# debbiemarkslab/EVcouplings

Hardware: AMD Instinct MI355X
Metric: plmc L-BFGS iterations/sec (PLM fit, synthetic MSA) (higher is better)
Workload: dtype f32 (forward: f16 hi/lo split couplings on the 2:4 sparse MFMA, f32 accumulation -- in the last iterations of a fit 39-bit fixed-point couplings as five int8 digit planes, exact; backward: 24-bit fixed-point residuals as three int8 digit planes on the int8 MFMA (32-bit / four there), exact int32 acc; 1 GPU; headline: synthetic MSA L=300 q=21 N=50000, theta=0.8, lambda_h=0.01, lambda_J=59.8; parallelism=single GPU

## Files before the change

### evcouplings_amd/_lib.py

```python
import ctypes as C
import os

_HERE = os.path.dirname(os.path.abspath(__file__))
LIB_PATH = os.environ.get("PLM_HIP_LIB") or os.path.join(_HERE, "libplm_hip.so")

PLM_OK = 0
STATUS_CONVERGED, STATUS_MAXITER, STATUS_LINESEARCH, STATUS_INTERRUPTED = 0, 1, 2, 3
ABI_VERSION = 2
K_EXPAND, K_FORWARD, K_BACKWARD, K_ASSEMBLE, K_TOTAL, K_REWEIGHT, K_FIELDS, K_FORWARD_ACCURATE, K_LBFGS_VECTOR, K_COUNT = 0, 1, 2, 3, 4, 5, 6, 7, 8, 9
S_COUNT = 7

ITER_CB = C.CFUNCTYPE(C.c_int, C.c_int32, C.c_double, C.c_double, C.c_double, C.c_double,
                      C.c_double, C.c_double, C.c_void_p)
EXCHANGE_CB = C.CFUNCTYPE(C.c_int, C.c_void_p, C.c_size_t, C.c_int32, C.c_int32, C.c_void_p)
COLLECTIVE_CB = C.CFUNCTYPE(C.c_int, C.c_int32, C.c_void_p, C.c_void_p, C.POINTER(C.c_int64),
                            C.POINTER(C.c_int64), C.c_int32, C.c_int32, C.c_void_p)
COLL_ALLTOALL, COLL_ALLREDUCE_F64, COLL_ALLREDUCE_F32, COLL_BROADCAST = 1, 2, 3, 4


class PlmProblem(C.Structure):
    _fields_ = [
        ("n_seqs", C.c_int32), ("n_sites", C.c_int32), ("n_states", C.c_int32),
        ("msa", C.c_void_p),
        ("theta_id", C.c_double), ("scale", C.c_double),
# ... 181 lines not shown
    ("plm_version", C.c_int, []),
    ("plm_device_count", C.c_int, []),
    ("plm_strerror", C.c_char_p, [C.c_int]),
    ("plm_last_error", C.c_char_p, []),
    ("plm_fit", C.c_int, [C.POINTER(PlmProblem), C.POINTER(PlmResult), C.c_int, _P, ITER_CB, _P,
                          EXCHANGE_CB, _P]),
    ("plm_fit_sharded", C.c_int, [C.POINTER(PlmProblem), C.POINTER(PlmResult), C.c_int, _P, ITER_CB, _P,
                                  COLLECTIVE_CB, _P]),
    ("plm_fit_sharded_rccl", C.c_int, [C.POINTER(PlmProblem), C.POINTER(PlmResult), C.c_int, _P, ITER_CB, _P, _P]),
    ("plm_rccl_unique_id", C.c_int, [_P]),
    ("plm_rccl_runtime_version", C.c_int, []),
    ("plm_rccl_selftest", C.c_int, [C.c_int, _P]),
    ("plm_ctx_attach_rccl", C.c_int, [_P, _P]),
    ("plm_reweight", C.c_int, [_P, C.c_int32, C.c_int32, C.c_double, _P]),
    ("plm_reweight_ex", C.c_int, [_P, C.c_int32, C.c_int32, C.c_double, C.c_int32, _P]),
    ("plm_marginals", C.c_int, [_P, _P, C.c_int32, C.c_int32, C.c_int32, _P, _P]),
    ("plm_eval", C.c_int, [_P, _P, C.c_int32, C.c_int32, C.c_int32, C.c_double, C.c_double, _P,
                           C.POINTER(C.c_double), C.POINTER(C.c_double), _P]),
    ("plm_scores", C.c_int, [_P, C.c_int32, C.c_int32, _P, _P]),
    ("plm_scores_ex", C.c_int, [_P, C.c_int32, C.c_int32, C.c_int32, _P, _P]),
    ("plm_hamiltonians", C.c_int, [_P, C.c_int32, C.c_int32, C.c_int32, _P, C.c_int, _P, _P]),
    ("plm_potentials", C.c_int, [_P, C.c_int32, C.c_int32, C.c_int32, _P, C.c_int, _P, _P]),
    ("plm_model_pair_scores", C.c_int, [_P, _P, _P, C.c_int32, C.c_int32, C.c_int, _P, _P, _P]),
    ("plm_model_pair_scores_ex", C.c_int, [_P, _P, _P, C.c_int32, C.c_int32, C.c_int32, C.c_int, _P, _P, _P]),
    ("plm_double_mutants", C.c_int, [_P, _P, _P, C.c_int32, C.c_int32, C.c_int, _P, _P]),
    ("plm_independent_fields", C.c_int, [_P, C.c_int32, C.c_int32, C.c_double, C.c_double, C.c_int, _P, _P, _P]),
    ("plm_sample", C.c_int, [C.c_int32, C.c_int32, _P, C.POINTER(PlmSampleOpts), C.c_int, _P, _P, _P]),
    ("plm_sample_plan", C.c_int, [C.c_int32, C.c_int32, C.c_int32, C.c_int32, C.POINTER(PlmSamplePlanInfo)]),
    ("plm_bm_fit", C.c_int, [C.c_int32, C.c_int32, _P, _P, _P, C.POINTER(PlmBmOpts), C.c_int, _P, BM_EPOCH_CB, _P,
                             C.POINTER(PlmBmResult)]),
    ("plm_ais", C.c_int, [C.c_int32, C.c_int32, _P, C.POINTER(PlmAisOpts), C.c_int, _P, AIS_CB, _P,
                          C.POINTER(PlmAisResult)]),
    ("plm_pt", C.c_int, [C.c_int32, C.c_int32, _P, C.POINTER(PlmPtOpts), C.c_int, _P, PT_CB, _P,
                         C.POINTER(PlmPtResult)]),
    ("plm_anneal", C.c_int, [C.c_int32, C.c_int32, _P, C.POINTER(PlmAnnealOpts), C.c_int, _P, ANNEAL_CB, _P,
                             C.POINTER(PlmAnnealResult)]),
    ("plm_meanfield", C.c_int, [_P, C.c_int32, C.c_int32, C.c_int32, C.c_double, C.c_double, C.c_int, _P,
                                C.POINTER(PlmMfResult)]),
    ("plm_direct_information", C.c_int, [_P, _P, C.c_int32, C.c_int32, C.c_int, _P, _P]),
    ("plm_alignment_stats", C.c_int, [_P, C.c_int32, C.c_int32, C.c_int32, _P, _P, _P, _P, C.c_int, _P]),
    ("plm_cross_identities", C.c_int, [_P, C.c_int32, _P, C.c_int32, C.c_int32, C.POINTER(PlmIdentOpts), _P, _P, _P, _P,
                                       C.c_int, _P]),
    ("plm_redundancy_filter", C.c_int, [_P, C.c_int32, C.c_int32, C.POINTER(PlmIdentOpts), _P, _P, C.c_int, _P]),
    ("plm_triplet_stats", C.c_int, [_P, _P, C.c_int32, C.c_int32, C.c_int32, _P, C.c_int32, C.POINTER(PlmTripletOpts), _P,
                                    _P, _P, C.POINTER(C.c_uint64), C.c_int, _P]),
    ("plm_triplet_scan", C.c_int, [_P, _P, C.c_int32, C.c_int32, C.c_int32, _P, C.c_int32, C.POINTER(PlmTripletOpts), _P,
                                   _P, _P, C.POINTER(C.c_uint64), C.c_int, _P]),
    ("plm_residue_distances", C.c_int, [_P, C.c_int32, _P, C.c_int32, _P, C.c_int32, _P, C.c_int32, _P, C.c_int, _P]),
    ("plm_distance_maps_aggregate", C.c_int, [_P, C.c_int32, _P, _P, C.c_int32, _P, _P, C.c_int32, C.c_int32, _P,
                                              C.c_int32, _P, _P, C.c_int, _P]),
    ("plm_fasta_split", C.c_int, [_P, C.c_int64, C.POINTER(C.c_int64), C.POINTER(C.c_int64), _P, _P, _P, _P]),
    ("plm_encode_columns", C.c_int, [_P, C.c_int64, C.c_int64, _P, C.c_int64, _P, _P, _P]),
    ("plm_write_raw_ec_file", C.c_int, [C.c_char_p, C.c_int32, _P, C.c_char_p, _P]),
    ("plm_ctx_create", C.c_int, [C.POINTER(PlmProblem), C.c_int, _P, C.POINTER(_P)]),
    ("plm_ctx_destroy", None, [_P]),
    ("plm_ctx_set_exchange", C.c_int, [_P, EXCHANGE_CB, _P]),
    ("plm_ctx_set_collective", C.c_int, [_P, COLLECTIVE_CB, _P]),
    ("plm_ctx_set_options", C.c_int, [_P, C.c_int32, C.c_double, C.c_int32]),
    ("plm_ctx_native_size", C.c_int64, [_P]),
    ("plm_ctx_reweight", C.c_int, [_P]),
    ("plm_ctx_set_weights", C.c_int, [_P, _P]),
    ("plm_ctx_get_weights", C.c_int, [_P, _P, _P, C.POINTER(C.c_float)]),
    ("plm_ctx_marginals", C.c_int, [_P, _P, _P]),
    ("plm_ctx_set_x", C.c_int, [_P, _P]),
    ("plm_ctx_get_x", C.c_int, [_P, _P]),
    ("plm_ctx_get_g", C.c_int, [_P, _P]),
    ("plm_ctx_eval", C.c_int, [_P, C.POINTER(C.c_double), C.POINTER(C.c_double)]),
    ("plm_ctx_optimize", C.c_int, [_P, ITER_CB, _P, C.POINTER(PlmResult)]),
    ("plm_ctx_scores", C.c_int, [_P, _P, _P]),
    ("plm_ctx_time_kernels", C.c_int, [_P, C.c_int32, _P]),
    ("plm_ctx_time_field_positions", C.c_int, [_P, C.c_int32, _P]),
    ("plm_ctx_solver_stats", C.c_int, [_P, _P]),
    ("plm_ctx_field_position", C.c_int, [_P, C.c_int32, C.c_int32, C.c_int32, C.c_int32, C.POINTER(PlmFieldBuffers)]),
    ("plm_ctx_field_solve", C.c_int, [_P, C.c_double, C.c_int32, C.c_int32, C.c_int32, C.POINTER(PlmFieldSolve), _P,
                                      C.c_int64]),
    ("plm_lbfgs_gram", C.c_int, [C.c_int64, C.c_int64, C.c_int32, C.c_int32, C.c_int32, _P, _P, _P, _P, _P, _P, _P, _P,
                                 C.c_int, _P, _P, _P, _P]),
    ("plm_lbfgs_direction", C.c_int, [C.c_int64, C.c_int32, C.c_int32, C.c_int32, _P, _P, _P, _P, _P, C.c_double, _P, _P,
                                      C.c_float, C.c_int, _P, _P]),
    ("plm_lbfgs_multidot", C.c_int, [C.c_int64, C.c_int32, _P, C.c_int32, _P, C.c_int32, _P, _P, C.c_uint32, C.c_uint64,
                                     C.c_int, _P]),
    ("plm_lbfgs_dots", C.c_int, [C.c_int64, C.c_int32, _P, C.c_int32, _P, _P, C.c_int64, C.c_int, _P]),
    ("plm_lbfgs_lincomb", C.c_int, [C.c_int64, C.c_float, _P, C.c_float, _P, C.c_int, _P]),
    ("plm_ctx_precond_diagonal", C.c_int, [_P, _P]),
    ("plm_rccl_probe", C.c_int, [_P, C.c_int32, C.c_int32, C.c_int, _P]),
    ("plm_rccl_probe_local", C.c_int, [C.c_int32, C.c_int, _P]),
    ("plm_lbfgs_coefficients", None, [C.c_int, C.c_int, C.c_int, _P, _P, _P, _P, C.c_double, _P, _P,
                                      C.POINTER(C.c_double), C.POINTER(C.c_double)]),
    ("plm_linesearch_run", C.c_int, [PHI_CB, _P, C.c_double, C.c_double, C.c_double, C.POINTER(C.c_int32),
                                     C.POINTER(C.c_int32), C.POINTER(C.c_double), _P]),
    ("plm_lbfgs_admit", C.c_int, [C.c_int32, C.POINTER(C.c_int32), C.POINTER(C.c_int32), C.POINTER(C.c_int32), _P, _P, _P,
                                  _P, C.POINTER(C.c_double), C.POINTER(C.c_double), _P, C.c_int32, C.c_int32, C.c_int32,
                                  C.c_int32, C.POINTER(C.c_int32), C.POINTER(C.c_int32)]),
    ("plm_mutant_effects", C.c_int, [_P, C.c_int32, C.c_int32, _P, C.c_int64, _P, C.c_int64, _P, _P, C.c_int, _P, _P, _P,
                                     _P]),
    ("plm_mutant_scan", C.c_int, [_P, C.c_int32, C.c_int32, _P, C.POINTER(PlmScanOpts), C.c_int, _P,
                                  C.POINTER(PlmScanResult)]),
]

_lib = None


class PlmError(RuntimeError):

    def __init__(self, code, message):
        super().__init__("libplm_hip error %d: %s" % (code, message))
        self.code = code


def load():
    global _lib
    if _lib is not None:
        return _lib
    if not os.path.exists(LIB_PATH):
        raise ImportError(
            "%s is missing: build it with `python -c 'import __graft_entry__ as g; g.build()'` "
            "(there is no CPU fallback for the PLM solver)" % LIB_PATH)
    lib = C.CDLL(LIB_PATH)
    for name, res, args in SYMBOLS:
        if os.environ.get("PLM_HIP_LIB") and not hasattr(lib, name):
            continue
        fn = getattr(lib, name)
        fn.restype = res
        fn.argtypes = args
    if lib.plm_version() != ABI_VERSION:
        raise ImportError("libplm_hip ABI version %d, expected %d" % (lib.plm_version(), ABI_VERSION))
    _lib = lib
    return lib


def check(rc):
    if rc != PLM_OK:
        lib = load()
        msg = lib.plm_last_error() or lib.plm_strerror(rc) or b""
        raise PlmError(rc, msg.decode("utf-8", "replace"))
```

### evcouplings_amd/csrc/plm_host.cpp

```cpp
#include "../../include/plm_hip.h"
#include "plm_internal.h"
#include "plm_host_util.h"
#include "plm_lbfgs.h"

#include <algorithm>
#include <chrono>
#include <cmath>
#include <cstdarg>
#include <cstdio>
#include <cstdlib>
#include <cstring>
#include <string>
#include <vector>

namespace {

thread_local std::string g_err;

int fail(int code, const char *fmt, ...) {
    char buf[512];
    va_list ap;
    va_start(ap, fmt);
    vsnprintf(buf, sizeof buf, fmt, ap);
    va_end(ap);
    g_err = buf;
    return code;
}

}
int plm_fail(int code, const char *fmt, ...) {
    char buf[512];
    va_list ap;
    va_start(ap, fmt);
    vsnprintf(buf, sizeof buf, fmt, ap);
    va_end(ap);
    return fail(code, "%s", buf);
}
namespace {

double now_s() {
    return std::chrono::duration<double>(std::chrono::steady_clock::now().time_since_epoch()).count();
}

int check_device(int device) {
    int n = 0;
    if (hipGetDeviceCount(&n) != hipSuccess || n <= 0)
        return fail(PLM_EDEVICE, "no HIP device visible (libplm_hip has no CPU path)");
    if (device < 0 || device >= n) return fail(PLM_EINVAL, "device %d out of range (%d visible)", device, n);
    hipDeviceProp_t prop;
    PLM_HIP(hipGetDeviceProperties(&prop, device));
    if (strncmp(prop.gcnArchName, "gfx950", 6) != 0)
        return fail(PLM_EDEVICE, "device %d is %s; this library is built for gfx950 only", device, prop.gcnArchName);
    PLM_HIP(hipSetDevice(device));
    return PLM_OK;
}

}
int plm_check_device(int device) { return check_device(device); }
namespace {

int cluster_threshold(double theta_id, int L, int conv) {
    if (conv & PLM_CONV_THRESHOLD_F32) {
        const float t = (float)(1.0 - theta_id);
        const float need = (1.0f - t) * (float)L;
        return (int)std::ceil(need);
    }
    return (int)std::ceil(theta_id * (double)L - 1e-9);
}

}
PlmOptions plm_options_from_env() {
    PlmOptions o;
    if (const char *e = getenv("PLM_BWD_PLANES")) o.bwd_planes = atoi(e) == 4 ? 4 : 3;
    if (const char *e = getenv("PLM_KSPLIT")) o.ksplit = std::max(1, atoi(e));
    if (const char *e = getenv("PLM_JEXP_BIAS")) o.jexp_bias = atoi(e);
    if (const char *e = getenv("PLM_BWD_KERNEL")) o.bwd_kernel = atoi(e) ? 1 : 0;
    if (const char *e = getenv("PLM_FWD_KERNEL")) o.fwd_kernel = atoi(e) ? 1 : 0;
    if (const char *e = getenv("PLM_FWD_ACCURATE")) o.fwd_mode = atoi(e) ? 1 : 0;
    if (const char *e = getenv("PLM_VP_FLOOR")) o.vp_floor = atof(e);
    if (const char *e = getenv("PLM_VP_REL")) o.vp_rel = atof(e);
    if (const char *e = getenv("PLM_VP_HESS_POS")) o.vp_hess_pos = atoi(e);
    if (const char *e = getenv("PLM_ACC_FACTOR")) o.acc_factor = atof(e);
    o.debug = getenv("PLM_DEBUG") != nullptr;
    o.debug_vp = getenv("PLM_DEBUG_VP") != nullptr;
    return o;
}
namespace {

int pick_ksplit(const PlmDims &d, const PlmOptions &opt, int nplanes, int *out) {
    const int ks_min = std::max(1, (d.nst128 + 1022) / 1023);
    const int ks_max = std::max(ks_min, std::max(1, std::min(16, d.nst128 / 8)));
    if ((int64_t)((d.nst128 + ks_min - 1) / ks_min) * PLM_BWD_KSTEP * 128 * 128 >= ((int64_t)1 << 31))
        return fail(PLM_EUNSUPPORTED, "%d sequences: no admissible K split of the backward GEMM", d.N);
    const double beta = (2.0 * nplanes * (double)d.nmf * d.nnfl * 1024.0 / 12e12) / ((double)d.nst128 * 1.3e-6);
    int best = ks_min;
    double best_cost = 1e300;
    for (int ks = ks_min; ks <= ks_max; ks++) {
        const int groups_per_xcd = (d.ncol_tiles * nplanes * ks + 7) / 8;
        const double cost = (double)((groups_per_xcd * d.nrow_tiles + 31) / 32) / ks + beta * ks;
        if (cost < best_cost * 0.98) { best_cost = cost; best = ks; }
    }
    if (opt.ksplit) best = std::max(ks_min, std::min(ks_max, opt.ksplit));
    *out = best;
    return PLM_OK;
}

int make_dims(const plm_problem_t &p, const PlmOptions &opt, PlmDims *out) {
    PlmDims d;
    memset(&d, 0, sizeof d);
    if (p.n_seqs <= 0 || p.n_sites <= 1) return fail(PLM_EINVAL, "need n_seqs > 0 and n_sites > 1");
    if (!plm_q_supported(p.n_states))
        return fail(PLM_EUNSUPPORTED, "alphabet size %d outside 2..32", p.n_states);
    const int nshards = p.n_shards > 0 ? p.n_shards : 1;
    if (p.shard < 0 || p.shard >= nshards) return fail(PLM_EINVAL, "shard %d outside 0..%d", p.shard, nshards - 1);
    d.N = p.n_seqs;
    d.L = p.n_sites;
    d.Qc = p.n_states;
    d.Q = plm_q_template(p.n_states);
    d.Np = (d.N + PLM_SEQ_TILE - 1) / PLM_SEQ_TILE * PLM_SEQ_TILE;
    d.nb16 = (d.L + 15) / 16;
    d.Lp16 = d.nb16 * 16;
    d.nu = (d.L + 31) / 32;
    d.Lp32 = d.nu * 32;
    d.nksteps = d.nu * PLM_FWD_TILES(d.Q);
    d.nssteps = d.Np / 32;
    d.nst128 = d.Np / PLM_BWD_KSTEP;
    d.nplanes = (p.epsilon > 0 && p.epsilon < 1e-4) ? 4 : 3;
    if (opt.bwd_planes) d.nplanes = opt.bwd_planes;
    d.jexp_bias = opt.jexp_bias;
    const float qmax = d.nplanes == 4 ? PLM_R_QMAX4 : PLM_R_QMAX3;
    d.rscale = qmax;
    d.gscale = 1.0f / (qmax * (float)PLM_BWD_ONEHOT_VALUE);
    d.nstiles = d.Np / PLM_SEQ_TILE;
    plm_pick_tile(d.Q, &d.FM, &d.FN);
    d.nmf = d.nb16 * d.Q + d.FM;
    d.nshards = nshards;
    d.shard = p.shard;
    d.blk_per_shard = (d.nb16 + nshards - 1) / nshards;
    d.shard_base = d.nb16 / nshards;
    d.shard_rem = d.nb16 % nshards;
    d.b16_lo = plm_shard_lo(d, d.shard);
    d.b16_hi = d.b16_lo + plm_shard_cnt(d, d.shard);
    d.nnfl = d.blk_per_shard * d.Q;
    d.nrow_tiles = (d.nmf + 4 * d.FM - 1) / (4 * d.FM);
    d.ncol_tiles = (d.nnfl + 2 * d.FN - 1) / (2 * d.FN);
    d.fwd_w = (d.Q == 21 && opt.fwd_kernel != 0) ? 1 : 0;
    d.bwd_w = (d.Q == 21 && opt.bwd_kernel != 0) ? 1 : 0;
    if (d.bwd_w) d.ncol_tiles = (d.nnfl + PLM_BWDW_COLS - 1) / PLM_BWDW_COLS;
    PLM_TRY(pick_ksplit(d, opt, d.nplanes, &d.ksplit));
    d.nbp = (int64_t)d.nb16 * (d.nb16 + 1) / 2;
    d.nh_pad = ((int64_t)d.L * d.Q + 255) / 256 * 256;
    d.n_native = d.nh_pad + d.nbp * d.Q * d.Q * 256;
    d.n_canon = (int64_t)d.L * d.Qc + (int64_t)d.L * (d.L - 1) / 2 * d.Qc * d.Qc;
    d.gap_mode = (p.flags & PLM_FLAG_IGNORE_GAPS) ? 1 : 0;
    d.conv = p.flags & PLM_CONV_MASK;
    d.theta = p.theta_id;
    d.sharded = ((p.flags & PLM_FLAG_SHARDED_STATE) && nshards > 1) ? 1 : 0;
    d.own_lo = d.sharded ? d.b16_lo : 0;
    d.own_hi = d.sharded ? d.b16_hi : d.nb16;
    d.nblk_own = d.own_hi - d.own_lo;
    d.h_site0 = d.own_lo * 16;
    d.bp_base = 0;
    for (int p = 0; p < PLM_MAX_SHARDS; p++) d.own_base[p] = d.oth_base[p] = -1;
    d.nx_halo = d.ng_halo = 0;
    if (d.sharded) {
        if (nshards > PLM_MAX_SHARDS) return fail(PLM_EUNSUPPORTED, "sharded-state mode takes at most %d shards", PLM_MAX_SHARDS);
        d.ntri = d.nblk_own * (d.nblk_own + 1) / 2;
        for (int p = 0; p < nshards; p++) {
            if (p == d.shard) continue;
            const int64_t mine = plm_half_blocks(d, p), theirs = (int64_t)d.nblk_own * plm_shard_cnt(d, p) - mine;
            d.own_base[p] = (int)d.ng_halo;
            d.ng_halo += mine;
            d.oth_base[p] = (int)d.nx_halo;
            d.nx_halo += theirs;
        }
        d.np_own = d.ntri + d.ng_halo;
    } else {
        d.np_own = d.nbp;
        d.ntri = (int)d.nbp;
    }
    {
        const int site_end = std::min(d.L, d.own_hi * 16);
        const int64_t nhl = (int64_t)std::max(0, site_end - d.h_site0) * d.Q;
        d.nh_pad_l = d.sharded ? std::max<int64_t>(256, (nhl + 255) / 256 * 256) : d.nh_pad;
    }
    d.n_local = d.nh_pad_l + d.np_own * d.Q * d.Q * 256;
    if (d.gap_mode && d.Qc < 3) return fail(PLM_EINVAL, "ignore_gaps needs at least 2 non-gap states");
    *out = d;
    return PLM_OK;
}

}

struct plm_ctx {
    plm_problem_t prob;
    PlmOptions opt;
    PlmDims d;
    int device = 0;
    hipStream_t st = nullptr;
    plm_exchange_cb exchange = nullptr;
    void *exchange_user = nullptr;
    int8_t *msa_rm = nullptr, *msa_cm = nullptr;
    float *w = nullptr;
    int32_t *counts = nullptr;
    void *Bt = nullptr, *Rt = nullptr;
    int32_t *G = nullptr;
    float *gather = nullptr;
    plm_collective_cb collective = nullptr;
    void *collective_user = nullptr;
    PlmRccl *rccl = nullptr;
    float *xhalo = nullptr, *ghalo = nullptr, *xsend = nullptr, *gsend = nullptr;
    std::vector<int64_t> x_send, x_recv, g_send, g_recv;
    double *fx_part = nullptr, *reg_part = nullptr, *dot_scratch = nullptr, *scal = nullptr;
    uint32_t *maxbits = nullptr;
    int32_t *jexp = nullptr;
    float *x = nullptr, *g = nullptr, *xp = nullptr, *gp = nullptr, *dir = nullptr, *hist = nullptr;
    float *xa = nullptr, *ga = nullptr;
    float *canon = nullptr;
    float *pair_n2 = nullptr;
    float *dinv = nullptr;
    float *hj = nullptr, *hpart = nullptr;
    double *gpart = nullptr, *dpart = nullptr;
    double *hg2 = nullptr, *hinv = nullptr, *h64 = nullptr;
    double *hcnt = nullptr;
    bool hcnt_valid = false;
    int *vp_flag = nullptr;
    int vp_hess_age = -1;
    int vp_c_prev = 3;
    int vp_pos = 0;
    unsigned vp_hess_mask = 0;
    int vp_extra = 0;
    double vp_last_gh2 = 0;
    double vp_floor2 = 0;
    hipEvent_t vp_ev[2] = {nullptr, nullptr};
    hipEvent_t gemm_ev[3] = {nullptr, nullptr, nullptr};
    bool vp_ev_pending = false;
    double stat_field_ms = 0, stat_passes = 0, stat_fwd_ms = 0, stat_bwd_ms = 0;
    int stat_gemm_evals = 0;
    int stat_field_evals = 0, stat_chain_short = 0;
    int hist_m = 0;
    double *h_scal = nullptr;
    bool have_weights = false;
    float wmax = 0;
    bool eval_valid = false;
    bool hj_at_x = false;
    double last_fx = 0, last_nll = 0, last_gh2 = 0;
    bool eval_vp = false;
    bool fwd_accurate = false;
    bool eval_accurate = false;
    int planes_base = 3, ksplit_base = 1, ksplit4 = 1;
    double n_eff = 0;
    int n_evals = 0;
    std::vector<float> h_fi;

    int n_fx_part() const { return d.nstiles * (d.b16_hi - d.b16_lo); }
};

namespace {

std::vector<int8_t> padded_rows(const PlmDims &d, const int8_t *seqs) {
    return plm_padded_rows(seqs, d.N, d.L, (size_t)d.Np + 32, (size_t)d.Lp32, (int8_t)PLM_PAD_STATE);
}

void ctx_set_accurate(plm_ctx *c, bool on) {
    c->fwd_accurate = on;
    const int planes = c->opt.bwd_planes ? c->opt.bwd_planes : (on ? 4 : c->planes_base);
    c->d.nplanes = planes;
    c->d.ksplit = planes == 4 ? c->ksplit4 : c->ksplit_base;
    const float qmax = planes == 4 ? PLM_R_QMAX4 : PLM_R_QMAX3, wmax = c->wmax > 0 ? c->wmax : 1.f;
    c->d.rscale = qmax / wmax;
    c->d.gscale = wmax / (qmax * (float)PLM_BWD_ONEHOT_VALUE);
}

int ctx_alloc_lbfgs(plm_ctx *c, int m) {
    if (c->xp && c->hist_m >= m) return PLM_OK;
    const size_t n = (size_t)c->d.n_local;
    if (!c->xp) {
        PLM_TRY(plm_dalloc(&c->xp, n));
        PLM_TRY(plm_dalloc(&c->gp, n));
        PLM_TRY(plm_dalloc(&c->dir, n));
    }
    if (c->hist) (void)hipFree(c->hist);
    c->hist = nullptr;
    PLM_TRY(plm_dalloc(&c->hist, n * 2 * (size_t)m));
    c->hist_m = m;
    return PLM_OK;
}

int ctx_collective(plm_ctx *c, int op, void *send, void *recv, const int64_t *scounts, const int64_t *rcounts) {
    if (c->rccl) {
        if (plm_rccl_collective(c->rccl, op, send, recv, scounts, rcounts, c->st) != 0)
            return fail(PLM_ECALLBACK, "RCCL collective failed (op %d): %s", op, plm_rccl_error());
        return PLM_OK;
    }
    if (!c->collective) return fail(PLM_EINVAL, "sharded-state mode needs a collective callback or an RCCL communicator");
    PLM_HIP(hipStreamSynchronize(c->st));
    if (c->collective(op, send, recv, scounts, rcounts, c->d.nshards, c->d.shard, c->collective_user) != 0)
        return fail(PLM_ECALLBACK, "collective callback failed (op %d)", op);
    return PLM_OK;
}
int ctx_allreduce_scalars(plm_ctx *c, int first, int count) {
    if (!c->d.sharded) return PLM_OK;
    const int64_t bytes = (int64_t)sizeof(double) * count;
    return ctx_collective(c, PLM_COLL_ALLREDUCE_F64, c->scal + first, c->scal + first, &bytes, &bytes);
}

int group_norms(plm_ctx *c) {
    if (!(c->prob.lambda_group > 0)) return PLM_OK;
    if (!c->pair_n2) PLM_TRY(plm_dalloc(&c->pair_n2, (size_t)std::max<int64_t>(1, c->d.np_own) * 256));
    PLM_HIP(plm_launch_pair_norms(c->d, c->x, c->pair_n2, c->st));
    return PLM_OK;
}
int vp_alloc(plm_ctx *c);
int forward_at_x(plm_ctx *c) {
    const PlmDims &d = c->d;
    PLM_TRY(vp_alloc(c));
    PLM_HIP(plm_launch_forward_store(d, c->msa_rm, c->Bt, c->jexp, c->hj, c->fwd_accurate, c->st));
    PLM_HIP(plm_launch_h64_init(d, c->x, c->h64, c->st));
    PLM_HIP(plm_launch_hpass(d, c->hj, c->msa_rm, c->w, c->h64, 1, 0, c->fwd_accurate, c->Rt, c->fx_part, nullptr, nullptr, nullptr, nullptr, PLM_VP_ALWAYS, c->st));
    return PLM_OK;
}

float *x_rectangles(plm_ctx *c) { return c->x + c->d.nh_pad_l + (size_t)c->d.ntri * PLM_BLOCK_FLOATS(c->d); }

int ctx_eval_enqueue_sharded(plm_ctx *c) {
    const PlmDims &d = c->d;
    PLM_TRY(ctx_collective(c, PLM_COLL_ALLTOALL, x_rectangles(c), c->xhalo, c->x_send.data(), c->x_recv.data()));
    PLM_HIP(plm_launch_maxabs2(c->x + d.nh_pad_l, d.n_local - d.nh_pad_l, c->xhalo,
                               d.nx_halo * (int64_t)PLM_BLOCK_FLOATS(d), c->maxbits, c->jexp, d.jexp_bias, c->st));
    PLM_HIP(plm_launch_expand(d, c->x, c->xhalo, c->jexp, c->Bt, c->fwd_accurate ? 1 : 0, c->st));
    PLM_TRY(forward_at_x(c));
    if (d.nblk_own > 0) PLM_HIP(plm_launch_backward(d, c->msa_cm, c->Rt, c->G, nullptr, c->st));
    PLM_HIP(plm_launch_pack_g(d, c->G, c->gsend, c->st));
    PLM_TRY(ctx_collective(c, PLM_COLL_ALLTOALL, c->gsend, c->ghalo, c->g_send.data(), c->g_recv.data()));
    PLM_TRY(group_norms(c));
    PLM_HIP(plm_launch_assemble(d, c->G, d.ksplit, c->ghalo, c->x, c->g, c->prob.lambda_h, c->prob.lambda_j,
                                c->reg_part, 0, 0.f, c->pair_n2, (float)c->prob.lambda_group, c->st));
    PLM_HIP(plm_launch_finish_fx(d, c->fx_part, c->n_fx_part(), nullptr, 0, c->reg_part, plm_reg_parts(d), c->scal,
                                 c->st));
    c->n_evals++;
    return PLM_OK;
}

int ctx_eval_enqueue(plm_ctx *c) {
    const PlmDims &d = c->d;
    if (d.sharded) return ctx_eval_enqueue_sharded(c);
    PLM_HIP(plm_launch_maxabs(d, c->x, c->maxbits, c->jexp, c->st));
    PLM_HIP(plm_launch_expand(d, c->x, nullptr, c->jexp, c->Bt, c->fwd_accurate ? 1 : 0, c->st));
    PLM_TRY(forward_at_x(c));
    PLM_HIP(plm_launch_backward(d, c->msa_cm, c->Rt, c->G, nullptr, c->st));
    const void *Gsrc = c->G;
    int ks_count = d.ksplit, n_shard_nll = 0;
    const double *shard_nll = nullptr;
    if (d.nshards > 1) {
        const size_t slab = plm_slab_bytes(d);
        char *mine = (char *)c->gather + (size_t)d.shard * slab;
        PLM_HIP(plm_launch_slab_reduce(d, c->G, (float *)mine, c->st));
        PLM_HIP(plm_launch_partial_sum(c->fx_part, c->n_fx_part(), (double *)(mine + slab - 256), c->st));
        PLM_HIP(hipStreamSynchronize(c->st));
        if (!c->exchange) return fail(PLM_EINVAL, "n_shards > 1 but no exchange callback set");
        if (c->exchange(c->gather, slab, d.nshards, d.shard, c->exchange_user) != 0)
            return fail(PLM_ECALLBACK, "exchange callback failed");
        Gsrc = c->gather;
        ks_count = 0;
        n_shard_nll = d.nshards;
        shard_nll = (const double *)((char *)c->gather + slab - 256);
    }
    PLM_TRY(group_norms(c));
    PLM_HIP(plm_launch_assemble(d, Gsrc, ks_count, nullptr, c->x, c->g, c->prob.lambda_h, c->prob.lambda_j,
                                c->reg_part, 0, 0.f, c->pair_n2, (float)c->prob.lambda_group, c->st));
    PLM_HIP(plm_launch_finish_fx(d, c->fx_part, c->n_fx_part(), shard_nll, n_shard_nll, c->reg_part,
                                 plm_reg_parts(d), c->scal, c->st));
    c->n_evals++;
    return PLM_OK;
}

bool vp_enabled(const plm_ctx *c) {
    return !(c->prob.flags & PLM_FLAG_JOINT_LBFGS) && (c->d.nshards == 1 || c->d.sharded) && c->prob.lambda_h > 0;
}
int vp_alloc(plm_ctx *c) {
    if (c->hj) return PLM_OK;
    const size_t nsites = (size_t)std::max(std::max(1, (c->d.b16_hi - c->d.b16_lo) * 16),
                                           std::min(c->d.L, c->d.own_hi * 16) - c->d.h_site0);
    PLM_TRY(plm_dalloc((char **)&c->hj, plm_hj_bytes(c->d)));
    PLM_TRY(plm_dalloc((char **)&c->hpart, plm_hpart_bytes(c->d)));
    PLM_TRY(plm_dalloc((char **)&c->gpart, plm_gpart_bytes(c->d)));
    PLM_TRY(plm_dalloc((char **)&c->dpart, plm_gpart_bytes(c->d)));
    PLM_TRY(plm_dalloc(&c->hg2, nsites));
    PLM_TRY(plm_dalloc(&c->hinv, nsites * c->d.Q * c->d.Q));
    PLM_TRY(plm_dalloc(&c->h64, 2 * plm_h64_stride(c->d)));
    PLM_TRY(plm_dalloc(&c->hcnt, plm_h64_stride(c->d)));
    c->hcnt_valid = false;
    PLM_TRY(plm_dalloc((char **)&c->vp_flag, sizeof(PlmVpState)));
    PLM_HIP(hipMemsetAsync(c->vp_flag, 0, sizeof(PlmVpState), c->st));
    for (auto &e : c->vp_ev) PLM_HIP(hipEventCreate(&e));
    for (auto &e : c->gemm_ev) PLM_HIP(hipEventCreate(&e));
    c->vp_hess_age = -1;
    return PLM_OK;
}
int vp_counts(plm_ctx *c) {
    if (!c->hcnt_valid) {
        PLM_HIP(plm_launch_site_counts(c->d, c->msa_cm, c->w, c->hcnt, c->st));
        c->hcnt_valid = true;
    }
    return PLM_OK;
}
int vp_stage1(plm_ctx *c) {
    const PlmDims &d = c->d;
    PLM_TRY(vp_counts(c));
    if (d.sharded) {
        PLM_TRY(ctx_collective(c, PLM_COLL_ALLTOALL, x_rectangles(c), c->xhalo, c->x_send.data(), c->x_recv.data()));
        PLM_HIP(plm_launch_maxabs2(c->x + d.nh_pad_l, d.n_local - d.nh_pad_l, c->xhalo,
                                   d.nx_halo * (int64_t)PLM_BLOCK_FLOATS(d), c->maxbits, c->jexp, d.jexp_bias, c->st));
        PLM_HIP(plm_launch_expand(d, c->x, c->xhalo, c->jexp, c->Bt, c->fwd_accurate ? 1 : 0, c->st));
    } else {
        PLM_HIP(plm_launch_maxabs(d, c->x, c->maxbits, c->jexp, c->st));
        PLM_HIP(plm_launch_expand(d, c->x, nullptr, c->jexp, c->Bt, c->fwd_accurate ? 1 : 0, c->st));
    }
    if (c->gemm_ev[0]) PLM_HIP(hipEventRecord(c->gemm_ev[0], c->st));
    PLM_HIP(plm_launch_forward_store(d, c->msa_rm, c->Bt, c->jexp, c->hj, c->fwd_accurate, c->st));
    PLM_HIP(plm_launch_h64_init(d, c->x, c->h64, c->st));
    return PLM_OK;
}
int vp_counts(plm_ctx *c);
int vp_step_and_residuals(plm_ctx *c, bool refresh) {
    const PlmDims &d = c->d;
    PLM_TRY(vp_counts(c));
    const int full = (refresh || c->vp_hess_age < 0) ? 1 : 0;
    PLM_HIP(plm_launch_hpass(d, c->hj, c->msa_rm, c->w, c->h64, 0, full ? 2 : 1, c->fwd_accurate, nullptr, nullptr, c->hpart,
                             c->gpart, c->dpart, nullptr, PLM_VP_ALWAYS, c->st));
    PLM_HIP(plm_launch_hsolve(d, c->hpart, c->gpart, full, c->x, c->h64, c->prob.lambda_h, 1, c->hinv, c->hg2, c->scal + 5, 0.0,
                              0.0, nullptr, 0, c->hcnt, c->dpart, c->st));
    if (full) c->vp_hess_age = 0;
    PLM_HIP(plm_launch_hpass(d, c->hj, c->msa_rm, c->w, c->h64, 1, 1, c->fwd_accurate, c->Rt, c->fx_part, c->hpart, c->gpart,
                             nullptr, nullptr, PLM_VP_ALWAYS, c->st));
    PLM_HIP(plm_launch_hsolve(d, c->hpart, c->gpart, 0, c->x, c->h64, c->prob.lambda_h, 0, c->hinv, c->hg2, c->scal + 5, 0.0,
                              0.0, nullptr, 0, c->hcnt, c->dpart, c->st));
    return PLM_OK;
}
int vp_chain(plm_ctx *c, int npos, int hess_upto, int expected_last, double tol2) {
    const PlmDims &d = c->d;
    for (int k = 0; k < npos; k++) {
        const int pos = c->vp_pos++;
        const bool hess = pos < hess_upto || pos > expected_last || c->vp_hess_age < 0;
        PLM_HIP(plm_launch_hpass(d, c->hj, c->msa_rm, c->w, c->h64, 0, hess ? 2 : 1, c->fwd_accurate, nullptr, nullptr, c->hpart,
                                 c->gpart, c->dpart, c->vp_flag, PLM_VP_PASS, c->st));
        PLM_HIP(plm_launch_hpass(d, c->hj, c->msa_rm, c->w, c->h64, 1, 1, c->fwd_accurate, c->Rt, c->fx_part, c->hpart, c->gpart,
                                 nullptr, c->vp_flag, PLM_VP_PASS_RT, c->st));
        PLM_HIP(plm_launch_hsolve(d, c->hpart, c->gpart, hess ? 2 : 0, c->x, c->h64, c->prob.lambda_h, 1, c->hinv, c->hg2,
                                  c->scal + 5, tol2, c->vp_floor2, c->vp_flag, 1, c->hcnt, c->dpart, c->st));
        if (hess && pos < 32) c->vp_hess_mask |= 1u << pos;
        if (hess && c->vp_hess_age < 0) c->vp_hess_age = 0;
    }
    return PLM_OK;
}
int vp_stage3(plm_ctx *c, bool conditional, float *gout = nullptr, int mode = 2) {
    const PlmDims &d = c->d;
    if (!gout) gout = c->g;
    if (c->gemm_ev[1]) PLM_HIP(hipEventRecord(c->gemm_ev[1], c->st));
    if (d.nblk_own > 0 || !d.sharded)
        PLM_HIP(plm_launch_backward(d, c->msa_cm, c->Rt, c->G, (conditional && !d.sharded) ? c->vp_flag : nullptr, c->st));
    if (c->gemm_ev[2]) PLM_HIP(hipEventRecord(c->gemm_ev[2], c->st));
    if (d.sharded) {
        PLM_HIP(plm_launch_pack_g(d, c->G, c->gsend, c->st));
        PLM_TRY(ctx_collective(c, PLM_COLL_ALLTOALL, c->gsend, c->ghalo, c->g_send.data(), c->g_recv.data()));
    }
    PLM_TRY(group_norms(c));
    PLM_HIP(plm_launch_assemble(d, c->G, d.ksplit, d.sharded ? c->ghalo : nullptr, c->x, gout, c->prob.lambda_h,
                                c->prob.lambda_j, c->reg_part, mode, 0.f, c->pair_n2, (float)c->prob.lambda_group, c->st));
    if (mode == 2)
        PLM_HIP(plm_launch_finish_fx(d, c->fx_part, c->n_fx_part(), nullptr, 0, c->reg_part, plm_reg_parts(d), c->scal,
                                     c->st));
    return PLM_OK;
}
int ctx_eval_vp_enqueue(plm_ctx *c, double tol2) {
    const PlmDims &d = c->d;
    PLM_TRY(vp_stage1(c));
    if (c->vp_ev_pending) c->vp_ev_pending = false;
    PLM_HIP(hipEventRecord(c->vp_ev[0], c->st));
    const int c_prev = c->vp_c_prev;
    if (c->vp_hess_age >= 0) c->vp_hess_age++;
    const bool stale = c->vp_hess_age < 0 || c->vp_hess_age >= 32;
    PLM_HIP(plm_launch_vp_reset(c->vp_flag, (c_prev == 0 && !stale) ? 1 : 0, c->scal + 5, c->st));
    c->vp_pos = 0;
    c->vp_extra = 0;
    c->vp_hess_mask = 0;
    c->vp_last_gh2 = INFINITY;
    int hess_upto = c_prev >= 2 ? c_prev : (stale ? 1 : 0);
    if (c->opt.vp_hess_pos >= 0) hess_upto = std::min(hess_upto, std::max(c->opt.vp_hess_pos, c->vp_hess_age < 0 ? 1 : 0));
    PLM_TRY(vp_chain(c, std::min(14, c_prev + 3), hess_upto, c_prev, tol2));
    PLM_HIP(plm_launch_fields_to_x(d, c->h64, c->vp_flag, c->x, c->st));
    PLM_HIP(plm_launch_hpass(d, c->hj, c->msa_rm, c->w, c->h64, 1, 0, c->fwd_accurate, c->Rt, c->fx_part, nullptr, nullptr, nullptr,
                             c->vp_flag, PLM_VP_FINAL, c->st));
    PLM_HIP(hipEventRecord(c->vp_ev[1], c->st));
    c->vp_ev_pending = true;
    PLM_TRY(vp_stage3(c, true));
    c->n_evals++;
    return PLM_OK;
}
// ... 73 lines not shown
template <class Fetch>
int ctx_eval_vp_run(plm_ctx *c, double tol2, Fetch &&fetch, double *gh2_out) {
    PLM_TRY(ctx_eval_vp_enqueue(c, tol2));
    for (;;) {
        PLM_TRY(fetch());
        bool again = false;
        PLM_TRY(ctx_eval_vp_finish(c, tol2, &again, gh2_out));
        if (!again) break;
    }
    return PLM_OK;
}

int dots(plm_ctx *c, int npairs, const float *const *a, const float *const *b, int64_t n, int slot) {
    PLM_HIP(plm_launch_dots(npairs, a, b, n, c->dot_scratch, c->scal + slot, c->st));
    return PLM_OK;
}

const char *status_text(int status) {
    switch (status) {
    case PLM_STATUS_CONVERGED: return "converged (|g|/max(1,|x|) below epsilon)";
    case PLM_STATUS_MAXITER: return "maximum number of iterations reached";
    case PLM_STATUS_INTERRUPTED: return "interrupted by the caller";
    default: return "line search could not improve further (treated as converged to precision)";
    }
}

int set_start_point(plm_ctx *c) {
    const PlmDims &d = c->d;
    if (c->h_fi.empty()) return fail(PLM_EINVAL, "start point needs single-site frequencies: run marginals first");
    std::vector<float> h((size_t)d.nh_pad_l, 0.f);
    const int a0 = d.gap_mode;
    for (int i = d.h_site0; i < std::min(d.L, d.own_hi * 16); i++) {
        double mean = 0;
        std::vector<double> v(d.Q);
        for (int a = a0; a < d.Qc; a++) {
            v[a] = std::log((double)c->h_fi[(size_t)i * d.Qc + a] + 1.0 / c->n_eff);
            mean += v[a];
        }
        mean /= (d.Qc - a0);
        for (int a = a0; a < d.Qc; a++) h[(size_t)(i - d.h_site0) * d.Q + a] = (float)(v[a] - mean);
    }
    c->eval_valid = false;
    PLM_HIP(hipMemsetAsync(c->x, 0, sizeof(float) * d.n_local, c->st));
    PLM_HIP(hipMemcpyAsync(c->x, h.data(), sizeof(float) * d.nh_pad_l, hipMemcpyHostToDevice, c->st));
    PLM_HIP(hipStreamSynchronize(c->st));
    return PLM_OK;
}

}

extern "C" {

int plm_version(void) { return PLM_ABI_VERSION; }

int plm_device_count(void) {
    int n = 0;
    if (hipGetDeviceCount(&n) != hipSuccess) return fail(PLM_EDEVICE, "hipGetDeviceCount failed");
    return n;
}

const char *plm_strerror(int code) {
    switch (code) {
    case PLM_OK: return "ok";
    case PLM_EINVAL: return "invalid argument";
    case PLM_ENOMEM: return "out of memory";
    case PLM_EDEVICE: return "HIP device error";
    case PLM_EUNSUPPORTED: return "unsupported alphabet size";
    case PLM_ENUMERIC: return "non-finite value in objective";
    case PLM_ECALLBACK: return "exchange callback failed";
    default: return "unknown error";
    }
}

const char *plm_last_error(void) { return g_err.c_str(); }

void plm_ctx_destroy(plm_ctx_t *c) {
    if (!c) return;
    (void)hipSetDevice(c->device);
    for (auto &e : c->gemm_ev)
        if (e) (void)hipEventDestroy(e);
    for (auto &e : c->vp_ev)
        if (e) (void)hipEventDestroy(e);
    void *bufs[] = {c->msa_rm, c->msa_cm, c->w, c->counts, c->Bt, c->Rt, c->G, c->gather, c->fx_part, c->reg_part,
                    c->dot_scratch, c->scal, c->maxbits, c->jexp, c->x, c->g, c->xp, c->gp, c->dir, c->hist,
                    c->canon, c->xhalo, c->ghalo, c->xsend, c->gsend, c->dinv, c->hj, c->hpart, c->gpart, c->dpart, c->hg2, c->hinv, c->h64, c->hcnt, c->vp_flag,
                    c->xa, c->ga, c->pair_n2};
    for (void *b : bufs)
        if (b) (void)hipFree(b);
    if (c->h_scal) (void)hipHostFree(c->h_scal);
    if (c->rccl) {
        (void)hipStreamSynchronize(c->st);
        plm_rccl_destroy(c->rccl);
    }
    delete c;
}

struct CtxScope {
    plm_ctx_t *c;
    ~CtxScope() { plm_ctx_destroy(c); }
};

int plm_ctx_create(const plm_problem_t *prob, int device, void *stream, plm_ctx_t **out) {
    if (!prob || !out || !prob->msa) return fail(PLM_EINVAL, "NULL problem / msa / out");
    *out = nullptr;
    PLM_TRY(check_device(device));
    const PlmOptions opt = plm_options_from_env();
    PlmDims d;
    PLM_TRY(make_dims(*prob, opt, &d));
    if (!(prob->theta_id >= 0.0 && prob->theta_id <= 1.0)) return fail(PLM_EINVAL, "theta_id must be in [0,1]");
    if (prob->lambda_h < 0 || prob->lambda_j < 0 || prob->lambda_group < 0)
        return fail(PLM_EINVAL, "negative regularisation strength");
    for (size_t k = 0; k < (size_t)d.N * d.L; k++)
        if (prob->msa[k] < 0 || prob->msa[k] >= d.Qc)
            return fail(PLM_EINVAL, "msa[%zu] = %d outside 0..%d", k, (int)prob->msa[k], d.Qc - 1);
    plm_ctx *c = new plm_ctx();
    c->prob = *prob;
    c->prob.msa = nullptr;
    c->opt = opt;
    c->d = d;
    c->planes_base = d.nplanes;
    c->ksplit_base = d.ksplit;
    {
        int ks4 = 1;
        const int rc4 = pick_ksplit(d, opt, 4, &ks4);
        if (rc4 != PLM_OK) { delete c; return rc4; }
        c->ksplit4 = ks4;
    }
    PlmDims dmax = d;
    dmax.nplanes = opt.bwd_planes ? opt.bwd_planes : 4;
    dmax.ksplit = std::max(c->ksplit_base, c->ksplit4);
    c->device = device;
    c->st = (hipStream_t)stream;
    CtxScope scope{c};
    const size_t cm_rows = (size_t)(d.nb16 + 1) * 16, cm_size = cm_rows * d.Np;
    const std::vector<int8_t> rm = padded_rows(d, prob->msa);
    {
        const int m = std::min(20, prob->lbfgs_m > 0 ? prob->lbfgs_m : 6);
        const double need = (double)rm.size() + (double)cm_size + (double)plm_bt_bytes(d) + (double)plm_rt_bytes(dmax) +
                            (double)plm_g_bytes(dmax) + (vp_enabled(c) ? (double)plm_hj_bytes(d) : 0.0) +
                            4.0 * ((double)d.n_local * (2 * m + 5) + (double)d.n_canon + (double)d.L * d.L);
        PLM_TRY(plm_check_free(need, "the problem"));
    }
    PLM_TRY(plm_dalloc(&c->msa_rm, rm.size()));
    PLM_TRY(plm_dalloc(&c->msa_cm, cm_size));
    PLM_TRY(plm_dalloc(&c->w, (size_t)d.Np));
    PLM_TRY(plm_dalloc(&c->counts, (size_t)d.Np));
    PLM_TRY(plm_dalloc((char **)&c->Bt, plm_bt_bytes(d)));
    PLM_TRY(plm_dalloc((char **)&c->Rt, plm_rt_bytes(dmax)));
    PLM_TRY(plm_dalloc((char **)&c->G, plm_g_bytes(dmax)));
    PLM_TRY(plm_dalloc(&c->fx_part, (size_t)c->n_fx_part()));
    PLM_TRY(plm_dalloc(&c->reg_part, (size_t)plm_reg_parts(d)));
    PLM_TRY(plm_dalloc(&c->dot_scratch, (size_t)4 * PLM_MAX_BASIS * PLM_DOT_BLOCKS));
    PLM_TRY(plm_dalloc(&c->scal, (size_t)256));
    PLM_TRY(plm_dalloc(&c->maxbits, (size_t)1));
    PLM_TRY(plm_dalloc(&c->jexp, (size_t)1));
    PLM_TRY(plm_dalloc(&c->x, (size_t)d.n_local));
    PLM_TRY(plm_dalloc(&c->g, (size_t)d.n_local));
    PLM_TRY(plm_dalloc(&c->canon, (size_t)d.n_canon + (size_t)d.L * d.L));
    if (d.nshards > 1 && !d.sharded) PLM_TRY(plm_dalloc((char **)&c->gather, plm_slab_bytes(d) * d.nshards));
    if (d.sharded) {
        const size_t blk = PLM_BLOCK_FLOATS(d);
        PLM_TRY(plm_dalloc(&c->xhalo, (size_t)d.nx_halo * blk));
        PLM_TRY(plm_dalloc(&c->gsend, (size_t)d.nx_halo * blk));
        PLM_TRY(plm_dalloc(&c->ghalo, (size_t)d.ng_halo * blk));
        c->x_send.assign(d.nshards, 0); c->x_recv.assign(d.nshards, 0);
        c->g_send.assign(d.nshards, 0); c->g_recv.assign(d.nshards, 0);
        for (int r = 0; r < d.nshards; r++) {
            if (r == d.shard) continue;
            const int64_t mine = plm_half_blocks(d, r), theirs = (int64_t)d.nblk_own * plm_shard_cnt(d, r) - mine;
            c->x_send[r] = c->g_recv[r] = mine * (int64_t)blk * 4;
            c->x_recv[r] = c->g_send[r] = theirs * (int64_t)blk * 4;
        }
    }
    const hipError_t eh = hipHostMalloc((void **)&c->h_scal, sizeof(double) * 256);
    if (eh != hipSuccess) return fail(PLM_ENOMEM, "hipHostMalloc failed: %s", hipGetErrorString(eh));
    PLM_HIP(hipMemcpyAsync(c->msa_rm, rm.data(), rm.size(), hipMemcpyHostToDevice, c->st));
    PLM_HIP(plm_launch_msa_columns(d, c->msa_rm, c->msa_cm, (int)cm_rows, c->st));
    PLM_HIP(hipMemsetAsync(c->w, 0, sizeof(float) * d.Np, c->st));
    PLM_HIP(hipMemsetAsync(c->Rt, 0, plm_rt_bytes(dmax), c->st));
    PLM_HIP(hipMemsetAsync(c->x, 0, sizeof(float) * d.n_local, c->st));
    PLM_HIP(hipMemsetAsync(c->g, 0, sizeof(float) * d.n_local, c->st));
    PLM_HIP(hipMemsetAsync(c->scal, 0, sizeof(double) * 256, c->st));
    if (c->gather) PLM_HIP(hipMemsetAsync(c->gather, 0, plm_slab_bytes(d) * d.nshards, c->st));
    PLM_HIP(hipStreamSynchronize(c->st));
    scope.c = nullptr;
    *out = c;
    return PLM_OK;
}

int plm_ctx_set_exchange(plm_ctx_t *c, plm_exchange_cb exchange, void *user) {
    if (!c) return fail(PLM_EINVAL, "NULL ctx");
    c->exchange = exchange;
    c->exchange_user = user;
    return PLM_OK;
}

int plm_ctx_set_collective(plm_ctx_t *c, plm_collective_cb collective, void *user) {
    if (!c) return fail(PLM_EINVAL, "NULL ctx");
    c->collective = collective;
    c->collective_user = user;
    return PLM_OK;
}

int plm_ctx_attach_rccl(plm_ctx_t *c, const void *rccl_id) {
    if (!c || !rccl_id) return fail(PLM_EINVAL, "NULL ctx / id");
    if (c->rccl) return fail(PLM_EINVAL, "context already has a communicator");
    PLM_HIP(hipSetDevice(c->device));
    if (plm_rccl_init(rccl_id, c->d.nshards, c->d.shard, &c->rccl) != 0)
        return fail(PLM_ECALLBACK, "RCCL communicator of %d ranks: %s", c->d.nshards, plm_rccl_error());
    return PLM_OK;
}

int plm_rccl_unique_id(void *id_out) {
    if (!id_out) return fail(PLM_EINVAL, "NULL id");
    if (plm_rccl_id(id_out) != 0) return fail(PLM_ECALLBACK, "%s", plm_rccl_error());
    return PLM_OK;
}
int plm_rccl_runtime_version(void) { return plm_rccl_version(); }

int plm_rccl_selftest(int device, void *stream) {
    PLM_TRY(check_device(device));
    hipStream_t st = (hipStream_t)stream;
    unsigned char id[PLM_RCCL_ID_BYTES];
    PLM_TRY(plm_rccl_unique_id(id));
    PlmRccl *r = nullptr;
    if (plm_rccl_init(id, 1, 0, &r) != 0) return fail(PLM_ECALLBACK, "%s", plm_rccl_error());
    const int n = 1000;
    double *buf = nullptr;
    DeviceBuffers mem;
    int rc = mem.alloc(&buf, (size_t)2 * n);
    std::vector<double> h(2 * n, 0.0), back(2 * n, -1.0);
    for (int k = 0; k < n; k++) h[k] = 0.5 * k - 7.0;
    const int64_t bytes = (int64_t)sizeof(double) * n, root = 0;
    auto run = [&](int op, void *s, void *d) {
        if (rc == PLM_OK && plm_rccl_collective(r, op, s, d, &bytes, op == PLM_COLL_BROADCAST ? &root : &bytes, st) != 0)
            rc = fail(PLM_ECALLBACK, "op %d: %s", op, plm_rccl_error());
    };
    if (rc == PLM_OK && hipMemcpyAsync(buf, h.data(), sizeof(double) * 2 * n, hipMemcpyHostToDevice, st) != hipSuccess)
// ... 245 lines not shown
int plm_ctx_get_g(plm_ctx_t *c, float *g_canonical_host) { return get_vec(c, c ? c->g : nullptr, g_canonical_host); }

int plm_ctx_eval(plm_ctx_t *c, double *fx_out, double *nll_out) {
    if (!c) return fail(PLM_EINVAL, "NULL ctx");
    if (!c->have_weights) return fail(PLM_EINVAL, "weights not set");
    PLM_HIP(hipSetDevice(c->device));
    ctx_set_accurate(c, c->opt.fwd_mode != 0);
    PLM_TRY(ctx_eval_enqueue(c));
    if (c->d.sharded) PLM_TRY(ctx_allreduce_scalars(c, 0, 2));
    c->eval_valid = false;
    if (fx_out || nll_out) {
        PLM_TRY(fetch_scalars(c, 0, 2));
        if (fx_out) *fx_out = c->h_scal[0];
        if (nll_out) *nll_out = c->h_scal[1];
        c->eval_valid = true;
        c->eval_vp = false;
        c->eval_accurate = c->fwd_accurate;
        c->last_fx = c->h_scal[0];
        c->last_nll = c->h_scal[1];
    }
    return PLM_OK;
}

static int ctx_build_dinv(plm_ctx_t *c) {
    const PlmDims &d = c->d;
    if (!c->dinv) PLM_TRY(plm_dalloc(&c->dinv, (size_t)d.n_local));
    const size_t lq = (size_t)d.L * d.Q;
    std::vector<float> fv(2 * lq, 0.f);
    const int a0 = d.gap_mode;
    for (int i = 0; i < d.L; i++) {
        double tot = 0;
        for (int a = a0; a < d.Qc; a++) tot += (double)c->h_fi[i * d.Qc + a] + 1.0 / c->n_eff;
        for (int a = a0; a < d.Qc; a++) {
            const double pa = ((double)c->h_fi[i * d.Qc + a] + 1.0 / c->n_eff) / tot;
            fv[i * d.Q + a] = c->h_fi[i * d.Qc + a];
            fv[lq + i * d.Q + a] = (float)(pa * (1.0 - pa));
        }
    }
    PLM_HIP(hipMemcpyAsync(c->canon, fv.data(), sizeof(float) * fv.size(), hipMemcpyHostToDevice, c->st));
    PLM_HIP(plm_launch_precond(d, c->canon, (float)c->n_eff, (float)c->prob.lambda_h, (float)c->prob.lambda_j,
                               c->dinv, c->st));
    PLM_HIP(hipStreamSynchronize(c->st));
    return PLM_OK;
}
static void lbfgs_gram_basis(const float *S, const float *Y, const float *g, int64_t n, int nst, PlmVecList *B,
                             unsigned long long *wb_out, unsigned *wq_out) {
    B->n = 0;
    for (int i = 0; i < nst; i++) B->v[B->n++] = S + (size_t)i * n;
    unsigned long long wb = 0;
    for (int i = 0; i < nst; i++) { wb |= 1ull << B->n; B->v[B->n++] = Y + (size_t)i * n; }
    wb |= 1ull << B->n;
    B->v[B->n++] = g;
    B->v[B->n++] = g;
    *wb_out = wb;
    *wq_out = 6u;
}
static int lbfgs_direction_basis(const float *S, const float *Y, const float *g, int64_t n, int m, int stored, int end,
                                 const double *cs, const double *cy, double cg, PlmVecList *B, PlmCoefList *C) {
    B->n = 0;
    for (int i = 0; i < stored; i++) { const int j = lbfgs_live_slot(m, end, i); B->v[B->n] = S + (size_t)j * n; C->c[B->n++] = (float)cs[j]; }
    const int first_weighted = B->n;
    for (int i = 0; i < stored; i++) { const int j = lbfgs_live_slot(m, end, i); B->v[B->n] = Y + (size_t)j * n; C->c[B->n++] = (float)cy[j]; }
    B->v[B->n] = g;
    C->c[B->n++] = (float)cg;
    return first_weighted;
}

int plm_ctx_optimize(plm_ctx_t *c, plm_iter_cb cb, void *user, plm_result_t *res) {
    if (!c) return fail(PLM_EINVAL, "NULL ctx");
    if (!c->have_weights) return fail(PLM_EINVAL, "weights not set");
    PLM_HIP(hipSetDevice(c->device));
    const double eps = c->prob.epsilon > 0 ? c->prob.epsilon : 1e-3;
    const double t0 = now_s();
    const PlmDims &d = c->d;
    const int64_t n = d.n_local;
    const int m = std::min(20, c->prob.lbfgs_m > 0 ? c->prob.lbfgs_m : 6);
    const int max_iter = c->prob.max_iter;
    PLM_TRY(ctx_alloc_lbfgs(c, m));
    float *S = c->hist, *Y = c->hist + (size_t)m * n;
    const bool precond = (c->prob.flags & PLM_FLAG_PRECOND) && !c->h_fi.empty();
    if (precond) PLM_TRY(ctx_build_dinv(c));
    const float *dinv = precond ? c->dinv : nullptr;
    LbfgsHistory hist(m);
    double xx = 0, hh = 0;
    c->n_evals = 0;
    enum { SL_FX = 0, SL_NLL = 1, SL_DG = 2, SL_XX = 3, SL_HH = 4, SL_GH2 = 5, SL_MD = 8 };

    auto norm_dots = [&]() -> int {
        const float *a[1] = {c->x};
        PLM_TRY(dots(c, 1, a, a, n, SL_XX));
        PLM_TRY(dots(c, 1, a, a, d.nh_pad_l, SL_HH));
        return PLM_OK;
    };
    auto direction = [&](double *dginit, const float *xacc, float stp0, float *trial) -> int {
        double cg;
        hist.coefficients(&cg, dginit);
        PlmVecList B;
        PlmCoefList C;
        const int first_weighted =
            lbfgs_direction_basis(S, Y, c->g, n, m, hist.stored, hist.end, hist.cs.data(), hist.cy.data(), cg, &B, &C);
        if (trial) PLM_HIP(plm_launch_multiaxpy_trial(c->dir, B, C, n, dinv, first_weighted, xacc, stp0, trial, c->st));
        else PLM_HIP(plm_launch_multiaxpy(c->dir, B, C, n, dinv, first_weighted, c->st));
        return PLM_OK;
    };

    const bool vp = vp_enabled(c);
    if (vp) PLM_TRY(vp_alloc(c));
    c->stat_field_ms = c->stat_passes = c->stat_fwd_ms = c->stat_bwd_ms = 0;
    c->stat_field_evals = c->stat_chain_short = c->stat_gemm_evals = 0;
    double gh2 = 0;
    const double vp_rel = c->opt.vp_rel;
    c->vp_floor2 = ctx_vp_floor2(c);
    auto vp_tol2 = [&](double xnorm2) {
        const double t = std::max(0.1 * eps * std::max(1.0, std::sqrt(xnorm2)), vp_rel * std::sqrt(hist.gg));
        return t * t;
    };
    const double fwd_noise = 3e-11 * (double)d.N * (double)d.L;
    const double acc_thr = std::max(3.0 * eps, c->opt.acc_factor * fwd_noise);
    auto want_accurate = [&](double cond) {
        return c->opt.fwd_mode == 1 || (c->opt.fwd_mode != 0 && fwd_noise > 0.05 * eps && cond < acc_thr);
    };
    const bool resume = c->eval_valid && c->eval_vp == vp;
    ctx_set_accurate(c, c->opt.fwd_mode == 1 || (c->opt.fwd_mode != 0 && resume && c->eval_accurate));
    auto start_eval = [&](bool have) -> int {
        const double tol2 = vp_tol2((double)d.L);
        auto fetch = [&]() -> int {
            PlmVecList Qg, Bg;
            Qg.n = 1; Qg.v[0] = c->g;
            Bg.n = 2; Bg.v[0] = c->g; Bg.v[1] = c->g;
            PLM_HIP(plm_launch_multidot(Qg, Bg, n, c->dot_scratch, c->scal + SL_MD, dinv, 1u, 1ull, c->st));
            PLM_TRY(norm_dots());
            PLM_TRY(ctx_allreduce_scalars(c, have ? SL_DG : 0, (have ? 8 - SL_DG : 8) + 2));
            PLM_TRY(fetch_scalars(c, 0, 10));
            return PLM_OK;
        };
        if (vp && !have) {
            PLM_TRY(ctx_eval_vp_run(c, tol2, fetch, &gh2));
        } else {
            if (!have) PLM_TRY(ctx_eval_enqueue(c));
            PLM_TRY(fetch());
        }
        hist.gDg = c->h_scal[SL_MD];
        hist.gg = c->h_scal[SL_MD + 1];
        xx = c->h_scal[SL_XX];
        hh = c->h_scal[SL_HH];
        return PLM_OK;
    };
    PLM_TRY(start_eval(resume));
    if (resume) gh2 = c->last_gh2;
    double fx = resume ? c->last_fx : c->h_scal[SL_FX], nll = resume ? c->last_nll : c->h_scal[SL_NLL];
    c->eval_valid = false;
    if (!std::isfinite(fx)) return fail(PLM_ENUMERIC, "objective is not finite at the start point");
    if (!c->fwd_accurate && want_accurate(std::sqrt(hist.gg + gh2) / std::max(1.0, std::sqrt(xx)))) {
        ctx_set_accurate(c, true);
        PLM_TRY(start_eval(false));
        fx = c->h_scal[SL_FX];
        nll = c->h_scal[SL_NLL];
    }
    auto shipped_cond = [&](double *out) -> int {
        PLM_HIP(plm_launch_h64_init(d, c->x, c->h64, c->st));
        PLM_HIP(plm_launch_hpass(d, c->hj, c->msa_rm, c->w, c->h64, 1, 0, c->fwd_accurate, c->Rt, c->fx_part, nullptr, nullptr,
                                 nullptr, nullptr, PLM_VP_ALWAYS, c->st));
        PLM_TRY(vp_stage3(c, false, c->dir, 0));
        const float *a[1] = {c->dir};
        PLM_TRY(dots(c, 1, a, a, n, SL_DG));
        PLM_TRY(ctx_allreduce_scalars(c, SL_DG, 1));
        PLM_TRY(fetch_scalars(c, SL_DG, 1));
        *out = std::sqrt(c->h_scal[SL_DG]) / std::max(1.0, std::sqrt(xx));
        return PLM_OK;
    };
    double eps_eff = eps;
    double rounding_note = 0;
    int n_cert = 0;
    int k = 0, status = PLM_STATUS_CONVERGED, ls_reason = 0, restarts = 0;
    double last_cond = std::sqrt(hist.gg + gh2) / std::max(1.0, std::sqrt(xx));
    if (last_cond <= eps && vp && (!resume || c->hj_at_x)) {
        double cj = 0;
        PLM_TRY(shipped_cond(&cj));
        const double r2 = std::max(0.0, cj * cj - last_cond * last_cond);
        if (cj > eps && r2 >= 0.75 * eps * eps) rounding_note = std::sqrt(r2);
        else if (cj > eps) { eps_eff = std::sqrt(eps * eps - r2); last_cond = cj; }
    }
    if (last_cond > eps) {
        auto first_step = [&]() { return precond ? std::min(1.0, 1.0 / std::sqrt(hist.gDg)) : 1.0 / std::sqrt(hist.gg); };
        double step = first_step();
        for (k = 1;; k++) {
            double dginit;
            const float stp0 = (float)std::max(MtSearch::stpmin, std::min(MtSearch::stpmax, step));
            PLM_TRY(direction(&dginit, c->x, stp0, c->xp));
            if (!(dginit < 0)) { status = PLM_STATUS_LINESEARCH; ls_reason = 10; k--; break; }
            std::swap(c->x, c->xp);
            std::swap(c->g, c->gp);
            const double finit = fx, nllinit = nll;
            float *s_new = S + (size_t)hist.end * n, *y_new = Y + (size_t)hist.end * n;
            const int nst = hist.nst();
            PlmVecList B;
            unsigned long long wb;
            unsigned wq;
            lbfgs_gram_basis(S, Y, c->g, n, nst, &B, &wb, &wq);
            double gh2_trial = 0;
            auto evaluate_trial = [&]() -> int {
                const double tol2 = vp_tol2(xx);
                if (!vp) PLM_TRY(ctx_eval_enqueue(c));
                else PLM_TRY(ctx_eval_vp_enqueue(c, tol2));
              for (;;) {
                PLM_HIP(plm_launch_sy_multidot(s_new, y_new, c->x, hist.anchored ? c->xa : c->xp, c->g, hist.anchored ? c->ga : c->gp,
                                               c->dir, B, n, d.nh_pad_l, c->dot_scratch, c->scal + SL_MD, c->scal + SL_DG, dinv,
                                               wq, wb, c->st));
                PLM_TRY(ctx_allreduce_scalars(c, SL_FX, SL_MD + 3 * B.n + 1 - SL_FX));
                PLM_TRY(fetch_scalars(c, SL_FX, SL_MD + 3 * B.n + 1 - SL_FX));
                bool again = false;
                if (vp) PLM_TRY(ctx_eval_vp_finish(c, tol2, &again, &gh2_trial));
                if (!again) break;
              }
                return PLM_OK;
            };
            MtSearch ls;
            ls.start(finit, dginit, step);
            int lsrc;
            do {
                const double stp = ls.next();
                if (!(ls.count == 0 && (float)stp == stp0))
                    PLM_HIP(plm_launch_lincomb(c->x, 1.f, c->xp, (float)stp, c->dir, n, c->st));
                PLM_TRY(evaluate_trial());
                double dg = c->h_scal[SL_DG];
                fx = c->h_scal[SL_FX];
                nll = c->h_scal[SL_NLL];
                lsrc = ls.feed(fx, dg);
            } while (lsrc == 0);
            if (lsrc < 0 && c->opt.debug) ls.dump_failure(k, lsrc);
            if (lsrc < 0) {
                std::swap(c->x, c->xp);
                std::swap(c->g, c->gp);
                fx = finit;
                nll = nllinit;
                k--;
                if (hist.stored > 0 && restarts < 2) {
                    restarts++;
                    hist.reset();
                    step = first_step();
                    continue;
                }
                status = PLM_STATUS_LINESEARCH;
                ls_reason = -lsrc;
                break;
            }
            restarts = 0;
            if (c->opt.debug)
                fprintf(stderr, "[plm] it %d: %d trial(s), step %.4e (first %.4e), f - f0 = %.6e, dg0 = %.4e, dg = %.4e%s\n", k, ls.count, ls.stp,
                        ls.trace[0][0], fx - finit, dginit, c->h_scal[SL_DG], c->fwd_accurate ? " [accurate]" : "");
            step = ls.stp;
            const double *md = c->h_scal + SL_MD;
            const int nbv = B.n;
            bool straddle = false;
            if (!c->fwd_accurate &&
                want_accurate(std::sqrt(md[2 * nbv + 2 * nst + 1] + gh2_trial) / std::max(1.0, std::sqrt(c->h_scal[SL_XX])))) {
                ctx_set_accurate(c, true);
                straddle = true;
                PLM_TRY(evaluate_trial());
                fx = c->h_scal[SL_FX];
                nll = c->h_scal[SL_NLL];
                if (!std::isfinite(fx)) return fail(PLM_ENUMERIC, "objective is not finite after the switch of the forward GEMM");
            }
            hist.absorb(md, nbv, nst);
            xx = c->h_scal[SL_XX];
            hh = c->h_scal[SL_HH];
            gh2 = gh2_trial;
            const double xnorm = std::sqrt(xx), gnorm = std::sqrt(hist.gg + gh2);
            last_cond = gnorm / std::max(1.0, xnorm);
            if (cb && cb(k, now_s() - t0, last_cond, fx, nll, std::sqrt(hh), std::sqrt(std::max(0.0, xx - hh)), user) != 0) {
                status = PLM_STATUS_INTERRUPTED;
                break;
            }
            if (last_cond <= eps_eff) {
                if (!vp) { status = PLM_STATUS_CONVERGED; break; }
                double cj = 0;
                PLM_TRY(shipped_cond(&cj));
                if (!(cj > eps)) { last_cond = cj; status = PLM_STATUS_CONVERGED; break; }
                const double r2 = std::max(0.0, cj * cj - last_cond * last_cond);
                if (r2 >= 0.75 * eps * eps || ++n_cert > 8) {
                    status = PLM_STATUS_CONVERGED;
                    rounding_note = std::sqrt(r2);
                    break;
                }
                eps_eff = std::min(0.9 * eps_eff, std::sqrt(eps * eps - r2));
            }
            if (max_iter > 0 && k >= max_iter) { status = PLM_STATUS_MAXITER; break; }
            if (hist.admit(md, nbv, nst, vp, straddle, c->opt.debug).copy_anchor) {
                if (!c->xa) {
                    PLM_TRY(plm_dalloc(&c->xa, (size_t)n));
                    PLM_TRY(plm_dalloc(&c->ga, (size_t)n));
                }
                PLM_HIP(hipMemcpyAsync(c->xa, c->xp, sizeof(float) * n, hipMemcpyDeviceToDevice, c->st));
                PLM_HIP(hipMemcpyAsync(c->ga, c->gp, sizeof(float) * n, hipMemcpyDeviceToDevice, c->st));
            }
            step = 1.0;
        }
    }
    PLM_HIP(hipStreamSynchronize(c->st));
    c->eval_valid = true;
    c->hj_at_x = vp && status != PLM_STATUS_LINESEARCH;
    c->eval_vp = vp;
    c->eval_accurate = c->fwd_accurate;
    c->last_fx = fx;
    c->last_nll = nll;
    c->last_gh2 = gh2;
// ... 201 lines not shown
        PLM_HIP(hipMemset(*p, 0xFF, sizeof(T) * n_elems));
        return PLM_OK;
    }
    int nan_scratch() {
        if (!scratch) PLM_TRY(mem.alloc(&scratch, n_scratch));
        PLM_HIP(hipMemset(scratch, 0xFF, sizeof(double) * n_scratch));
        return PLM_OK;
    }
    template <typename T> int download(T *host, const T *p, size_t n_elems) {
        PLM_HIP(hipMemcpy(host, p, sizeof(T) * n_elems, hipMemcpyDeviceToHost));
        return PLM_OK;
    }
};
int lbfgs_probe_length(int64_t n) {
    if (n <= 0 || (n & 3)) return fail(PLM_EINVAL, "the vector length must be a positive multiple of 4, not %lld", (long long)n);
    return PLM_OK;
}
}
}

int plm_lbfgs_gram(int64_t n, int64_t nh, int32_t m, int32_t end, int32_t nst, const float *S, const float *Y,
                   const float *x, const float *xp, const float *g, const float *gp, const float *dir, const float *dinv,
                   int device, float *s_new, float *y_new, double *md, double *ex) {
    if (!S || !Y || !x || !xp || !g || !gp || !dir || !s_new || !y_new || !md || !ex) return fail(PLM_EINVAL, "NULL argument");
    PLM_TRY(lbfgs_probe_length(n));
    if (nh < 0 || (nh & 3) || nh > n) return fail(PLM_EINVAL, "nh must be a multiple of 4 in 0..n, not %lld", (long long)nh);
    if (m < 1 || nst < 1 || nst > m) return fail(PLM_EINVAL, "need 1 <= nst <= m (m = %d, nst = %d)", (int)m, (int)nst);
    if (2 * nst + 2 > PLM_MAX_BASIS) return fail(PLM_EINVAL, "%d basis vectors, at most %d", 2 * (int)nst + 2, PLM_MAX_BASIS);
    if (end < 0 || end >= m) return fail(PLM_EINVAL, "ring slot %d outside 0..%d", (int)end, (int)m - 1);
    if (end >= nst) return fail(PLM_EINVAL, "the new pair's slot %d is not among the %d slots of the basis", (int)end, (int)nst);
    PLM_TRY(check_device(device));
    LbfgsProbe P;
    float *dS, *dY, *dx, *dxp, *dg, *dgp, *ddir, *ddinv = nullptr;
    double *dmd, *dex;
    const size_t nn = (size_t)n;
    PLM_TRY(P.upload(&dS, S, (size_t)nst * nn));
    PLM_TRY(P.upload(&dY, Y, (size_t)nst * nn));
    PLM_TRY(P.upload(&dx, x, nn));
    PLM_TRY(P.upload(&dxp, xp, nn));
    PLM_TRY(P.upload(&dg, g, nn));
    PLM_TRY(P.upload(&dgp, gp, nn));
    PLM_TRY(P.upload(&ddir, dir, nn));
    if (dinv) PLM_TRY(P.upload(&ddinv, dinv, nn));
    PlmVecList B;
    unsigned long long wb;
    unsigned wq;
    lbfgs_gram_basis(dS, dY, dg, n, nst, &B, &wb, &wq);
    PLM_TRY(P.nan_out(&dmd, (size_t)3 * B.n + 1));
    PLM_TRY(P.nan_out(&dex, 3));
    PLM_TRY(P.nan_scratch());
    float *ds_new = dS + (size_t)end * nn, *dy_new = dY + (size_t)end * nn;
    PLM_HIP(plm_launch_sy_multidot(ds_new, dy_new, dx, dxp, dg, dgp, ddir, B, n, nh, P.scratch, dmd, dex, ddinv, wq, wb, nullptr));
    PLM_HIP(hipDeviceSynchronize());
    PLM_TRY(P.download(s_new, ds_new, nn));
    PLM_TRY(P.download(y_new, dy_new, nn));
    PLM_TRY(P.download(md, dmd, (size_t)3 * B.n + 1));
    PLM_TRY(P.download(ex, dex, 3));
    return PLM_OK;
}

int plm_lbfgs_direction(int64_t n, int32_t m, int32_t stored, int32_t end, const float *S, const float *Y, const float *g,
                        const double *cs, const double *cy, double cg, const float *dinv, const float *xacc, float stp0,
                        int device, float *dir, float *trial) {
    if (!S || !Y || !g || !cs || !cy || !dir) return fail(PLM_EINVAL, "NULL argument");
    if (trial && !xacc) return fail(PLM_EINVAL, "a trial point needs xacc");
    PLM_TRY(lbfgs_probe_length(n));
    if (m < 1 || stored < 0 || stored > m) return fail(PLM_EINVAL, "need 0 <= stored <= m (m = %d, stored = %d)", (int)m, (int)stored);
    if (2 * stored + 1 > PLM_MAX_BASIS) return fail(PLM_EINVAL, "%d basis vectors, at most %d", 2 * (int)stored + 1, PLM_MAX_BASIS);
    if (end < 0 || end >= m) return fail(PLM_EINVAL, "ring slot %d outside 0..%d", (int)end, (int)m - 1);
    PLM_TRY(check_device(device));
    LbfgsProbe P;
    float *dS, *dY, *dg, *ddinv = nullptr, *dxacc = nullptr, *ddir, *dtrial = nullptr;
    const size_t nn = (size_t)n;
    PLM_TRY(P.upload(&dS, S, (size_t)m * nn));
    PLM_TRY(P.upload(&dY, Y, (size_t)m * nn));
    PLM_TRY(P.upload(&dg, g, nn));
    if (dinv) PLM_TRY(P.upload(&ddinv, dinv, nn));
    if (trial) PLM_TRY(P.upload(&dxacc, xacc, nn));
    PLM_TRY(P.nan_out(&ddir, nn));
    if (trial) PLM_TRY(P.nan_out(&dtrial, nn));
    PlmVecList B;
    PlmCoefList C;
    const int first_weighted = lbfgs_direction_basis(dS, dY, dg, n, m, stored, end, cs, cy, cg, &B, &C);
    if (trial) PLM_HIP(plm_launch_multiaxpy_trial(ddir, B, C, n, ddinv, first_weighted, dxacc, stp0, dtrial, nullptr));
    else PLM_HIP(plm_launch_multiaxpy(ddir, B, C, n, ddinv, first_weighted, nullptr));
    PLM_HIP(hipDeviceSynchronize());
    PLM_TRY(P.download(dir, ddir, nn));
    if (trial) PLM_TRY(P.download(trial, dtrial, nn));
    return PLM_OK;
}

int plm_lbfgs_multidot(int64_t n, int32_t nv, const float *V, int32_t nq, const int32_t *q_index, int32_t nb,
                       const int32_t *b_index, const float *dinv, uint32_t wq, uint64_t wb, int device, double *out) {
    if (!V || !q_index || !b_index || !out) return fail(PLM_EINVAL, "NULL argument");
    PLM_TRY(lbfgs_probe_length(n));
    if (nv < 1) return fail(PLM_EINVAL, "no vectors");
    if (nq < 1 || nq > 4) return fail(PLM_EINVAL, "%d queries, need 1..4", (int)nq);
    if (nb < 1 || nb > PLM_MAX_BASIS) return fail(PLM_EINVAL, "%d basis vectors, need 1..%d", (int)nb, PLM_MAX_BASIS);
    for (int k = 0; k < nq; k++)
        if (q_index[k] < 0 || q_index[k] >= nv) return fail(PLM_EINVAL, "query %d names vector %d of %d", k, (int)q_index[k], (int)nv);
    for (int k = 0; k < nb; k++)
        if (b_index[k] < 0 || b_index[k] >= nv) return fail(PLM_EINVAL, "basis entry %d names vector %d of %d", k, (int)b_index[k], (int)nv);
    PLM_TRY(check_device(device));
    LbfgsProbe P;
    float *dV, *ddinv = nullptr;
    double *dout;
    const size_t nn = (size_t)n;
    PLM_TRY(P.upload(&dV, V, (size_t)nv * nn));
    if (dinv) PLM_TRY(P.upload(&ddinv, dinv, nn));
    PLM_TRY(P.nan_out(&dout, (size_t)nq * nb));
    PLM_TRY(P.nan_scratch());
    PlmVecList Qv, B;
    Qv.n = nq;
    for (int k = 0; k < nq; k++) Qv.v[k] = dV + (size_t)q_index[k] * nn;
    B.n = nb;
    for (int k = 0; k < nb; k++) B.v[k] = dV + (size_t)b_index[k] * nn;
    PLM_HIP(plm_launch_multidot(Qv, B, n, P.scratch, dout, ddinv, wq, wb, nullptr));
    PLM_HIP(hipDeviceSynchronize());
    PLM_TRY(P.download(out, dout, (size_t)nq * nb));
    return PLM_OK;
}

int plm_lbfgs_dots(int64_t stride, int32_t nv, const float *V, int32_t npairs, const int32_t *a_index,
                   const int32_t *b_index, int64_t n, int device, double *out) {
    if (!V || !a_index || !b_index || !out) return fail(PLM_EINVAL, "NULL argument");
    PLM_TRY(lbfgs_probe_length(stride));
    if (n < 0 || (n & 3) || n > stride) return fail(PLM_EINVAL, "n must be a multiple of 4 in 0..stride, not %lld", (long long)n);
    if (nv < 1) return fail(PLM_EINVAL, "no vectors");
    if (npairs < 1 || npairs > 4) return fail(PLM_EINVAL, "%d pairs, need 1..4", (int)npairs);
    for (int k = 0; k < npairs; k++)
        if (a_index[k] < 0 || a_index[k] >= nv || b_index[k] < 0 || b_index[k] >= nv)
            return fail(PLM_EINVAL, "pair %d names vectors %d, %d of %d", k, (int)a_index[k], (int)b_index[k], (int)nv);
    PLM_TRY(check_device(device));
    LbfgsProbe P;
    float *dV;
    double *dout;
    const size_t ns = (size_t)stride;
    PLM_TRY(P.upload(&dV, V, (size_t)nv * ns));
    PLM_TRY(P.nan_out(&dout, (size_t)npairs));
    PLM_TRY(P.nan_scratch());
    const float *a[4], *b[4];
    for (int k = 0; k < npairs; k++) { a[k] = dV + (size_t)a_index[k] * ns; b[k] = dV + (size_t)b_index[k] * ns; }
    PLM_HIP(plm_launch_dots(npairs, a, b, n, P.scratch, dout, nullptr));
    PLM_HIP(hipDeviceSynchronize());
    PLM_TRY(P.download(out, dout, (size_t)npairs));
    return PLM_OK;
}

int plm_lbfgs_lincomb(int64_t n, float ca, const float *a, float cb, const float *b, int device, float *out) {
    if (!a || !out) return fail(PLM_EINVAL, "NULL argument");
    PLM_TRY(lbfgs_probe_length(n));
    PLM_TRY(check_device(device));
    LbfgsProbe P;
    float *da, *db = nullptr, *dout;
    PLM_TRY(P.upload(&da, a, (size_t)n));
    if (b) PLM_TRY(P.upload(&db, b, (size_t)n));
    PLM_TRY(P.nan_out(&dout, (size_t)n));
    PLM_HIP(plm_launch_lincomb(dout, ca, da, cb, db, n, nullptr));
    PLM_HIP(hipDeviceSynchronize());
    PLM_TRY(P.download(out, dout, (size_t)n));
    return PLM_OK;
}

int plm_ctx_precond_diagonal(plm_ctx_t *c, float *canonical_out) {
    if (!c || !canonical_out) return fail(PLM_EINVAL, "NULL argument");
    if (c->d.nshards != 1 || c->d.sharded) return fail(PLM_EINVAL, "the H0 diagonal is returned for single-shard contexts only");
    if (c->h_fi.empty()) return fail(PLM_EINVAL, "the H0 diagonal needs single-site frequencies: run marginals first");
    PLM_HIP(hipSetDevice(c->device));
    PLM_TRY(ctx_build_dinv(c));
    return get_vec(c, c->dinv, canonical_out);
}

int plm_ctx_time_kernels(plm_ctx_t *c, int32_t reps, float *out_ms) {
    if (!c || !out_ms || reps <= 0) return fail(PLM_EINVAL, "bad argument");
    if (!c->have_weights) return fail(PLM_EINVAL, "weights not set");
    if (c->d.nshards > 1 && !c->d.sharded) return fail(PLM_EUNSUPPORTED, "kernel timing runs on 1-shard or sharded-state contexts");
    PLM_HIP(hipSetDevice(c->device));
    c->eval_valid = false;
    ctx_set_accurate(c, false);
    const PlmDims &d = c->d;
    struct Events {
        hipEvent_t e[6] = {nullptr, nullptr, nullptr, nullptr, nullptr, nullptr};
        ~Events() { for (auto &x : e) if (x) (void)hipEventDestroy(x); }
    } evs;
    hipEvent_t (&ev)[6] = evs.e;
    for (auto &e : ev) PLM_HIP(hipEventCreate(&e));
    double acc[PLM_K_COUNT] = {0};
    const bool vp = vp_enabled(c);
    if (vp) PLM_TRY(vp_alloc(c));
    for (int r = 0; r < reps; r++) {
        float ms;
        PLM_HIP(hipEventRecord(ev[0], c->st));
        if (d.sharded) {
            PLM_HIP(plm_launch_maxabs2(c->x + d.nh_pad_l, d.n_local - d.nh_pad_l, c->xhalo,
                                       d.nx_halo * (int64_t)PLM_BLOCK_FLOATS(d), c->maxbits, c->jexp, d.jexp_bias, c->st));
            PLM_HIP(plm_launch_expand(d, c->x, c->xhalo, c->jexp, c->Bt, c->fwd_accurate ? 1 : 0, c->st));
        } else {
            PLM_HIP(plm_launch_maxabs(d, c->x, c->maxbits, c->jexp, c->st));
            PLM_HIP(plm_launch_expand(d, c->x, nullptr, c->jexp, c->Bt, c->fwd_accurate ? 1 : 0, c->st));
        }
        PLM_HIP(hipEventRecord(ev[1], c->st));
        if (vp) {
            PLM_HIP(plm_launch_forward_store(d, c->msa_rm, c->Bt, c->jexp, c->hj, 0, c->st));
            PLM_HIP(hipEventRecord(ev[2], c->st));
            PLM_TRY(vp_step_and_residuals(c, r == 0));
            PLM_HIP(hipEventRecord(ev[5], c->st));
        } else {
            PLM_TRY(forward_at_x(c));
            PLM_HIP(hipEventRecord(ev[2], c->st));
            PLM_HIP(hipEventRecord(ev[5], c->st));
        }
        if (d.nblk_own > 0 || !d.sharded) PLM_HIP(plm_launch_backward(d, c->msa_cm, c->Rt, c->G, nullptr, c->st));
        PLM_HIP(hipEventRecord(ev[3], c->st));
        if (d.sharded) PLM_HIP(plm_launch_pack_g(d, c->G, c->gsend, c->st));
        PLM_HIP(plm_launch_assemble(d, c->G, d.ksplit, d.sharded ? c->ghalo : nullptr, c->x, c->g, c->prob.lambda_h, c->prob.lambda_j,
                                    c->reg_part, vp ? 2 : 0, 0.f, nullptr, 0.f, c->st));
        PLM_HIP(plm_launch_finish_fx(d, c->fx_part, c->n_fx_part(), nullptr, 0, c->reg_part, plm_reg_parts(d),
                                     c->scal, c->st));
        PLM_HIP(hipEventRecord(ev[4], c->st));
        PLM_HIP(hipEventSynchronize(ev[4]));
        PLM_HIP(hipEventElapsedTime(&ms, ev[0], ev[1])); acc[PLM_K_EXPAND] += ms;
        PLM_HIP(hipEventElapsedTime(&ms, ev[1], ev[2])); acc[PLM_K_FORWARD] += ms;
        PLM_HIP(hipEventElapsedTime(&ms, ev[2], ev[5])); acc[PLM_K_FIELDS] += ms;
        PLM_HIP(hipEventElapsedTime(&ms, ev[5], ev[3])); acc[PLM_K_BACKWARD] += ms;
        PLM_HIP(hipEventElapsedTime(&ms, ev[3], ev[4])); acc[PLM_K_ASSEMBLE] += ms;
        PLM_HIP(hipEventElapsedTime(&ms, ev[0], ev[4])); acc[PLM_K_TOTAL] += ms;
    }
    {
        const int m = 6;
        PLM_TRY(ctx_alloc_lbfgs(c, m));
        const int64_t n = d.n_local;
        float *S = c->hist, *Y = c->hist + (size_t)m * n;
        PlmVecList Qv, B;
        PlmCoefList C;
        Qv.n = 3; Qv.v[0] = S; Qv.v[1] = Y; Qv.v[2] = c->g;
        B.n = 0;
        for (int i = 0; i < m; i++) B.v[B.n++] = S + (size_t)i * n;
        for (int i = 0; i < m; i++) B.v[B.n++] = Y + (size_t)i * n;
        B.v[B.n++] = c->g;
        B.v[B.n++] = c->g;
        for (int i = 0; i < B.n; i++) C.c[i] = 0.f;
        PLM_HIP(hipMemsetAsync(c->hist, 0, sizeof(float) * 2 * (size_t)m * n, c->st));
        PLM_HIP(hipMemsetAsync(c->dir, 0, sizeof(float) * n, c->st));
        PLM_HIP(hipMemcpyAsync(c->xp, c->x, sizeof(float) * n, hipMemcpyDeviceToDevice, c->st));
        PLM_HIP(hipMemcpyAsync(c->gp, c->g, sizeof(float) * n, hipMemcpyDeviceToDevice, c->st));
        PLM_HIP(hipEventRecord(ev[0], c->st));
        for (int r = 0; r < reps; r++) {
            PLM_HIP(plm_launch_sy_multidot(S, Y, c->x, c->xp, c->g, c->gp, c->dir, B, n, d.nh_pad_l, c->dot_scratch, c->scal + 8,
                                           c->scal + 2, nullptr, 6u, 0ull, c->st));
            B.n -= 1;
            PLM_HIP(plm_launch_multiaxpy_trial(c->dir, B, C, n, nullptr, m, c->xp, 0.f, c->x, c->st));
            B.n += 1;
        }
        PLM_HIP(hipEventRecord(ev[1], c->st));
        PLM_HIP(hipEventSynchronize(ev[1]));
        float ms;
        PLM_HIP(hipEventElapsedTime(&ms, ev[0], ev[1]));
        acc[PLM_K_LBFGS_VECTOR] = ms;
        PLM_HIP(hipMemsetAsync(c->hist, 0, sizeof(float) * 2 * (size_t)m * n, c->st));
    }
    if (vp && !d.sharded) {
        float ms;
        PLM_HIP(plm_launch_expand(d, c->x, nullptr, c->jexp, c->Bt, 1, c->st));
        PLM_HIP(hipEventRecord(ev[0], c->st));
        for (int r = 0; r < reps; r++) PLM_HIP(plm_launch_forward_store(d, c->msa_rm, c->Bt, c->jexp, c->hj, 1, c->st));
        PLM_HIP(hipEventRecord(ev[1], c->st));
        PLM_HIP(hipEventSynchronize(ev[1]));
        PLM_HIP(hipEventElapsedTime(&ms, ev[0], ev[1]));
        acc[PLM_K_FORWARD_ACCURATE] = ms;
    }
    {
        const int thresh = cluster_threshold(c->prob.theta_id, d.L, d.conv);
        PLM_HIP(hipEventRecord(ev[0], c->st));
        PLM_HIP(plm_launch_reweight(d, c->msa_rm, std::max(1, thresh), c->counts, c->st));
        PLM_HIP(hipEventRecord(ev[1], c->st));
        PLM_HIP(hipEventSynchronize(ev[1]));
        float ms;
        PLM_HIP(hipEventElapsedTime(&ms, ev[0], ev[1]));
        acc[PLM_K_REWEIGHT] = ms * reps;
    }
    for (int k = 0; k < PLM_K_COUNT; k++) out_ms[k] = (float)(acc[k] / reps);
    return PLM_OK;
}

int plm_ctx_solver_stats(plm_ctx_t *c, double *out) {
    if (!c || !out) return fail(PLM_EINVAL, "NULL argument");
    out[PLM_S_EVALS] = c->stat_field_evals;
    out[PLM_S_FIELD_MS] = c->stat_field_ms;
    out[PLM_S_PASSES] = c->stat_passes;
    out[PLM_S_CHAIN_SHORT] = c->stat_chain_short;
    out[PLM_S_GEMM_EVALS] = c->stat_gemm_evals;
    out[PLM_S_FWD_MS] = c->stat_fwd_ms;
    out[PLM_S_BWD_MS] = c->stat_bwd_ms;
    return PLM_OK;
}

static plm_problem_t basic_problem(const int8_t *msa, int n, int l, int q) {
    plm_problem_t p;
    memset(&p, 0, sizeof p);
    p.n_seqs = n; p.n_sites = l; p.n_states = q; p.msa = msa;
    p.theta_id = 0.8; p.scale = 1.0; p.n_shards = 1;
    return p;
}

int plm_reweight(const int8_t *msa, int32_t n_seqs, int32_t n_sites, double theta_id, int32_t *counts_out) {
    return plm_reweight_ex(msa, n_seqs, n_sites, theta_id, 0, counts_out);
}

int plm_reweight_ex(const int8_t *msa, int32_t n_seqs, int32_t n_sites, double theta_id, int32_t flags,
                    int32_t *counts_out) {
    if (!msa || !counts_out) return fail(PLM_EINVAL, "NULL argument");
    for (size_t k = 0; k < (size_t)n_seqs * n_sites; k++)
        if (msa[k] < 0 || msa[k] > 126) return fail(PLM_EINVAL, "msa[%zu] outside 0..126", k);
    plm_problem_t p = basic_problem(msa, n_seqs, n_sites, 21);
    p.theta_id = theta_id;
    p.flags = flags & (PLM_FLAG_IGNORE_GAPS | PLM_CONV_MASK);
    PLM_TRY(check_device(0));
    PlmDims d;
    PLM_TRY(make_dims(p, plm_options_from_env(), &d));
    const std::vector<int8_t> rm = padded_rows(d, msa);
    int8_t *dev = nullptr;
    int32_t *cnt = nullptr;
    DeviceBuffers mem;
    PLM_TRY(mem.alloc(&dev, rm.size()));
    PLM_TRY(mem.alloc(&cnt, (size_t)d.Np));
    const int thresh = cluster_threshold(theta_id, d.L, d.conv);
    PLM_HIP(hipMemcpy(dev, rm.data(), rm.size(), hipMemcpyHostToDevice));
    if (thresh > 0) {
        PLM_HIP(plm_launch_reweight(d, dev, thresh, cnt, nullptr));
        PLM_HIP(hipMemcpy(counts_out, cnt, sizeof(int32_t) * d.N, hipMemcpyDeviceToHost));
    } else {
        std::fill(counts_out, counts_out + d.N, d.N);
    }
    return PLM_OK;
// ... 300 lines not shown
```

### evcouplings_amd/csrc/plm_internal.h

```cpp
#pragma once
#include <stdint.h>
#include <stddef.h>
#include <hip/hip_runtime.h>

#define PLM_MAX_SHARDS 16
#define PLM_PAD_STATE 127
#define PLM_SEQ_TILE 256
#define PLM_R_EXP 14
#define PLM_BWD_MAXPLANES 4
#define PLM_R_QMAX3 8355000.0f
#define PLM_R_QMAX4 2138000000.0f
#define PLM_BWD_KSTEP 128
#define PLM_BWDW_COLS 9
#define PLM_BWD_ONEHOT_VALUE (-128)

#define PLM_FWD_NG(Q) (((Q) + 2) / 4)
#define PLM_FWD_SPU(Q) (4 * PLM_FWD_NG(Q))
#define PLM_FWD_TILES(Q) (5 * PLM_FWD_NG(Q))

struct PlmDims {
    int N, L, Q;
    int Qc;
    int Np;
    int nb16;
    int Lp16;
    int nu;
    int Lp32;
    int nksteps;
    int nssteps;
    int nst128;
    int nplanes;
    float rscale;
    float gscale;
    int nstiles;
    int FM, FN;
    int nmf;
    int nshards, shard;
    int blk_per_shard;
    int shard_base, shard_rem;
    int b16_lo, b16_hi;
    int nnfl;
    int ksplit;
    int nrow_tiles, ncol_tiles;
    int fwd_w;
    int bwd_w;
    int64_t nbp;
    int64_t nh_pad;
    int64_t n_native;
    int64_t n_canon;
    int gap_mode;
    int jexp_bias;
    int conv;
    double theta;
    int sharded;
    int own_lo, own_hi;
    int nblk_own;
    int h_site0;
    int64_t bp_base;
    int64_t np_own;
    int64_t nh_pad_l;
    int64_t n_local;
    int64_t nx_halo;
    int64_t ng_halo;
    int ntri;
    int own_base[PLM_MAX_SHARDS], oth_base[PLM_MAX_SHARDS];
};

struct PlmOptions {
    int bwd_planes = 0;
    int ksplit = 0;
    int fwd_kernel = -1;
    int bwd_kernel = -1;
    int jexp_bias = 0;
    int fwd_mode = -1;
    double acc_factor = 8.0;
    double vp_rel = 1e-4;
    int vp_hess_pos = -1;
    double vp_floor = 2e-7;
    bool debug = false;
    bool debug_vp = false;
};
PlmOptions plm_options_from_env();

static inline __host__ __device__ int plm_shard_lo(const PlmDims &d, int r) {
    const int small = d.nshards - d.shard_rem;
    return r * d.shard_base + (r > small ? r - small : 0);
}
static inline __host__ __device__ int plm_shard_cnt(const PlmDims &d, int r) {
    return d.shard_base + (r >= d.nshards - d.shard_rem ? 1 : 0);
}
static inline __host__ __device__ int plm_shard_of(const PlmDims &d, int b) {
    const int small = d.nshards - d.shard_rem, nsmall = small * d.shard_base;
    if (b < nsmall) return d.shard_base > 0 ? b / d.shard_base : 0;
    return small + (b - nsmall) / (d.shard_base + 1);
}
static inline __host__ __device__ int64_t plm_bp_index(int I, int J, int nb16) {
    return (int64_t)I * nb16 - (int64_t)I * (I - 1) / 2 + (J - I);
}
static inline __host__ __device__ int plm_pair_owner(const PlmDims &d, int I, int sI, int sJ) {
    return ((I - plm_shard_lo(d, sI)) & 1) ? sJ : sI;
}
static inline __host__ __device__ int64_t plm_half_blocks(const PlmDims &d, int p) {
    return d.shard < p ? (int64_t)((d.nblk_own + 1) / 2) * plm_shard_cnt(d, p) : (int64_t)(plm_shard_cnt(d, p) / 2) * d.nblk_own;
}
static inline __host__ __device__ int64_t plm_pair_local(const PlmDims &d, int I, int J, int *halo) {
    if (halo) *halo = -1;
    if (!d.sharded) return plm_bp_index(I, J, d.nb16);
    const int sI = plm_shard_of(d, I), sJ = plm_shard_of(d, J);
    if (sI == d.shard && sJ == d.shard) {
        const int r = I - d.own_lo;
        return (int64_t)r * d.nblk_own - (int64_t)r * (r - 1) / 2 + (J - I);
    }
    if (sI != d.shard && sJ != d.shard) return -1;
    const int p = sI == d.shard ? sJ : sI;
    const int idx = ((I - plm_shard_lo(d, sI)) >> 1) * plm_shard_cnt(d, sJ) + (J - plm_shard_lo(d, sJ));
    if (plm_pair_owner(d, I, sI, sJ) == d.shard) return (int64_t)d.ntri + d.own_base[p] + idx;
    if (halo) *halo = d.oth_base[p] + idx;
    return -1;
}
static inline __host__ __device__ void plm_half_pair(const PlmDims &d, int p, bool mine, int64_t k, int *I, int *J) {
    const int np = plm_shard_cnt(d, p);
    if (d.shard < p) {
        *I = d.own_lo + 2 * (int)(k / np) + (mine ? 0 : 1);
        *J = plm_shard_lo(d, p) + (int)(k % np);
    } else {
        *I = plm_shard_lo(d, p) + 2 * (int)(k / d.nblk_own) + (mine ? 1 : 0);
        *J = d.own_lo + (int)(k % d.nblk_own);
    }
}
static inline __host__ __device__ void plm_pair_of_local(const PlmDims &d, int64_t k, int *I, int *J) {
    if (k < d.ntri) {
        int r = 0;
        while (k >= d.nblk_own - r) { k -= d.nblk_own - r; r++; }
        *I = d.own_lo + r;
        *J = d.own_lo + r + (int)k;
        return;
    }
    k -= d.ntri;
    for (int p = 0; p < d.nshards; p++) {
        if (p == d.shard) continue;
        const int64_t n = plm_half_blocks(d, p);
        if (k < n) {
            plm_half_pair(d, p, true, k, I, J);
            return;
        }
        k -= n;
    }
    *I = *J = 0;
}
static inline __host__ __device__ int64_t plm_pair_index(int i, int j, int L) {
    return (int64_t)i * (2 * L - i - 1) / 2 + (j - i - 1);
}

hipError_t plm_launch_reweight(const PlmDims &d, const int8_t *msa_rm, int thresh, int32_t *counts,
                               hipStream_t st);
hipError_t plm_launch_onehot_rt(const PlmDims &d, const int8_t *msa_rm, const float *w, void *Rt,
                                hipStream_t st);
hipError_t plm_launch_maxabs(const PlmDims &d, const float *x, uint32_t *maxbits, int32_t *jexp,
                             hipStream_t st);
hipError_t plm_launch_expand(const PlmDims &d, const float *x, const float *xhalo, const int32_t *jexp,
                             void *Bt, int exact, hipStream_t st);
hipError_t plm_launch_forward_energy(const PlmDims &d, const int8_t *msa_rm, const void *Bt, const float *x,
                                     const int32_t *jexp, int potentials, int accurate, float *out, hipStream_t st);
hipError_t plm_launch_energy_sum(const PlmDims &d, const float *part, double *out, hipStream_t st);
hipError_t plm_launch_forward_store(const PlmDims &d, const int8_t *msa_rm, const void *Bt, const int32_t *jexp,
                                    float *hj, int exact, hipStream_t st);
int plm_fwd_groups(int q, int exact);
hipError_t plm_launch_hpass(const PlmDims &d, const float *hj, const int8_t *msa_rm, const float *w,
                            const double *h64, int write_rt, int stats, int exact, void *Rt, double *fx_part, float *hpart,
                            double *gpart, double *dpart, const int *state, int cond, hipStream_t st);
#define PLM_VP_HIST 24
#define PLM_VP_MAXBLK 256
struct PlmVpState {
    int done;
    int want_rt;
    int final_skip;
    int passes;
    int cur;
    int pad_;
    double g2_prev;
    double g2_prev2;
    double hist[PLM_VP_HIST];
    int hist_loud[PLM_VP_HIST];
    unsigned char quiet[PLM_VP_MAXBLK];
};
#define PLM_VP_ALWAYS 0
#define PLM_VP_PASS 1
#define PLM_VP_PASS_RT 2
#define PLM_VP_FINAL 3
hipError_t plm_launch_vp_reset(int *state, int want_rt, double *zero3, hipStream_t st);
struct PlmRccl;
int plm_rccl_id(void *id128);
int plm_rccl_version();
int plm_rccl_init(const void *id128, int nranks, int rank, PlmRccl **out);
void plm_rccl_destroy(PlmRccl *p);
int plm_rccl_collective(PlmRccl *p, int op, void *send, void *recv, const int64_t *scounts, const int64_t *rcounts,
                        hipStream_t st);
const char *plm_rccl_error();
hipError_t plm_launch_h64_init(const PlmDims &d, const float *x, double *h64, hipStream_t st);
hipError_t plm_launch_hsolve(const PlmDims &d, const float *hpart, const double *gpart, int full, float *x, double *h64,
                             double lambda_h, int update, double *hinv, double *g2_site, double *g2_out, double tol2,
                             double floor2, int *state, int chain, const double *cnt, const double *dpart, hipStream_t st);
hipError_t plm_launch_site_counts(const PlmDims &d, const int8_t *msa_cm, const float *w, double *cnt, hipStream_t st);
size_t plm_h64_stride(const PlmDims &d);
hipError_t plm_launch_fields_to_x(const PlmDims &d, const double *h64, const int *state, float *x, hipStream_t st);
size_t plm_hj_bytes(const PlmDims &d);
size_t plm_hpart_bytes(const PlmDims &d);
size_t plm_gpart_bytes(const PlmDims &d);
hipError_t plm_launch_backward(const PlmDims &d, const int8_t *msa_cm, const void *Rt, int32_t *G, const int *run,
                               hipStream_t st);
hipError_t plm_launch_slab_reduce(const PlmDims &d, const int32_t *G, float *slab, hipStream_t st);
hipError_t plm_launch_assemble(const PlmDims &d, const void *G, int ks_count, const float *ghalo,
                               const float *x, float *g, float lambda_h, float lambda_j, double *reg_part,
                               int mode, float inv_neff, const float *pair_n2, float lambda_g, hipStream_t st);
hipError_t plm_launch_pair_norms(const PlmDims &d, const float *x, float *n2, hipStream_t st);
#define PLM_BLOCK_FLOATS(d) ((size_t)(d).Q * (d).Q * 256)
hipError_t plm_launch_pack_g(const PlmDims &d, const int32_t *G, float *sendbuf, hipStream_t st);
hipError_t plm_launch_maxabs2(const float *a, int64_t na, const float *b, int64_t nb, uint32_t *maxbits,
                              int32_t *jexp, int jexp_bias, hipStream_t st);
hipError_t plm_launch_finish_fx(const PlmDims &d, const double *fx_part, int n_fx_part,
                                const double *shard_nll, int n_shard_nll, const double *reg_part,
                                int n_reg_part, double *out2 , hipStream_t st);
hipError_t plm_launch_partial_sum(const double *part, int n, double *out, hipStream_t st);
#define PLM_DOT_BLOCKS 1024
hipError_t plm_launch_dots(int npairs, const float *const *a, const float *const *b, int64_t n,
                           double *scratch, double *out, hipStream_t st);
hipError_t plm_launch_lincomb(float *out, float ca, const float *a, float cb, const float *b,
                              int64_t n, hipStream_t st);
hipError_t plm_launch_canon_to_native(const PlmDims &d, const float *xc, float *xn, hipStream_t st);
hipError_t plm_launch_native_to_canon(const PlmDims &d, const float *xn, float *xc, hipStream_t st);
hipError_t plm_launch_fn(const PlmDims &d, const float *jij_canon, float *fn, int a_lo, int g_lo, hipStream_t st);
hipError_t plm_launch_msa_columns(const PlmDims &d, const int8_t *msa_rm, int8_t *msa_cm, int cm_rows, hipStream_t st);
hipError_t plm_launch_compact_gap_blocks(const PlmDims &d, const float *blocks, float *out, hipStream_t st);
hipError_t plm_launch_gap_normalise_pairs(const PlmDims &d, float *fij_canon, double fixed_total, hipStream_t st);
hipError_t plm_launch_align_stats(const int8_t *msa, int n, int L, int gap_state, const int8_t *query, int32_t *seq_gaps,
                                  int32_t *col_gaps, int32_t *ident, hipStream_t st);
size_t plm_bt_bytes(const PlmDims &d);
size_t plm_rt_bytes(const PlmDims &d);
size_t plm_g_bytes(const PlmDims &d);
size_t plm_slab_bytes(const PlmDims &d);
int plm_reg_parts(const PlmDims &d);
bool plm_q_supported(int q);
int plm_q_template(int q);
void plm_pick_tile(int q, int *fm, int *fn);

#define PLM_MAX_BASIS 42
struct PlmVecList {
    const float *v[PLM_MAX_BASIS];
    int n;
};
hipError_t plm_launch_multidot(const PlmVecList &queries, const PlmVecList &basis, int64_t n, double *scratch,
                               double *out, const float *dinv, unsigned wq, unsigned long long wb, hipStream_t st);
struct PlmCoefList {
    float c[PLM_MAX_BASIS];
};
hipError_t plm_launch_multiaxpy(float *out, const PlmVecList &basis, const PlmCoefList &coef, int64_t n,
                                const float *dinv, int first_weighted, hipStream_t st);
hipError_t plm_launch_precond(const PlmDims &d, const float *fv, float neff, float lambda_h, float lambda_j, float *dinv,
                              hipStream_t st);
hipError_t plm_launch_sy_multidot(float *s_new, float *y_new, const float *x, const float *xp, const float *g, const float *gp,
                                  const float *dir, const PlmVecList &basis, int64_t n, int64_t nh, double *scratch,
                                  double *out_md, double *out_ex, const float *dinv, unsigned wq, unsigned long long wb,
                                  hipStream_t st);
hipError_t plm_launch_multiaxpy_trial(float *out, const PlmVecList &basis, const PlmCoefList &coef, int64_t n,
                                      const float *dinv, int first_weighted, const float *xacc, float stp, float *trial,
                                      hipStream_t st);
```

### evcouplings_amd/csrc/plm_kernels.hip

```cpp
#include "../../include/plm_hip.h"
#include "plm_internal.h"
#include <math.h>
#include <stdlib.h>
#include <string.h>
#include <mutex>
#include <utility>

typedef _Float16 half8 __attribute__((ext_vector_type(8)));
typedef _Float16 half4 __attribute__((ext_vector_type(4)));
typedef _Float16 half16 __attribute__((ext_vector_type(16)));
typedef float f32x4 __attribute__((ext_vector_type(4)));
typedef int i32x4 __attribute__((ext_vector_type(4)));
typedef unsigned int u32;

#ifndef PLM_DMA_STAGGER_FWD
#define PLM_DMA_STAGGER_FWD 4
#endif
#ifndef PLM_DMA_STAGGER_BWD
#define PLM_DMA_STAGGER_BWD 0
#endif
typedef unsigned long long u64;
#ifndef PLM_ASYNC_A
#define PLM_ASYNC_A 1
#endif
// ... 352 lines not shown
    return hipGetLastError();
}

__global__ __launch_bounds__(256) void k_msa_columns(PlmDims d, const int8_t *__restrict__ rm, int8_t *__restrict__ cm,
                                                    int cm_rows) {
    __shared__ int8_t tile[64][65];
    const int s0 = blockIdx.x * 64, i0 = blockIdx.y * 64;
    const int tx = threadIdx.x & 63, ty = threadIdx.x >> 6;
    const int ones_row = d.nb16 * 16;
#pragma unroll
    for (int k = 0; k < 16; k++) {
        const int s = s0 + ty * 16 + k, i = i0 + tx;
        int8_t v = (int8_t)PLM_PAD_STATE;
        if (s < d.Np && i < d.Lp32) v = rm[(size_t)s * d.Lp32 + i];
        if (i == ones_row) v = s < d.N ? (int8_t)0 : (int8_t)PLM_PAD_STATE;
        tile[ty * 16 + k][tx] = v;
    }
    __syncthreads();
#pragma unroll
    for (int k = 0; k < 16; k++) {
        const int i = i0 + ty * 16 + k, s = s0 + tx;
        if (i < cm_rows && s < d.Np) cm[(size_t)i * d.Np + s] = tile[tx][ty * 16 + k];
    }
}
hipError_t plm_launch_msa_columns(const PlmDims &d, const int8_t *msa_rm, int8_t *msa_cm, int cm_rows, hipStream_t st) {
    hipLaunchKernelGGL(k_msa_columns, dim3((d.Np + 63) / 64, (cm_rows + 63) / 64), dim3(256), 0, st, d, msa_rm, msa_cm, cm_rows);
    return hipGetLastError();
}

__global__ __launch_bounds__(256) void k_onehot_rt(PlmDims d, const int8_t *__restrict__ msa_rm,
                                                  const float *__restrict__ w, char *__restrict__ Rt) {
    const int s64 = blockIdx.x, b16l = blockIdx.y, b16 = d.b16_lo + b16l;
    for (int idx = threadIdx.x; idx < d.Q * 64; idx += 256) {
        const int a = idx >> 6, lane = idx & 63, kg = lane >> 4, ii = lane & 15;
        const int i = b16 * 16 + ii;
        u32 pw[PLM_BWD_MAXPLANES][4];
        const bool four = d.nplanes == 4;
#pragma unroll
        for (int q4 = 0; q4 < 4; q4++) {
            u32 x[4];
#pragma unroll
            for (int e = 0; e < 4; e++) {
                const int s = s64 * 64 + kg * 16 + q4 * 4 + e;
                float v = 0.f;
                if (i < d.L && b16 < d.nb16 && msa_rm[(size_t)s * d.Lp32 + i] == a) v = w[s] * d.rscale;
                x[e] = digits_of(v, four);
            }
            u32 pl[PLM_BWD_MAXPLANES];
            planes_of4(x[0], x[1], x[2], x[3], pl);
#pragma unroll
            for (int p = 0; p < PLM_BWD_MAXPLANES; p++) pw[p][q4] = pl[p];
        }
#pragma unroll
        for (int p = 0; p < PLM_BWD_MAXPLANES; p++)
            if (p < d.nplanes)
                *(uint4 *)(Rt + rt_slot(d, p, s64, b16l * d.Q + a, lane)) = make_uint4(pw[p][0], pw[p][1], pw[p][2], pw[p][3]);
    }
}
hipError_t plm_launch_onehot_rt(const PlmDims &d, const int8_t *msa_rm, const float *w, void *Rt,
                                hipStream_t st) {
    if (d.b16_hi <= d.b16_lo) return hipSuccess;
    hipLaunchKernelGGL(k_onehot_rt, dim3(2 * d.nst128, d.b16_hi - d.b16_lo), dim3(256), 0, st, d, msa_rm, w, (char *)Rt);
    return hipGetLastError();
}

__global__ __launch_bounds__(256) void k_maxabs(const float *__restrict__ x, int64_t n, u32 *maxbits) {
    u32 m = 0;
    const uint4 *x4 = (const uint4 *)x;
    for (int64_t i = (int64_t)blockIdx.x * 256 + threadIdx.x; i < n / 4; i += (int64_t)gridDim.x * 256) {
        const uint4 v = x4[i];
        m = max(max(m, v.x & 0x7fffffffu), max(max(v.y & 0x7fffffffu, v.z & 0x7fffffffu), v.w & 0x7fffffffu));
    }
    for (int64_t i = (n / 4) * 4 + (int64_t)blockIdx.x * 256 + threadIdx.x; i < n; i += (int64_t)gridDim.x * 256)
        m = max(m, __float_as_uint(x[i]) & 0x7fffffffu);
    for (int o = 32; o > 0; o >>= 1) m = max(m, (u32)__shfl_down((int)m, o, 64));
    __shared__ u32 wmax[4];
    if ((threadIdx.x & 63) == 0) wmax[threadIdx.x >> 6] = m;
    __syncthreads();
    if (threadIdx.x == 0) {
        const u32 t = max(max(wmax[0], wmax[1]), max(wmax[2], wmax[3]));
        if (t) atomicMax(maxbits, t);
    }
}
__global__ void k_scale_from_max(const u32 *maxbits, int32_t *jexp, int bias) {
    const float mx = __uint_as_float(*maxbits);
    int e = 0;
    if (mx > 0.f && mx < INFINITY) frexpf(mx, &e);
    int s = PLM_R_EXP - e + bias;
    s = max(-100, min(100, s));
    *jexp = (mx > 0.f) ? s : 0;
}
hipError_t plm_launch_maxabs2(const float *a, int64_t na, const float *b, int64_t nb, u32 *maxbits, int32_t *jexp,
                              int jexp_bias, hipStream_t st) {
    hipError_t e = hipMemsetAsync(maxbits, 0, sizeof(u32), st);
    if (e != hipSuccess) return e;
    if (na > 0) hipLaunchKernelGGL(k_maxabs, dim3((unsigned)std::min<int64_t>(512, (na / 4 + 255) / 256 + 1)), dim3(256), 0, st, a, na, maxbits);
    if (nb > 0) hipLaunchKernelGGL(k_maxabs, dim3((unsigned)std::min<int64_t>(256, (nb / 4 + 255) / 256 + 1)), dim3(256), 0, st, b, nb, maxbits);
    hipLaunchKernelGGL(k_scale_from_max, dim3(1), dim3(1), 0, st, maxbits, jexp, jexp_bias);
    return hipGetLastError();
}
hipError_t plm_launch_maxabs(const PlmDims &d, const float *x, u32 *maxbits, int32_t *jexp, hipStream_t st) {
    hipError_t e = hipMemsetAsync(maxbits, 0, sizeof(u32), st);
    if (e != hipSuccess) return e;
    const int64_t n = d.n_local - d.nh_pad_l;
    hipLaunchKernelGGL(k_maxabs, dim3((unsigned)std::min<int64_t>(512, (n / 4 + 255) / 256 + 1)), dim3(256), 0, st, x + d.nh_pad_l, n, maxbits);
    hipLaunchKernelGGL(k_scale_from_max, dim3(1), dim3(1), 0, st, maxbits, jexp, d.jexp_bias);
    return hipGetLastError();
}

__device__ __forceinline__ float load_coupling(const PlmDims &d, const float *__restrict__ xj,
                                               const float *__restrict__ xhalo, int I, int ii, int a, int J, int jj,
                                               int b) {
    const int QQ = d.Q * d.Q;
    if (I == J) {
        if (ii == jj) return 0.f;
        const float *blk = xj + (size_t)plm_pair_local(d, I, I, nullptr) * QQ * 256;
        return ii < jj ? blk[(a * d.Q + b) * 256 + ii * 16 + jj] : blk[(b * d.Q + a) * 256 + jj * 16 + ii];
    }
    int h;
    const int64_t k = plm_pair_local(d, min(I, J), max(I, J), &h);
    const float *blk = k >= 0 ? xj + (size_t)k * QQ * 256 : xhalo + (size_t)h * QQ * 256;
    return I < J ? blk[(a * d.Q + b) * 256 + ii * 16 + jj] : blk[(b * d.Q + a) * 256 + jj * 16 + ii];
}
__global__ __launch_bounds__(64) void k_fwd_ref(PlmDims d, const float *__restrict__ x, const float *__restrict__ xhalo,
                                               float *__restrict__ cref, double *__restrict__ cref64) {
    const int b16l = blockIdx.x, b16 = d.b16_lo + b16l, r = blockIdx.y, a = blockIdx.z, t = threadIdx.x;
    const int i = b16 * 16 + r;
    const float *__restrict__ xj = x + d.nh_pad_l;
    double s = 0;
    if (!d.gap_mode && i < d.L)
        for (int j = t; j < d.L; j += 64)
            if (j != i) s += (double)load_coupling(d, xj, xhalo, b16, r, a, j >> 4, j & 15, 0);
    for (int o = 32; o > 0; o >>= 1) s += __shfl_down(s, o, 64);
    if (t == 0) {
        cref[((size_t)b16l * 16 + r) * d.Q + a] = (float)s;
        cref64[((size_t)b16l * 16 + r) * d.Q + a] = s;
    }
}
__global__ __launch_bounds__(256) void k_expand(PlmDims d, const float *__restrict__ x,
                                               const float *__restrict__ xhalo,
                                               const int32_t *__restrict__ jexp, _Float16 *__restrict__ Bt) {
    const int NG = PLM_FWD_NG(d.Q), SPU = 4 * NG;
    const int u = blockIdx.x / (2 * NG), ci = blockIdx.x % (2 * NG), b16l = blockIdx.y, b16 = d.b16_lo + b16l;
    const float sc = ldexpf(1.f, *jexp);
    const float *__restrict__ xj = x + d.nh_pad_l;
    _Float16 *tile_hi = Bt + ((size_t)b16l * d.nu * SPU + (size_t)u * SPU + 2 * ci) * (size_t)(2 * d.Q * 512);
    _Float16 *tile_lo = tile_hi + (size_t)(2 * d.Q * 512);
    for (int idx = blockIdx.z * 256 + threadIdx.x; idx < d.Q * 64; idx += gridDim.z * 256) {
        const int a = idx >> 6, lane = idx & 63, gb = lane >> 4, r = lane & 15;
        const int i = b16 * 16 + r;
#pragma unroll
        for (int half = 0; half < 2; half++) {
            half8 hi, lo;
#pragma unroll
            for (int e8 = 0; e8 < 8; e8++) {
                const int ga = 2 * half + (gb >> 1), pp = 2 * (gb & 1) + (e8 >> 2), e = e8 & 3;
                const int gl = 4 * ci + pp, s8 = gl & 7, sg = gl >> 3;
                const int b = 4 * sg + e + 1, j = 32 * u + 8 * ga + s8;
                float v = 0.f;
                if (b < d.Q && i < d.L && j < d.L && i != j) {
                    v = load_coupling(d, xj, xhalo, b16, r, a, j >> 4, j & 15, b);
                    if (!d.gap_mode) v -= load_coupling(d, xj, xhalo, b16, r, a, j >> 4, j & 15, 0);
                    v *= sc;
                }
                const _Float16 h = (_Float16)v;
                hi[e8] = h;
                lo[e8] = (_Float16)(v - (float)h);
            }
            *(half8 *)(tile_hi + (size_t)(half * d.Q + a) * 512 + lane * 8) = hi;
            *(half8 *)(tile_lo + (size_t)(half * d.Q + a) * 512 + lane * 8) = lo;
        }
    }
}

#define PLM_FWDX_PLANES 5
#define PLM_FWDX_SHIFT 23
__global__ __launch_bounds__(256) void k_expand_x(PlmDims d, const float *__restrict__ x,
                                                 const float *__restrict__ xhalo,
                                                 const int32_t *__restrict__ jexp, char *__restrict__ Bt) {
    const int NG = PLM_FWD_NG(d.Q);
    const int u = blockIdx.x / NG, grp = blockIdx.x % NG, b16l = blockIdx.y, b16 = d.b16_lo + b16l;
    const double sc = ldexp(1.0, *jexp + PLM_FWDX_SHIFT);
    const float *__restrict__ xj = x + d.nh_pad_l;
    const size_t tile = (size_t)2 * d.Q * 1024, plane_stride = (size_t)d.nu * NG * tile;
    char *t0 = Bt + (size_t)b16l * PLM_FWDX_PLANES * plane_stride + ((size_t)u * NG + grp) * tile;
    for (int idx = threadIdx.x; idx < 2 * d.Q * 64; idx += 256) {
        const int h16 = idx / (d.Q * 64), rem = idx - h16 * d.Q * 64;
        const int a = rem >> 6, lane = rem & 63, kg = lane >> 4, r = lane & 15;
        const int i = b16 * 16 + r;
        u32 w[PLM_FWDX_PLANES][4];
#pragma unroll
        for (int e = 0; e < 4; e++) {
            u32 dig[4], top = 0;
#pragma unroll
            for (int t = 0; t < 4; t++) {
                const int b = 4 * grp + 1 + e, j = 32 * u + 8 * kg + 4 * h16 + t;
                double v = 0.0;
                if (b < d.Q && i < d.L && j < d.L && i != j) {
                    const float jb = load_coupling(d, xj, xhalo, b16, r, a, j >> 4, j & 15, b);
                    const float j0 = d.gap_mode ? 0.f : load_coupling(d, xj, xhalo, b16, r, a, j >> 4, j & 15, 0);
                    v = ((double)jb - (double)j0) * sc;
                }
                const long long R = llrint(v);
                const u64 dg = ((u64)R + 0x8080808080ull) ^ 0x8080808080ull;
                dig[t] = (u32)dg;
                top |= (u32)((dg >> 32) & 0xffu) << (8 * t);
            }
            u32 pl[PLM_BWD_MAXPLANES];
            planes_of4(dig[0], dig[1], dig[2], dig[3], pl);
#pragma unroll
            for (int p = 0; p < 4; p++) w[p][e] = pl[p];
            w[4][e] = top;
        }
#pragma unroll
        for (int p = 0; p < PLM_FWDX_PLANES; p++)
            *(uint4 *)(t0 + (size_t)p * plane_stride + (size_t)(h16 * d.Q + a) * 1024 + lane * 16) =
                make_uint4(w[p][0], w[p][1], w[p][2], w[p][3]);
    }
}
hipError_t plm_launch_expand(const PlmDims &d, const float *x, const float *xhalo, const int32_t *jexp, void *Bt,
                             int exact, hipStream_t st) {
    if (d.b16_hi <= d.b16_lo) return hipSuccess;
    const int NG = PLM_FWD_NG(d.Q);
    if (exact)
        hipLaunchKernelGGL(k_expand_x, dim3(d.nu * NG, d.b16_hi - d.b16_lo), dim3(256), 0, st, d, x, xhalo, jexp, (char *)Bt);
    else
        hipLaunchKernelGGL(k_expand, dim3(d.nu * 2 * NG, d.b16_hi - d.b16_lo, (d.Q * 64 + 255) / 256), dim3(256), 0, st, d, x, xhalo,
                           jexp, (_Float16 *)Bt);
    hipLaunchKernelGGL(k_fwd_ref, dim3(d.b16_hi - d.b16_lo, 16, d.Q), dim3(64), 0, st, d, x, xhalo,
                       (float *)bt_cref32(d, Bt), (double *)bt_cref64(d, Bt));
    return hipGetLastError();
}

struct FwdArgs {
    const int8_t *msa_rm;
    const char *Bt;
    const float *h;
    const int32_t *jexp;
    float *out;
};
enum { FWD_ENERGY = 1, FWD_POTENTIALS = 2, FWD_STORE = 3 };

template <int QG, int A>
__device__ __forceinline__ void fwd_state(f32x4 (&acc)[2][QG], const half8 &a0, const half8 &a1, int i0, int i1, u32 lb,
                                          half8 (&bh)[3], half8 (&bl)[3], const DmaPlan &dma) {
    constexpr int NP = (2 * QG + 7) / 8;
    if constexpr (A + 2 < QG) {
        bh[(A + 2) % 3] = lds_read_b128<(A + 2) * 1024>(lb);
        bl[(A + 2) % 3] = lds_read_b128<(QG + A + 2) * 1024>(lb);
    }
    constexpr int newer = (A + 2 < QG) ? 4 : (A + 1 < QG) ? 2 : 0;
    lds_wait<newer>(bh[A % 3], bl[A % 3]);
    const half16 bb = __builtin_shufflevector(bh[A % 3], bl[A % 3], 0, 1, 2, 3, 4, 5, 6, 7, 8, 9, 10, 11, 12, 13, 14, 15);
    acc[0][A] = __builtin_amdgcn_smfmac_f32_16x16x64_f16(a0, bb, acc[0][A], i0, 0, 0);
    dma_at<QG, A, NP, PLM_DMA_STAGGER_FWD>(dma);
    acc[1][A] = __builtin_amdgcn_smfmac_f32_16x16x64_f16(a1, bb, acc[1][A], i1, 0, 0);
}
template <int QG, int... A>
__device__ __forceinline__ void fwd_kstep(f32x4 (&acc)[2][QG], const half8 &a0, const half8 &a1, int i0, int i1, u32 lb,
                                          half8 (&bh)[3], half8 (&bl)[3], const DmaPlan &dma,
                                          std::integer_sequence<int, A...>) {
    bh[0] = lds_read_b128<0>(lb);
    bl[0] = lds_read_b128<QG * 1024>(lb);
    if constexpr (QG > 1) {
        bh[1] = lds_read_b128<1024>(lb);
        bl[1] = lds_read_b128<(QG + 1) * 1024>(lb);
    }
    (fwd_state<QG, A>(acc, a0, a1, i0, i1, lb, bh, bl, dma), ...);
}

template <int Q, int MODE, int NSG>
__global__ __launch_bounds__(512) void k_fwd(PlmDims d, FwdArgs A) {
    static_assert(Q % NSG == 0, "state groups must divide the alphabet");
    extern __shared__ __attribute__((aligned(16))) char smem[];
    constexpr int QG = Q / NSG;
    constexpr int TILE_G = 2 * Q * 1024, TILE = 2 * QG * 1024, NP = (2 * QG + 7) / 8;
    const int tid = threadIdx.x, lane = tid & 63, wave = tid >> 6;
    const int wave_s = __builtin_amdgcn_readfirstlane(wave);
    const int nwork = d.nstiles * (d.b16_hi - d.b16_lo) * NSG, per_xcd = (nwork + 7) >> 3;
    const int wk = (int)(blockIdx.x & 7) * per_xcd + (int)(blockIdx.x >> 3);
    if ((int)(blockIdx.x >> 3) >= per_xcd || wk >= nwork) return;
    const int stile = wk % d.nstiles, sg = (wk / d.nstiles) % NSG, b16l = wk / (d.nstiles * NSG);
    const int tile = b16l * d.nstiles + stile;
    const int a_lo = sg * QG;
    const int b16 = d.b16_lo + b16l;
    const int r = lane & 15, g = lane >> 4;
    const int s_wave = stile * PLM_SEQ_TILE + wave * 32;
    constexpr int NG = PLM_FWD_NG(Q), SPU = 4 * NG;
    const int nsteps = d.nu * SPU;
    const char *bt = A.Bt + (size_t)b16l * nsteps * TILE_G + (size_t)a_lo * 1024;
    const u32 arow0 = (u32)(s_wave + r) * (u32)d.Lp32 + 8 * g, arow1 = arow0 + 16 * (u32)d.Lp32;

    f32x4 acc[2][QG];
#pragma unroll
    for (int a = 0; a < QG; a++) {
        acc[0][a] = (f32x4){0.f, 0.f, 0.f, 0.f};
        acc[1][a] = (f32x4){0.f, 0.f, 0.f, 0.f};
    }
#if PLM_PROBE
    unsigned long long pr_wait = 0;
    const unsigned long long pr_t0 = PROBE_NOW();
#endif
    if (nsteps > 0) {
        const DmaPlan first{bt, smem, wave_s, 2 * QG, (u32)lane * 16, false, nullptr, 0, nullptr, QG, (Q - QG) * 1024};
        dma_issue_all<NP>(first);
    }
    u64 na0 = *(const u64 *)(A.msa_rm + arow0), na1 = *(const u64 *)(A.msa_rm + arow1);
    half8 bh[3], bl[3];
// ... 1869 lines not shown
                if (i0 + j * 256 < nfx) s += v[j];
        }
    }
    const double nll = block_reduce_sum(s, red);
    __syncthreads();
    double rsum = 0;
    for (int i0 = threadIdx.x; i0 < nreg; i0 += 8 * 256) {
        double v[8];
#pragma unroll
        for (int j = 0; j < 8; j++) v[j] = reg_part[min(i0 + j * 256, nreg - 1)];
#pragma unroll
        for (int j = 0; j < 8; j++)
            if (i0 + j * 256 < nreg) rsum += v[j];
    }
    const double reg = block_reduce_sum(rsum, red);
    if (threadIdx.x == 0) {
        out2[0] = nll + reg;
        out2[1] = nll;
    }
}
hipError_t plm_launch_partial_sum(const double *part, int n, double *out, hipStream_t st) {
    hipLaunchKernelGGL(k_sum_partials, dim3(1), dim3(256), 0, st, part, n, out);
    return hipGetLastError();
}
hipError_t plm_launch_finish_fx(const PlmDims &d, const double *fx_part, int n_fx_part, const double *shard_nll,
                                int n_shard_nll, const double *reg_part, int n_reg_part, double *out2,
                                hipStream_t st) {
    hipLaunchKernelGGL(k_finish_fx, dim3(1), dim3(256), 0, st, fx_part, n_fx_part, shard_nll,
                       plm_slab_bytes(d), n_shard_nll, reg_part, n_reg_part, out2);
    return hipGetLastError();
}

struct DotArgs {
    const float *a[4];
    const float *b[4];
};
template <int NP>
__global__ __launch_bounds__(256) void k_dots(DotArgs A, int64_t n4, double *__restrict__ scratch) {
    __shared__ double red[4];
    double s[NP];
#pragma unroll
    for (int p = 0; p < NP; p++) s[p] = 0;
    for (int64_t i = (int64_t)blockIdx.x * 256 + threadIdx.x; i < n4; i += (int64_t)gridDim.x * 256) {
#pragma unroll
        for (int p = 0; p < NP; p++) {
            const float4 u = ((const float4 *)A.a[p])[i], v = ((const float4 *)A.b[p])[i];
            s[p] += (double)u.x * v.x + (double)u.y * v.y + (double)u.z * v.z + (double)u.w * v.w;
        }
    }
#pragma unroll
    for (int p = 0; p < NP; p++) {
        const double t = block_reduce_sum(s[p], red);
        if (threadIdx.x == 0) scratch[(size_t)p * PLM_DOT_BLOCKS + blockIdx.x] = t;
        __syncthreads();
    }
}
__global__ __launch_bounds__(256) void k_dots_final(const double *__restrict__ scratch, double *out) {
    __shared__ double red[4];
    double s = 0;
    for (int i = threadIdx.x; i < PLM_DOT_BLOCKS; i += 256) s += scratch[(size_t)blockIdx.x * PLM_DOT_BLOCKS + i];
    const double t = block_reduce_sum(s, red);
    if (threadIdx.x == 0) out[blockIdx.x] = t;
}
hipError_t plm_launch_dots(int npairs, const float *const *a, const float *const *b, int64_t n, double *scratch,
                           double *out, hipStream_t st) {
    if (npairs < 1 || npairs > 4 || (n & 3)) return hipErrorInvalidValue;
    DotArgs A;
    for (int p = 0; p < 4; p++) {
        A.a[p] = a[p < npairs ? p : 0];
        A.b[p] = b[p < npairs ? p : 0];
    }
    const int64_t n4 = n / 4;
    switch (npairs) {
    case 1: hipLaunchKernelGGL(k_dots<1>, dim3(PLM_DOT_BLOCKS), dim3(256), 0, st, A, n4, scratch); break;
    case 2: hipLaunchKernelGGL(k_dots<2>, dim3(PLM_DOT_BLOCKS), dim3(256), 0, st, A, n4, scratch); break;
    case 3: hipLaunchKernelGGL(k_dots<3>, dim3(PLM_DOT_BLOCKS), dim3(256), 0, st, A, n4, scratch); break;
    default: hipLaunchKernelGGL(k_dots<4>, dim3(PLM_DOT_BLOCKS), dim3(256), 0, st, A, n4, scratch); break;
    }
    hipLaunchKernelGGL(k_dots_final, dim3(npairs), dim3(256), 0, st, scratch, out);
    return hipGetLastError();
}

__global__ __launch_bounds__(256) void k_lincomb(float4 *__restrict__ out, float ca, const float4 *__restrict__ a,
                                                float cb, const float4 *__restrict__ b, int64_t n4) {
    for (int64_t i = (int64_t)blockIdx.x * 256 + threadIdx.x; i < n4; i += (int64_t)gridDim.x * 256) {
        const float4 u = a[i];
        float4 r;
        if (b) {
            const float4 v = b[i];
            r.x = fmaf(cb, v.x, ca * u.x); r.y = fmaf(cb, v.y, ca * u.y);
            r.z = fmaf(cb, v.z, ca * u.z); r.w = fmaf(cb, v.w, ca * u.w);
        } else {
            r.x = ca * u.x; r.y = ca * u.y; r.z = ca * u.z; r.w = ca * u.w;
        }
        out[i] = r;
    }
}
hipError_t plm_launch_lincomb(float *out, float ca, const float *a, float cb, const float *b, int64_t n,
                              hipStream_t st) {
    if (n & 3) return hipErrorInvalidValue;
    hipLaunchKernelGGL(k_lincomb, dim3(2048), dim3(256), 0, st, (float4 *)out, ca, (const float4 *)a, cb,
                       (const float4 *)b, n / 4);
    return hipGetLastError();
}

__global__ __launch_bounds__(256) void k_canon_to_native(PlmDims d, const float *__restrict__ xc,
                                                        float *__restrict__ xn) {
    const int a = blockIdx.y;
    int I, J;
    plm_pair_of_local(d, blockIdx.x, &I, &J);
    const int ii = threadIdx.x >> 4, jj = threadIdx.x & 15;
    const int i = I * 16 + ii, j = J * 16 + jj;
    const bool valid = i < d.L && j < d.L && i < j && a < d.Qc;
    const size_t QQc = (size_t)d.Qc * d.Qc;
    const size_t src = valid ? (size_t)d.L * d.Qc + (size_t)plm_pair_index(i, j, d.L) * QQc + (size_t)a * d.Qc : 0;
    const size_t dst = d.nh_pad_l + ((size_t)blockIdx.x * d.Q + a) * d.Q * 256 + threadIdx.x;
    for (int b = 0; b < d.Q; b++) xn[dst + (size_t)b * 256] = (valid && b < d.Qc) ? xc[src + b] : 0.f;
}
__global__ __launch_bounds__(256) void k_copy_h(PlmDims d, const float *__restrict__ src, float *__restrict__ dst,
                                               int to_native) {
    const int nsites = min(d.L, d.own_hi * 16) - d.h_site0;
    const int64_t n = to_native ? d.nh_pad_l : (int64_t)nsites * d.Qc;
    for (int64_t k = (int64_t)blockIdx.x * 256 + threadIdx.x; k < n; k += (int64_t)gridDim.x * 256) {
        if (to_native) {
            const int64_t il = k / d.Q;
            const int a = (int)(k % d.Q);
            dst[k] = (il < nsites && a < d.Qc) ? src[(size_t)(d.h_site0 + il) * d.Qc + a] : 0.f;
        } else {
            const int64_t il = k / d.Qc;
            const int a = (int)(k % d.Qc);
            dst[(size_t)(d.h_site0 + il) * d.Qc + a] = src[(size_t)il * d.Q + a];
        }
    }
}
__global__ __launch_bounds__(64) void k_native_to_canon(PlmDims d, const float *__restrict__ xn,
                                                       float *__restrict__ xc) {
    const int i = blockIdx.x, j = blockIdx.y;
    if (j <= i) return;
    const int I = i >> 4, J = j >> 4;
    const int64_t k = plm_pair_local(d, I, J, nullptr);
    if (k < 0) return;
    const int QQc = d.Qc * d.Qc;
    const size_t src = d.nh_pad_l + (size_t)k * d.Q * d.Q * 256 + (i & 15) * 16 + (j & 15);
    const size_t dst = (size_t)d.L * d.Qc + (size_t)plm_pair_index(i, j, d.L) * QQc;
    for (int ab = threadIdx.x; ab < QQc; ab += 64)
        xc[dst + ab] = xn[src + (size_t)((ab / d.Qc) * d.Q + ab % d.Qc) * 256];
}
hipError_t plm_launch_canon_to_native(const PlmDims &d, const float *xc, float *xn, hipStream_t st) {
    hipLaunchKernelGGL(k_copy_h, dim3(64), dim3(256), 0, st, d, xc, xn, 1);
    if (d.np_own > 0)
        hipLaunchKernelGGL(k_canon_to_native, dim3((unsigned)d.np_own, d.Q), dim3(256), 0, st, d, xc, xn);
    return hipGetLastError();
}
hipError_t plm_launch_native_to_canon(const PlmDims &d, const float *xn, float *xc, hipStream_t st) {
    hipLaunchKernelGGL(k_copy_h, dim3(64), dim3(256), 0, st, d, xn, xc, 0);
    hipLaunchKernelGGL(k_native_to_canon, dim3(d.L, d.L), dim3(64), 0, st, d, xn, xc);
    return hipGetLastError();
}

__global__ __launch_bounds__(64) void k_fn(int L, int Q, const float *__restrict__ jij, float *__restrict__ fn,
                                          int a_lo, int g_lo) {
    __shared__ float blk[32 * 32];
    __shared__ double rm[32], cm[32];
    __shared__ double red[1];
    const int i = blockIdx.x, j = blockIdx.y;
    if (j <= i) {
        if (threadIdx.x == 0 && j == i) fn[(size_t)i * L + i] = 0.f;
        return;
    }
    const int QQ = Q * Q, Qm = Q - g_lo;
    const float *src = jij + (size_t)plm_pair_index(i, j, L) * QQ;
    for (int k = threadIdx.x; k < QQ; k += 64) blk[k] = src[k];
    __syncthreads();
    if (threadIdx.x < Q) {
        double r = 0, c = 0;
        for (int k = g_lo; k < Q; k++) {
            r += blk[threadIdx.x * Q + k];
            c += blk[k * Q + threadIdx.x];
        }
        rm[threadIdx.x] = r / Qm;
        cm[threadIdx.x] = c / Qm;
    }
    __syncthreads();
    double m = 0;
    for (int k = g_lo; k < Q; k++) m += rm[k];
    m /= Qm;
// ... 158 lines not shown
    if (p >= d.nshards) return;
    int I, J;
    plm_half_pair(d, p, false, k, &I, &J);
    const int lane = threadIdx.x & 63, wave = threadIdx.x >> 6;
    const size_t dst = (((size_t)blockIdx.x * d.Q + a) * d.Q) * 256 + 4 * lane;
    const size_t kstride = (size_t)d.nmf * d.nnfl * 256;
    for (int b = wave; b < d.Q; b += 4) {
        const size_t o = (d.shard < p ? g_frag(d, d.ksplit, 0, I, a, J * d.Q + b) : g_frag(d, d.ksplit, 0, J, b, I * d.Q + a)) + 4 * lane;
        float v[4];
        g_combine4(G, o, d.ksplit, kstride, d.nplanes, v);
        *(float4 *)(out + dst + (size_t)b * 256) = make_float4(v[0], v[1], v[2], v[3]);
    }
}
hipError_t plm_launch_pack_g(const PlmDims &d, const int32_t *G, float *sendbuf, hipStream_t st) {
    if (d.nblk_own <= 0 || d.nx_halo <= 0) return hipSuccess;
    hipLaunchKernelGGL(k_pack_g, dim3((unsigned)d.nx_halo, d.Q), dim3(256), 0, st, d, (const int *)G, sendbuf);
    return hipGetLastError();
}

#ifndef MD_CHUNK
#define MD_CHUNK 14
#endif
template <int NQ>
__global__ __launch_bounds__(256) void k_multidot(PlmVecList Q, PlmVecList B, int64_t n4, double *__restrict__ scratch,
                                                 const float4 *__restrict__ dinv, unsigned wq, unsigned long long wb) {
    __shared__ double red[4];
    const int nb = B.n, k0 = blockIdx.y * MD_CHUNK;
    const float4 *bp[MD_CHUNK];
#pragma unroll
    for (int k = 0; k < MD_CHUNK; k++) bp[k] = (const float4 *)B.v[min(k0 + k, nb - 1)];
    const unsigned wbc = (unsigned)(wb >> k0) & ((1u << MD_CHUNK) - 1u);
    const bool any_w = dinv != nullptr && wq != 0 && wbc != 0;
    double acc[NQ][MD_CHUNK];
#pragma unroll
    for (int q = 0; q < NQ; q++)
#pragma unroll
        for (int k = 0; k < MD_CHUNK; k++) acc[q][k] = 0;
    for (int64_t i = (int64_t)blockIdx.x * 256 + threadIdx.x; i < n4; i += (int64_t)gridDim.x * 256) {
        float4 qv[NQ], qd[NQ];
#pragma unroll
        for (int q = 0; q < NQ; q++) qd[q] = qv[q] = ((const float4 *)Q.v[q])[i];
        if (any_w) {
            const float4 dv = dinv[i];
#pragma unroll
            for (int q = 0; q < NQ; q++)
                if ((wq >> q) & 1u) { qd[q].x *= dv.x; qd[q].y *= dv.y; qd[q].z *= dv.z; qd[q].w *= dv.w; }
        }
#pragma unroll
        for (int k = 0; k < MD_CHUNK; k++) {
            const float4 b = bp[k][i];
            const bool wk = (wbc >> k) & 1u;
#pragma unroll
            for (int q = 0; q < NQ; q++) {
                const float4 a = wk ? qd[q] : qv[q];
                acc[q][k] += (double)a.x * b.x + (double)a.y * b.y + (double)a.z * b.z + (double)a.w * b.w;
            }
        }
    }
#pragma unroll
    for (int q = 0; q < NQ; q++)
#pragma unroll
        for (int k = 0; k < MD_CHUNK; k++) {
            const double t = block_reduce_sum(acc[q][k], red);
            if (threadIdx.x == 0 && k0 + k < nb) scratch[((size_t)q * nb + k0 + k) * PLM_DOT_BLOCKS + blockIdx.x] = t;
            __syncthreads();
        }
}
hipError_t plm_launch_multidot(const PlmVecList &queries, const PlmVecList &basis, int64_t n, double *scratch,
                               double *out, const float *dinv, unsigned wq, unsigned long long wb, hipStream_t st) {
    if (queries.n < 1 || queries.n > 4 || basis.n < 1 || basis.n > PLM_MAX_BASIS || (n & 3)) return hipErrorInvalidValue;
    const int64_t n4 = n / 4;
    const dim3 grid(PLM_DOT_BLOCKS, (basis.n + MD_CHUNK - 1) / MD_CHUNK), block(256);
    const float4 *d4 = (const float4 *)dinv;
    switch (queries.n) {
    case 1: hipLaunchKernelGGL(k_multidot<1>, grid, block, 0, st, queries, basis, n4, scratch, d4, wq, wb); break;
    case 2: hipLaunchKernelGGL(k_multidot<2>, grid, block, 0, st, queries, basis, n4, scratch, d4, wq, wb); break;
    case 3: hipLaunchKernelGGL(k_multidot<3>, grid, block, 0, st, queries, basis, n4, scratch, d4, wq, wb); break;
    default: hipLaunchKernelGGL(k_multidot<4>, grid, block, 0, st, queries, basis, n4, scratch, d4, wq, wb); break;
    }
    hipLaunchKernelGGL(k_dots_final, dim3(queries.n * basis.n), dim3(256), 0, st, scratch, out);
    return hipGetLastError();
}

__global__ __launch_bounds__(256) void k_multiaxpy(float4 *__restrict__ out, PlmVecList B, PlmCoefList C, int64_t n4,
                                                  const float4 *__restrict__ dinv, int kw,
                                                  const float4 *__restrict__ xacc, float stp, float4 *__restrict__ trial) {
    const int nb = B.n;
    for (int64_t i = (int64_t)blockIdx.x * 256 + threadIdx.x; i < n4; i += (int64_t)gridDim.x * 256) {
        float4 r = {0.f, 0.f, 0.f, 0.f}, t = {0.f, 0.f, 0.f, 0.f};
#pragma unroll 4
        for (int k = 0; k < kw; k++) {
            const float4 b = ((const float4 *)B.v[k])[i];
            const float c = C.c[k];
            r.x = fmaf(c, b.x, r.x); r.y = fmaf(c, b.y, r.y); r.z = fmaf(c, b.z, r.z); r.w = fmaf(c, b.w, r.w);
        }
#pragma unroll 4
        for (int k = kw; k < nb; k++) {
            const float4 b = ((const float4 *)B.v[k])[i];
            const float c = C.c[k];
            t.x = fmaf(c, b.x, t.x); t.y = fmaf(c, b.y, t.y); t.z = fmaf(c, b.z, t.z); t.w = fmaf(c, b.w, t.w);
        }
        if (dinv) {
            const float4 dv = dinv[i];
            r.x = fmaf(dv.x, t.x, r.x); r.y = fmaf(dv.y, t.y, r.y); r.z = fmaf(dv.z, t.z, r.z); r.w = fmaf(dv.w, t.w, r.w);
        } else {
            r.x += t.x; r.y += t.y; r.z += t.z; r.w += t.w;
        }
        out[i] = r;
        if (trial) {
            const float4 u = xacc[i];
            trial[i] = make_float4(fmaf(stp, r.x, 1.f * u.x), fmaf(stp, r.y, 1.f * u.y), fmaf(stp, r.z, 1.f * u.z),
                                   fmaf(stp, r.w, 1.f * u.w));
        }
    }
}
hipError_t plm_launch_multiaxpy(float *out, const PlmVecList &basis, const PlmCoefList &coef, int64_t n,
                                const float *dinv, int first_weighted, hipStream_t st) {
    if (basis.n < 1 || basis.n > PLM_MAX_BASIS || (n & 3)) return hipErrorInvalidValue;
    const int kw = dinv ? std::max(0, std::min(basis.n, first_weighted)) : basis.n;
    hipLaunchKernelGGL(k_multiaxpy, dim3(2048), dim3(256), 0, st, (float4 *)out, basis, coef, n / 4,
                       (const float4 *)dinv, kw, (const float4 *)nullptr, 0.f, (float4 *)nullptr);
    return hipGetLastError();
}
hipError_t plm_launch_multiaxpy_trial(float *out, const PlmVecList &basis, const PlmCoefList &coef, int64_t n,
                                      const float *dinv, int first_weighted, const float *xacc, float stp, float *trial,
                                      hipStream_t st) {
    if (basis.n < 1 || basis.n > PLM_MAX_BASIS || (n & 3) || !xacc || !trial) return hipErrorInvalidValue;
    const int kw = dinv ? std::max(0, std::min(basis.n, first_weighted)) : basis.n;
    hipLaunchKernelGGL(k_multiaxpy, dim3(2048), dim3(256), 0, st, (float4 *)out, basis, coef, n / 4,
                       (const float4 *)dinv, kw, (const float4 *)xacc, stp, (float4 *)trial);
    return hipGetLastError();
}

#define SYD_OLD 10
struct PlmSyDot {
    const float4 *x, *xp, *g, *gp, *dir, *dinv;
    float4 *s_new, *y_new;
    const float4 *old[PLM_MAX_BASIS];
    int pos[PLM_MAX_BASIS];
    int n_old, nb, pos_s, pos_y, pos_g0, pos_g1;
    unsigned wq;
    unsigned long long wb;
    int64_t n4, nh4;
};
__device__ __forceinline__ double dot4(const float4 &a, const float4 &b) {
    return (double)a.x * b.x + (double)a.y * b.y + (double)a.z * b.z + (double)a.w * b.w;
}
__global__ __launch_bounds__(256) void k_sy_multidot(PlmSyDot A, double *__restrict__ scratch) {
    __shared__ double red[4];
    const int k0 = blockIdx.y * SYD_OLD;
    const bool first = blockIdx.y == 0;
    const float4 *bp[SYD_OLD];
    unsigned wold = 0;
#pragma unroll
    for (int k = 0; k < SYD_OLD; k++) {
        const int kk = min(k0 + k, max(A.n_old - 1, 0));
        bp[k] = A.n_old > 0 ? A.old[kk] : A.g;
        if (A.n_old > 0 && ((A.wb >> A.pos[kk]) & 1ull)) wold |= 1u << k;
    }
    const int spos[4] = {A.pos_s, A.pos_y, A.pos_g0, A.pos_g1};
    bool wsp[4];
#pragma unroll
    for (int e = 0; e < 4; e++) wsp[e] = spos[e] >= 0 && ((A.wb >> spos[e]) & 1ull);
    const bool any_w = A.dinv != nullptr && A.wq != 0;
    double acc[3][SYD_OLD], sp[3][4], ex[3] = {0, 0, 0}, ssh = 0;
#pragma unroll
    for (int q = 0; q < 3; q++) {
#pragma unroll
        for (int k = 0; k < SYD_OLD; k++) acc[q][k] = 0;
#pragma unroll
        for (int e = 0; e < 4; e++) sp[q][e] = 0;
    }
    for (int64_t i = (int64_t)blockIdx.x * 256 + threadIdx.x; i < A.n4; i += (int64_t)gridDim.x * 256) {
        const float4 xv = A.x[i], xpv = A.xp[i], gv = A.g[i], gpv = A.gp[i];
        float4 qv[3], qd[3];
        qv[0] = make_float4(xv.x - xpv.x, xv.y - xpv.y, xv.z - xpv.z, xv.w - xpv.w);
        qv[1] = make_float4(gv.x - gpv.x, gv.y - gpv.y, gv.z - gpv.z, gv.w - gpv.w);
        qv[2] = gv;
        if (first) {
            A.s_new[i] = qv[0];
            A.y_new[i] = qv[1];
        }
#pragma unroll
        for (int q = 0; q < 3; q++) qd[q] = qv[q];
        if (any_w) {
            const float4 dv = A.dinv[i];
#pragma unroll
            for (int q = 0; q < 3; q++)
                if ((A.wq >> q) & 1u) { qd[q].x *= dv.x; qd[q].y *= dv.y; qd[q].z *= dv.z; qd[q].w *= dv.w; }
        }
        if (A.n_old > 0) {
#pragma unroll
            for (int k = 0; k < SYD_OLD; k++) {
                const float4 b = bp[k][i];
                const bool wk = (wold >> k) & 1u;
#pragma unroll
                for (int q = 0; q < 3; q++) acc[q][k] += dot4(wk ? qd[q] : qv[q], b);
            }
        }
        if (first) {
#pragma unroll
            for (int e = 0; e < 4; e++) {
                const float4 b = e == 0 ? qv[0] : e == 1 ? qv[1] : gv;
#pragma unroll
                for (int q = 0; q < 3; q++) sp[q][e] += dot4(wsp[e] ? qd[q] : qv[q], b);
            }
            ex[0] += dot4(gv, A.dir[i]);
            const double x2 = dot4(xv, xv);
            ex[1] += x2;
            if (i < A.nh4) {
                ex[2] += x2;
                ssh += dot4(qv[0], qv[0]);
            }
        }
    }
#pragma unroll
    for (int q = 0; q < 3; q++)
#pragma unroll
        for (int k = 0; k < SYD_OLD; k++) {
            const double t = block_reduce_sum(acc[q][k], red);
            if (threadIdx.x == 0 && k0 + k < A.n_old)
                scratch[((size_t)q * A.nb + A.pos[k0 + k]) * PLM_DOT_BLOCKS + blockIdx.x] = t;
            __syncthreads();
        }
    if (!first) return;
#pragma unroll
    for (int q = 0; q < 3; q++)
#pragma unroll
        for (int e = 0; e < 4; e++) {
            const double t = block_reduce_sum(sp[q][e], red);
            if (threadIdx.x == 0 && spos[e] >= 0) scratch[((size_t)q * A.nb + spos[e]) * PLM_DOT_BLOCKS + blockIdx.x] = t;
            __syncthreads();
        }
    {
        const double t = block_reduce_sum(ssh, red);
        if (threadIdx.x == 0) scratch[((size_t)3 * A.nb) * PLM_DOT_BLOCKS + blockIdx.x] = t;
        __syncthreads();
    }
#pragma unroll
    for (int e = 0; e < 3; e++) {
        const double t = block_reduce_sum(ex[e], red);
        if (threadIdx.x == 0) scratch[((size_t)3 * A.nb + 1 + e) * PLM_DOT_BLOCKS + blockIdx.x] = t;
        __syncthreads();
    }
}
__global__ __launch_bounds__(256) void k_dots_final2(const double *__restrict__ scratch, double *out_a, int na, double *out_b) {
    __shared__ double red[4];
    double s = 0;
    for (int i = threadIdx.x; i < PLM_DOT_BLOCKS; i += 256) s += scratch[(size_t)blockIdx.x * PLM_DOT_BLOCKS + i];
    const double t = block_reduce_sum(s, red);
    if (threadIdx.x == 0) {
        if ((int)blockIdx.x < na) out_a[blockIdx.x] = t;
        else out_b[blockIdx.x - na] = t;
    }
}
hipError_t plm_launch_sy_multidot(float *s_new, float *y_new, const float *x, const float *xp, const float *g, const float *gp,
                                  const float *dir, const PlmVecList &basis, int64_t n, int64_t nh, double *scratch,
                                  double *out_md, double *out_ex, const float *dinv, unsigned wq, unsigned long long wb,
                                  hipStream_t st) {
    if (basis.n < 1 || basis.n > PLM_MAX_BASIS || (n & 3) || (nh & 3) || nh > n) return hipErrorInvalidValue;
    PlmSyDot A;
    memset(&A, 0, sizeof A);
    A.x = (const float4 *)x; A.xp = (const float4 *)xp; A.g = (const float4 *)g; A.gp = (const float4 *)gp;
    A.dir = (const float4 *)dir; A.dinv = (const float4 *)dinv;
    A.s_new = (float4 *)s_new; A.y_new = (float4 *)y_new;
    A.nb = basis.n; A.wq = wq; A.wb = wb; A.n4 = n / 4; A.nh4 = nh / 4;
    A.pos_s = A.pos_y = A.pos_g0 = A.pos_g1 = -1;
    for (int k = 0; k < basis.n; k++) {
        const float *v = basis.v[k];
        if (v == s_new && A.pos_s < 0) A.pos_s = k;
        else if (v == y_new && A.pos_y < 0) A.pos_y = k;
        else if (v == g && A.pos_g0 < 0) A.pos_g0 = k;
        else if (v == g && A.pos_g1 < 0) A.pos_g1 = k;
        else { A.old[A.n_old] = (const float4 *)v; A.pos[A.n_old++] = k; }
    }
    const dim3 grid(PLM_DOT_BLOCKS, std::max(1, (A.n_old + SYD_OLD - 1) / SYD_OLD)), block(256);
    hipLaunchKernelGGL(k_sy_multidot, grid, block, 0, st, A, scratch);
    hipLaunchKernelGGL(k_dots_final2, dim3(3 * basis.n + 4), dim3(256), 0, st, scratch, out_md, 3 * basis.n + 1, out_ex);
    return hipGetLastError();
}
```

### evcouplings_amd/plm.py

```python
import ctypes as C

import numpy as np

from evcouplings_amd import _lib
from evcouplings_amd._lib import PlmProblem, PlmResult, check


def _ptr(a):
    return None if a is None else a.ctypes.data_as(C.c_void_p)


def _msa(msa):
    msa = np.ascontiguousarray(msa, dtype=np.int8)
    if msa.ndim != 2:
        raise ValueError("msa must be a 2-D (N, L) int8 matrix")
    return msa


def n_params(L, q):
    return L * q + L * (L - 1) // 2 * q * q


def default_lambda_j(L, q, base=0.01):
    return base * (q - 1) * (L - 1)
# ... 712 lines not shown

def top_combinations(target, q, hi, jij, sites, letters=None, top=100, device=0, max_keep=None, chunk=1 << 24):
    top = int(top)
    if top < 1:
        raise ValueError("top must be >= 1")
    kw = dict(letters=letters, device=device)
    ext = mutant_scan(target, q, hi, jij, sites, **kw)
    total = ext["n_combinations"]
    top = min(top, total)
    max_keep = max(4 * top, 1 << 20) if max_keep is None else max(int(max_keep), top)

    def best(idx, en):
        order = np.lexsort((idx, -en[:, 0]))[:top]
        return idx[order], en[order]

    def compact(thr, expect, first=0, count=None):
        res = mutant_scan(target, q, hi, jij, sites, first=first, count=count, threshold=thr, capacity=max(expect, 1), **kw)
        if res["kept_index"] is None:
            res = mutant_scan(target, q, hi, jij, sites, first=first, count=count, threshold=thr, capacity=res["n_kept"], **kw)
        return res["kept_index"], res["kept_energies"]

    lo, hi_ = ext["dh_min"], ext["dh_max"]
    thr, n_kept = -np.inf, total
    while n_kept > max_keep:
        edges = np.linspace(lo, hi_, _lib.SCAN_MAX_EDGES)
        edges[0], edges[-1] = lo, hi_
        edges = np.maximum.accumulate(np.clip(edges, lo, hi_))
        counts = mutant_scan(target, q, hi, jij, sites, edges=edges, **kw)["histogram"].astype(np.int64)
        tail = counts[::-1].cumsum()[::-1]
        b = int(np.nonzero(tail >= top)[0].max())
        if b == 0:
            break
        thr, n_kept = float(edges[b - 1]), int(tail[b])
        if n_kept <= max_keep:
            break
        if b == edges.size:
            break
        upper = float(edges[b])
        if not np.nextafter(thr, np.inf) < upper or (thr == lo and upper == hi_):
            break
        lo, hi_ = thr, upper
    if n_kept <= max_keep:
        return best(*compact(thr, n_kept))
    idx, en = np.zeros(0, np.int64), np.zeros((0, 3))
    for first in range(0, total, int(chunk)):
        count = min(int(chunk), total - first)
        ci, ce = compact(thr, min(count, max_keep), first, count)
        idx, en = best(np.concatenate([idx, ci]), np.concatenate([en, ce]))
    return idx, en


def _f32(a):
    return None if a is None else np.ascontiguousarray(a, dtype=np.float32)


def _i32(a):
    return np.ascontiguousarray(a, dtype=np.int32)


def _nan(shape, dtype):
    return np.full(shape, np.nan, dtype)


def lbfgs_gram(S, Y, x, xp, g, gp, direction, end, nst, nh, dinv=None, device=0):
    S, Y, x, xp, g, gp, direction, dinv = (_f32(a) for a in (S, Y, x, xp, g, gp, direction, dinv))
    m, n = S.shape
    s_new, y_new = _nan(n, np.float32), _nan(n, np.float32)
    md, ex = _nan(3 * (2 * nst + 2) + 1, np.float64), _nan(3, np.float64)
    check(_lib.load().plm_lbfgs_gram(n, int(nh), m, int(end), int(nst), _ptr(S), _ptr(Y), _ptr(x), _ptr(xp), _ptr(g),
                                     _ptr(gp), _ptr(direction), _ptr(dinv), device, _ptr(s_new), _ptr(y_new), _ptr(md),
                                     _ptr(ex)))
    return s_new, y_new, md, ex


def lbfgs_direction(S, Y, g, cs, cy, cg, stored, end, dinv=None, xacc=None, stp0=0.0, device=0):
    S, Y, g, dinv, xacc = (_f32(a) for a in (S, Y, g, dinv, xacc))
    cs, cy = _f64(cs), _f64(cy)
    m, n = S.shape
    out = _nan(n, np.float32)
    trial = None if xacc is None else _nan(n, np.float32)
    check(_lib.load().plm_lbfgs_direction(n, m, int(stored), int(end), _ptr(S), _ptr(Y), _ptr(g), _ptr(cs), _ptr(cy),
                                          float(cg), _ptr(dinv), _ptr(xacc), float(stp0), device, _ptr(out), _ptr(trial)))
    return out if xacc is None else (out, trial)


def lbfgs_multidot(V, q_index, b_index, dinv=None, wq=0, wb=0, device=0):
    V, dinv, q_index, b_index = _f32(V), _f32(dinv), _i32(q_index), _i32(b_index)
    nv, n = V.shape
    out = _nan((q_index.size, b_index.size), np.float64)
    check(_lib.load().plm_lbfgs_multidot(n, nv, _ptr(V), q_index.size, _ptr(q_index), b_index.size, _ptr(b_index),
                                         _ptr(dinv), int(wq), int(wb), device, _ptr(out)))
    return out


def lbfgs_dots(V, a_index, b_index, n=None, device=0):
    V, a_index, b_index = _f32(V), _i32(a_index), _i32(b_index)
    nv, stride = V.shape
    out = _nan(a_index.size, np.float64)
    check(_lib.load().plm_lbfgs_dots(stride, nv, _ptr(V), a_index.size, _ptr(a_index), _ptr(b_index),
                                     stride if n is None else int(n), device, _ptr(out)))
    return out


def lbfgs_lincomb(ca, a, cb=0.0, b=None, device=0):
    a, b = _f32(a), _f32(b)
    out = _nan(a.size, np.float32)
    check(_lib.load().plm_lbfgs_lincomb(a.size, float(ca), _ptr(a), float(cb), _ptr(b), device, _ptr(out)))
    return out


def linesearch_run(phi, finit, dginit, step0):
    def cfunc(stp, dphi, user):
        f, dphi[0] = phi(stp)
        return f
    code, count, stp = C.c_int32(0), C.c_int32(0), C.c_double(0)
    trace = _nan((_lib.LS_MAX_TRIALS, 3), np.float64)
    check(_lib.load().plm_linesearch_run(_lib.PHI_CB(cfunc), None, float(finit), float(dginit), float(step0),
                                         C.byref(code), C.byref(count), C.byref(stp), _ptr(trace)))
    return code.value, count.value, stp.value, trace[:count.value]


ADMIT_STORED, ADMIT_STRADDLE, ADMIT_SKIPPED, ADMIT_RESTARTED = 0, 1, 2, 3


def lbfgs_admit(state, md, vp=False, straddle=False):
    m = int(state["m"])
    SY, YDY, Sg, YDg = (_f64(state[k]).copy() for k in ("SY", "YDY", "Sg", "YDg"))
    md = _f64(md)
    stored, end, anchored = (C.c_int32(int(state[k])) for k in ("stored", "end", "anchored"))
    gDg, gg = C.c_double(state["gDg"]), C.c_double(state["gg"])
    outcome, copy_anchor = C.c_int32(-1), C.c_int32(-1)
    nst = min(m, stored.value + 1)
    if SY.shape != (m, m) or YDY.shape != (m, m) or Sg.shape != (m,) or YDg.shape != (m,) or md.size != 3 * (2 * nst + 2) + 1:
        raise ValueError("history arrays or md of the wrong shape")
    check(_lib.load().plm_lbfgs_admit(m, C.byref(stored), C.byref(end), C.byref(anchored), _ptr(SY), _ptr(YDY), _ptr(Sg),
                                      _ptr(YDg), C.byref(gDg), C.byref(gg), _ptr(md), 2 * nst + 2, nst, int(bool(vp)),
                                      int(bool(straddle)), C.byref(outcome), C.byref(copy_anchor)))
    new = dict(m=m, stored=stored.value, end=end.value, anchored=bool(anchored.value), SY=SY, YDY=YDY, Sg=Sg, YDg=YDg,
               gDg=gDg.value, gg=gg.value)
    return new, outcome.value, bool(copy_anchor.value)


FLAG_IGNORE_GAPS = 2
FLAG_SHARDED_STATE = 4
FLAG_PRECOND = 8
FLAG_JOINT_LBFGS = 16
FLAG_COMPACT_GAPS = 1024


class _IterationCallback:

    def __init__(self, callback=None):
        self.table, self.callback, self.pending = [], callback, None
        self.cfunc = _lib.ITER_CB(self._call)

    def _call(self, it, secs, cond, fx, nll, nh, ne, user):
        try:
            self.table.append((it, secs, cond, fx, nll, nh, ne))
            if self.callback is not None:
                self.callback(it, secs, cond, fx, nll, nh, ne)
            return 0
        except BaseException as exc:
            self.pending = exc
            return 1

    def reraise(self):
# ... 307 lines not shown
```

### include/plm_hip.h

```cpp
#ifndef PLM_HIP_H
#define PLM_HIP_H

#include <stddef.h>
#include <stdint.h>

#ifdef __cplusplus
extern "C" {
#endif
#pragma GCC visibility push(default)

#define PLM_ABI_VERSION 2

#define PLM_OK 0
#define PLM_EINVAL (-1)
#define PLM_ENOMEM (-2)
#define PLM_EDEVICE (-3)
#define PLM_EUNSUPPORTED (-4)
#define PLM_ENUMERIC (-5)
#define PLM_ECALLBACK (-6)

#define PLM_STATUS_CONVERGED 0
#define PLM_STATUS_MAXITER 1
#define PLM_STATUS_LINESEARCH 2
#define PLM_STATUS_INTERRUPTED 3
// ... 299 lines not shown
int plm_fasta_split(const char *buf, int64_t n, int64_t *n_records, int64_t *seq_bytes, int64_t *hdr_off,
                    int32_t *hdr_len, int64_t *seq_len, char *seq_out);
int plm_encode_columns(const uint8_t *mat, int64_t n_rows, int64_t width, const int64_t *cols, int64_t n_cols,
                       const int8_t *lut256, int8_t *out, uint8_t *valid);
int plm_write_raw_ec_file(const char *path, int32_t n_sites, const int32_t *index_list, const char *target_seq,
                          const double *cn);

int plm_ctx_create(const plm_problem_t *problem, int device, void *stream, plm_ctx_t **out);
void plm_ctx_destroy(plm_ctx_t *ctx);
int plm_ctx_set_exchange(plm_ctx_t *ctx, plm_exchange_cb exchange, void *user);
int plm_ctx_set_collective(plm_ctx_t *ctx, plm_collective_cb collective, void *user);
int plm_ctx_attach_rccl(plm_ctx_t *ctx, const void *rccl_id);
int plm_ctx_set_options(plm_ctx_t *ctx, int32_t max_iter, double epsilon, int32_t lbfgs_m);
int64_t plm_ctx_native_size(const plm_ctx_t *ctx);
int plm_ctx_reweight(plm_ctx_t *ctx);
int plm_ctx_set_weights(plm_ctx_t *ctx, const float *weights_host);
int plm_ctx_get_weights(plm_ctx_t *ctx, float *weights_host, int32_t *counts_host, float *n_eff);
int plm_ctx_marginals(plm_ctx_t *ctx, float *fi_host, float *fij_host);
int plm_ctx_set_x(plm_ctx_t *ctx, const float *x_canonical_host);
int plm_ctx_get_x(plm_ctx_t *ctx, float *x_canonical_host);
int plm_ctx_get_g(plm_ctx_t *ctx, float *g_canonical_host);
int plm_ctx_eval(plm_ctx_t *ctx, double *fx_out, double *nll_out);
int plm_ctx_optimize(plm_ctx_t *ctx, plm_iter_cb cb, void *user, plm_result_t *result);
int plm_ctx_scores(plm_ctx_t *ctx, float *fn_host, float *cn_host);
#define PLM_K_EXPAND 0
#define PLM_K_FORWARD 1
#define PLM_K_BACKWARD 2
#define PLM_K_ASSEMBLE 3
#define PLM_K_TOTAL 4
#define PLM_K_REWEIGHT 5
#define PLM_K_FIELDS 6
#define PLM_K_FORWARD_ACCURATE 7
#define PLM_K_LBFGS_VECTOR 8
#define PLM_K_COUNT 9
int plm_ctx_time_kernels(plm_ctx_t *ctx, int32_t reps, float *out_ms );
int plm_ctx_time_field_positions(plm_ctx_t *ctx, int32_t reps, float *out_ms );
#define PLM_S_EVALS 0
#define PLM_S_FIELD_MS 1
#define PLM_S_PASSES 2
#define PLM_S_CHAIN_SHORT 3
#define PLM_S_GEMM_EVALS 4
#define PLM_S_FWD_MS 5
#define PLM_S_BWD_MS 6
#define PLM_S_COUNT 7
int plm_ctx_solver_stats(plm_ctx_t *ctx, double *out );

#define PLM_FIELD_ROLE_STATS 0
#define PLM_FIELD_ROLE_HESSIAN 1
#define PLM_FIELD_ROLE_RESIDUAL 2
typedef struct {
    double *gpart, *dpart;
    float *hpart;
    double *hcnt, *hinv, *g2_site, *g2_sum, *h64, *nll_part;
    int64_t n_gpart, n_hpart, n_hcnt, n_hinv, n_g2_site, n_h64, n_nll_part;
} plm_field_buffers_t;
int plm_ctx_field_position(plm_ctx_t *ctx, int32_t role, int32_t accurate, int32_t update, int32_t prefill,
                           plm_field_buffers_t *out);
#define PLM_FIELD_HIST 24
#define PLM_FIELD_MAXBLK 256
typedef struct {
    double gh2;
    double fx, nll;
    int32_t passes, done;
    int32_t continuations;
    int32_t final_skip, want_rt, cur, state_passes;
    int32_t c_prev_next;
    double hist[PLM_FIELD_HIST];
    unsigned char quiet[PLM_FIELD_MAXBLK];
} plm_field_solve_t;
int plm_ctx_field_solve(plm_ctx_t *ctx, double tol, int32_t vp_c_prev, int32_t invalidate, int32_t accurate,
                        plm_field_solve_t *result, double *fields, int64_t n_fields);

int plm_lbfgs_gram(int64_t n, int64_t nh, int32_t m, int32_t end, int32_t nst, const float *S, const float *Y,
                   const float *x, const float *xp, const float *g, const float *gp, const float *dir, const float *dinv,
                   int device, float *s_new, float *y_new, double *md, double *ex);
int plm_lbfgs_direction(int64_t n, int32_t m, int32_t stored, int32_t end, const float *S, const float *Y, const float *g,
                        const double *cs, const double *cy, double cg, const float *dinv, const float *xacc, float stp0,
                        int device, float *dir, float *trial);
int plm_lbfgs_multidot(int64_t n, int32_t nv, const float *V, int32_t nq, const int32_t *q_index, int32_t nb,
                       const int32_t *b_index, const float *dinv, uint32_t wq, uint64_t wb, int device, double *out);
int plm_lbfgs_dots(int64_t stride, int32_t nv, const float *V, int32_t npairs, const int32_t *a_index,
                   const int32_t *b_index, int64_t n, int device, double *out);
int plm_lbfgs_lincomb(int64_t n, float ca, const float *a, float cb, const float *b, int device, float *out);
int plm_ctx_precond_diagonal(plm_ctx_t *ctx, float *canonical_out);

void plm_lbfgs_coefficients(int m, int stored, int end, const double *SY, const double *YDY, const double *Sg,
                            const double *YDg, double gDg, double *cs, double *cy, double *cg, double *dg);

#define PLM_LS_MAX_TRIALS 20
typedef double (*plm_phi_cb)(double stp, double *dphi, void *user);
int plm_linesearch_run(plm_phi_cb phi, void *user, double finit, double dginit, double step0, int32_t *code,
                       int32_t *n_trials, double *stp, double *trace);
int plm_lbfgs_admit(int32_t m, int32_t *stored, int32_t *end, int32_t *anchored, double *SY, double *YDY, double *Sg,
                    double *YDg, double *gDg, double *gg, const double *md, int32_t nbv, int32_t nst, int32_t vp,
                    int32_t straddle, int32_t *outcome, int32_t *copy_anchor);

#define PLM_MUT_OK 0
#define PLM_MUT_ETOOMANY 1
#define PLM_MUT_EPOSITION 2
#define PLM_MUT_ESTATE 3
#define PLM_MUT_EREPEAT 4
int plm_mutant_effects(const float *x_canonical, int32_t n_sites, int32_t n_states, const int8_t *target,
                       int64_t n_variants, const int64_t *offsets, int64_t n_entries, const int32_t *positions,
                       const int8_t *states, int device, void *stream, double *out, uint8_t *status,
                       double *tables_out);

#define PLM_SCAN_MAX_SITES 8
#define PLM_SCAN_MAX_EDGES 1024
typedef struct {
    int32_t n_scan_sites;
    int32_t flags;
    const int32_t *sites;
    const int32_t *letter_offsets;
    const int8_t *letters;
    int64_t first, count;
    const double *edges;
    int32_t n_edges;
    int32_t use_threshold;
    double threshold;
    int64_t capacity;
} plm_scan_opts;
typedef struct {
    double *energies;
    uint64_t *histogram;
    int64_t *kept_index;
    double *kept_energies;
    double dh_min, dh_max;
    int64_t n_kept;
    int64_t n_combinations;
} plm_scan_result;
int plm_mutant_scan(const float *x_canonical, int32_t n_sites, int32_t n_states, const int8_t *target,
                    const plm_scan_opts *opts, int device, void *stream, plm_scan_result *result);

#pragma GCC visibility pop
#ifdef __cplusplus
}
#endif
#endif
```

Baseline: 112.9 iterations/s.

## Fuse coupling max-abs scale reduction into trial-point kernels; add transposed expand and templated multidot

The trial-point writers (multiaxpy trial and a new lincomb_scale) now fold a max-abs reduction over the coupling part into their own pass. The last block to finish, found through grouped atomic counters, writes the exponent, so the separate maxabs kernel launch and its full read of x are skipped when x was just produced that way. The change also adds an optional transposed expand kernel behind an environment switch, and templates the S/Y multidot kernel on first/weighted with a software-pipelined load order and launch_bounds(256,2). The risks are atomic contention in the fused reduction, and correctness of the last-block handoff, which relies on relaxed atomics.

After: 112.4 iterations/s. No clear change (-0.4%).

```diff
diff --git a/evcouplings_amd/_lib.py b/evcouplings_amd/_lib.py
--- a/evcouplings_amd/_lib.py
+++ b/evcouplings_amd/_lib.py
@@ -287,6 +287,8 @@
                                      C.c_int, _P]),
     ("plm_lbfgs_dots", C.c_int, [C.c_int64, C.c_int32, _P, C.c_int32, _P, _P, C.c_int64, C.c_int, _P]),
     ("plm_lbfgs_lincomb", C.c_int, [C.c_int64, C.c_float, _P, C.c_float, _P, C.c_int, _P]),
+    ("plm_lbfgs_trial_scale", C.c_int, [C.c_int64, C.c_int64, C.c_int32, C.c_int32, C.c_int32, _P, _P, _P, _P, _P, C.c_double,
+                                        _P, _P, C.c_int32, _P, C.c_int32, C.c_int, _P, _P, _P, C.POINTER(C.c_int32)]),
     ("plm_ctx_precond_diagonal", C.c_int, [_P, _P]),
     ("plm_rccl_probe", C.c_int, [_P, C.c_int32, C.c_int32, C.c_int, _P]),
     ("plm_rccl_probe_local", C.c_int, [C.c_int32, C.c_int, _P]),
diff --git a/evcouplings_amd/csrc/plm_host.cpp b/evcouplings_amd/csrc/plm_host.cpp
--- a/evcouplings_amd/csrc/plm_host.cpp
+++ b/evcouplings_amd/csrc/plm_host.cpp
@@ -76,6 +76,7 @@
     if (const char *e = getenv("PLM_JEXP_BIAS")) o.jexp_bias = atoi(e);
     if (const char *e = getenv("PLM_BWD_KERNEL")) o.bwd_kernel = atoi(e) ? 1 : 0;
     if (const char *e = getenv("PLM_FWD_KERNEL")) o.fwd_kernel = atoi(e) ? 1 : 0;
+    if (const char *e = getenv("PLM_EXPAND_KERNEL")) o.expand_kernel = atoi(e) ? 1 : 0;
     if (const char *e = getenv("PLM_FWD_ACCURATE")) o.fwd_mode = atoi(e) ? 1 : 0;
     if (const char *e = getenv("PLM_VP_FLOOR")) o.vp_floor = atof(e);
     if (const char *e = getenv("PLM_VP_REL")) o.vp_rel = atof(e);
@@ -146,6 +147,7 @@
     d.ncol_tiles = (d.nnfl + 2 * d.FN - 1) / (2 * d.FN);
     d.fwd_w = (d.Q == 21 && opt.fwd_kernel != 0) ? 1 : 0;
     d.bwd_w = (d.Q == 21 && opt.bwd_kernel != 0) ? 1 : 0;
+    d.expand_t = opt.expand_kernel != 0 ? 1 : 0;
     if (d.bwd_w) d.ncol_tiles = (d.nnfl + PLM_BWDW_COLS - 1) / PLM_BWDW_COLS;
     PLM_TRY(pick_ksplit(d, opt, d.nplanes, &d.ksplit));
     d.nbp = (int64_t)d.nb16 * (d.nb16 + 1) / 2;
@@ -214,6 +216,8 @@
     double *fx_part = nullptr, *reg_part = nullptr, *dot_scratch = nullptr, *scal = nullptr;
     uint32_t *maxbits = nullptr;
     int32_t *jexp = nullptr;
+    uint32_t *scale_state = nullptr;
+    const float *jexp_of = nullptr;
     float *x = nullptr, *g = nullptr, *xp = nullptr, *gp = nullptr, *dir = nullptr, *hist = nullptr;
     float *xa = nullptr, *ga = nullptr;
     float *canon = nullptr;
@@ -342,10 +346,22 @@
     return PLM_OK;
 }
 
+int ctx_scale_exponent(plm_ctx *c) {
+    const bool have = c->jexp_of != nullptr && c->jexp_of == c->x;
+    c->jexp_of = nullptr;
+    if (!have) PLM_HIP(plm_launch_maxabs(c->d, c->x, c->maxbits, c->jexp, c->st));
+    return PLM_OK;
+}
+PlmScaleFuse ctx_scale_fuse(plm_ctx *c) {
+    PlmScaleFuse f;
+    if (!c->d.sharded) { f.state = c->scale_state; f.jexp = c->jexp; f.first = c->d.nh_pad_l; f.bias = c->d.jexp_bias; }
+    return f;
+}
+
 int ctx_eval_enqueue(plm_ctx *c) {
     const PlmDims &d = c->d;
     if (d.sharded) return ctx_eval_enqueue_sharded(c);
-    PLM_HIP(plm_launch_maxabs(d, c->x, c->maxbits, c->jexp, c->st));
+    PLM_TRY(ctx_scale_exponent(c));
     PLM_HIP(plm_launch_expand(d, c->x, nullptr, c->jexp, c->Bt, c->fwd_accurate ? 1 : 0, c->st));
     PLM_TRY(forward_at_x(c));
     PLM_HIP(plm_launch_backward(d, c->msa_cm, c->Rt, c->G, nullptr, c->st));
@@ -414,7 +430,7 @@
                                    d.nx_halo * (int64_t)PLM_BLOCK_FLOATS(d), c->maxbits, c->jexp, d.jexp_bias, c->st));
         PLM_HIP(plm_launch_expand(d, c->x, c->xhalo, c->jexp, c->Bt, c->fwd_accurate ? 1 : 0, c->st));
     } else {
-        PLM_HIP(plm_launch_maxabs(d, c->x, c->maxbits, c->jexp, c->st));
+        PLM_TRY(ctx_scale_exponent(c));
         PLM_HIP(plm_launch_expand(d, c->x, nullptr, c->jexp, c->Bt, c->fwd_accurate ? 1 : 0, c->st));
     }
     if (c->gemm_ev[0]) PLM_HIP(hipEventRecord(c->gemm_ev[0], c->st));
@@ -654,7 +670,7 @@
     for (auto &e : c->vp_ev)
         if (e) (void)hipEventDestroy(e);
     void *bufs[] = {c->msa_rm, c->msa_cm, c->w, c->counts, c->Bt, c->Rt, c->G, c->gather, c->fx_part, c->reg_part,
-                    c->dot_scratch, c->scal, c->maxbits, c->jexp, c->x, c->g, c->xp, c->gp, c->dir, c->hist,
+                    c->dot_scratch, c->scal, c->maxbits, c->scale_state, c->jexp, c->x, c->g, c->xp, c->gp, c->dir, c->hist,
                     c->canon, c->xhalo, c->ghalo, c->xsend, c->gsend, c->dinv, c->hj, c->hpart, c->gpart, c->dpart, c->hg2, c->hinv, c->h64, c->hcnt, c->vp_flag,
                     c->xa, c->ga, c->pair_n2};
     for (void *b : bufs)
@@ -726,6 +742,8 @@
     PLM_TRY(plm_dalloc(&c->scal, (size_t)256));
     PLM_TRY(plm_dalloc(&c->maxbits, (size_t)1));
     PLM_TRY(plm_dalloc(&c->jexp, (size_t)1));
+    PLM_TRY(plm_dalloc(&c->scale_state, (size_t)PLM_SCALE_WORDS));
+    PLM_HIP(hipMemset(c->scale_state, 0, sizeof(uint32_t) * PLM_SCALE_WORDS));
     PLM_TRY(plm_dalloc(&c->x, (size_t)d.n_local));
     PLM_TRY(plm_dalloc(&c->g, (size_t)d.n_local));
     PLM_TRY(plm_dalloc(&c->canon, (size_t)d.n_canon + (size_t)d.L * d.L));
@@ -1137,6 +1155,11 @@
     if (precond) PLM_TRY(ctx_build_dinv(c));
     const float *dinv = precond ? c->dinv : nullptr;
     LbfgsHistory hist(m);
+    struct ForgetScale {
+        plm_ctx_t *c;
+        ~ForgetScale() { c->jexp_of = nullptr; }
+    } forget_scale{c};
+    c->jexp_of = nullptr;
     double xx = 0, hh = 0;
     c->n_evals = 0;
     enum { SL_FX = 0, SL_NLL = 1, SL_DG = 2, SL_XX = 3, SL_HH = 4, SL_GH2 = 5, SL_MD = 8 };
@@ -1154,8 +1177,13 @@
         PlmCoefList C;
         const int first_weighted =
             lbfgs_direction_basis(S, Y, c->g, n, m, hist.stored, hist.end, hist.cs.data(), hist.cy.data(), cg, &B, &C);
-        if (trial) PLM_HIP(plm_launch_multiaxpy_trial(c->dir, B, C, n, dinv, first_weighted, xacc, stp0, trial, c->st));
-        else PLM_HIP(plm_launch_multiaxpy(c->dir, B, C, n, dinv, first_weighted, c->st));
+        if (trial) {
+            const PlmScaleFuse fuse = ctx_scale_fuse(c);
+            PLM_HIP(plm_launch_multiaxpy_trial(c->dir, B, C, n, dinv, first_weighted, xacc, stp0, trial, fuse, c->st));
+            c->jexp_of = fuse.state ? trial : nullptr;
+        } else {
+            PLM_HIP(plm_launch_multiaxpy(c->dir, B, C, n, dinv, first_weighted, c->st));
+        }
         return PLM_OK;
     };
 
@@ -1275,8 +1303,11 @@
             int lsrc;
             do {
                 const double stp = ls.next();
-                if (!(ls.count == 0 && (float)stp == stp0))
-                    PLM_HIP(plm_launch_lincomb(c->x, 1.f, c->xp, (float)stp, c->dir, n, c->st));
+                if (!(ls.count == 0 && (float)stp == stp0)) {
+                    const PlmScaleFuse fuse = ctx_scale_fuse(c);
+                    PLM_HIP(plm_launch_lincomb_scale(c->x, 1.f, c->xp, (float)stp, c->dir, n, fuse, c->st));
+                    c->jexp_of = fuse.state ? c->x : nullptr;
+                }
                 PLM_TRY(evaluate_trial());
                 double dg = c->h_scal[SL_DG];
                 fx = c->h_scal[SL_FX];
@@ -1644,11 +1675,66 @@
     PlmVecList B;
     PlmCoefList C;
     const int first_weighted = lbfgs_direction_basis(dS, dY, dg, n, m, stored, end, cs, cy, cg, &B, &C);
-    if (trial) PLM_HIP(plm_launch_multiaxpy_trial(ddir, B, C, n, ddinv, first_weighted, dxacc, stp0, dtrial, nullptr));
+    if (trial) PLM_HIP(plm_launch_multiaxpy_trial(ddir, B, C, n, ddinv, first_weighted, dxacc, stp0, dtrial, PlmScaleFuse(), nullptr));
     else PLM_HIP(plm_launch_multiaxpy(ddir, B, C, n, ddinv, first_weighted, nullptr));
     PLM_HIP(hipDeviceSynchronize());
     PLM_TRY(P.download(dir, ddir, nn));
     if (trial) PLM_TRY(P.download(trial, dtrial, nn));
+    return PLM_OK;
+}
+
+int plm_lbfgs_trial_scale(int64_t n, int64_t nh, int32_t m, int32_t stored, int32_t end, const float *S, const float *Y,
+                          const float *g, const double *cs, const double *cy, double cg, const float *dinv, const float *xacc,
+                          int32_t nsteps, const float *steps, int32_t jexp_bias, int device, float *trials, int32_t *jexp_fused,
+                          int32_t *jexp_pass, int32_t *state_nonzero) {
+    if (!S || !Y || !g || !cs || !cy || !xacc || !steps || !trials || !jexp_fused || !jexp_pass || !state_nonzero)
+        return fail(PLM_EINVAL, "NULL argument");
+    PLM_TRY(lbfgs_probe_length(n));
+    if (nh < 0 || (nh & 3) || nh > n) return fail(PLM_EINVAL, "nh must be a multiple of 4 in 0..n, not %lld", (long long)nh);
+    if (m < 1 || stored < 0 || stored > m) return fail(PLM_EINVAL, "need 0 <= stored <= m (m = %d, stored = %d)", (int)m, (int)stored);
+    if (2 * stored + 1 > PLM_MAX_BASIS) return fail(PLM_EINVAL, "%d basis vectors, at most %d", 2 * (int)stored + 1, PLM_MAX_BASIS);
+    if (end < 0 || end >= m) return fail(PLM_EINVAL, "ring slot %d outside 0..%d", (int)end, (int)m - 1);
+    if (nsteps < 1) return fail(PLM_EINVAL, "no step");
+    PLM_TRY(check_device(device));
+    LbfgsProbe P;
+    float *dS, *dY, *dg, *ddinv = nullptr, *dxacc, *ddir, *dtrial;
+    uint32_t *dstate, *dmaxbits;
+    int32_t *djexp;
+    const size_t nn = (size_t)n;
+    PLM_TRY(P.upload(&dS, S, (size_t)m * nn));
+    PLM_TRY(P.upload(&dY, Y, (size_t)m * nn));
+    PLM_TRY(P.upload(&dg, g, nn));
+    if (dinv) PLM_TRY(P.upload(&ddinv, dinv, nn));
+    PLM_TRY(P.upload(&dxacc, xacc, nn));
+    PLM_TRY(P.nan_out(&ddir, nn));
+    PLM_TRY(P.nan_out(&dtrial, nn));
+    PLM_TRY(P.nan_out(&djexp, (size_t)2));
+    PLM_TRY(P.nan_out(&dmaxbits, (size_t)1));
+    PLM_TRY(P.mem.alloc(&dstate, (size_t)PLM_SCALE_WORDS));
+    PLM_HIP(hipMemset(dstate, 0, sizeof(uint32_t) * PLM_SCALE_WORDS));
+    PlmVecList B;
+    PlmCoefList C;
+    const int first_weighted = lbfgs_direction_basis(dS, dY, dg, n, m, stored, end, cs, cy, cg, &B, &C);
+    PlmScaleFuse fuse;
+    fuse.state = dstate; fuse.jexp = djexp; fuse.first = nh; fuse.bias = jexp_bias;
+    PlmDims d;
+    memset(&d, 0, sizeof d);
+    d.n_local = n; d.nh_pad_l = nh; d.jexp_bias = jexp_bias;
+    for (int k = 0; k < nsteps; k++) {
+        PLM_HIP(hipMemset(djexp, 0xFF, sizeof(int32_t) * 2));
+        if (k == 0) PLM_HIP(plm_launch_multiaxpy_trial(ddir, B, C, n, ddinv, first_weighted, dxacc, steps[0], dtrial, fuse, nullptr));
+        else PLM_HIP(plm_launch_lincomb_scale(dtrial, 1.f, dxacc, steps[k], ddir, n, fuse, nullptr));
+        PLM_HIP(plm_launch_maxabs(d, dtrial, dmaxbits, djexp + 1, nullptr));
+        PLM_HIP(hipDeviceSynchronize());
+        int32_t je[2];
+        PLM_TRY(P.download(je, djexp, (size_t)2));
+        jexp_fused[k] = je[0];
+        jexp_pass[k] = je[1];
+        PLM_TRY(P.download(trials + (size_t)k * nn, dtrial, nn));
+    }
+    std::vector<uint32_t> st((size_t)PLM_SCALE_WORDS);
+    PLM_TRY(P.download(st.data(), dstate, st.size()));
+    *state_nonzero = (int32_t)std::count_if(st.begin(), st.end(), [](uint32_t v) { return v != 0; });
     return PLM_OK;
 }
 
@@ -1811,7 +1897,7 @@
             PLM_HIP(plm_launch_sy_multidot(S, Y, c->x, c->xp, c->g, c->gp, c->dir, B, n, d.nh_pad_l, c->dot_scratch, c->scal + 8,
                                            c->scal + 2, nullptr, 6u, 0ull, c->st));
             B.n -= 1;
-            PLM_HIP(plm_launch_multiaxpy_trial(c->dir, B, C, n, nullptr, m, c->xp, 0.f, c->x, c->st));
+            PLM_HIP(plm_launch_multiaxpy_trial(c->dir, B, C, n, nullptr, m, c->xp, 0.f, c->x, ctx_scale_fuse(c), c->st));
             B.n += 1;
         }
         PLM_HIP(hipEventRecord(ev[1], c->st));
diff --git a/evcouplings_amd/csrc/plm_internal.h b/evcouplings_amd/csrc/plm_internal.h
--- a/evcouplings_amd/csrc/plm_internal.h
+++ b/evcouplings_amd/csrc/plm_internal.h
@@ -44,6 +44,7 @@
     int nrow_tiles, ncol_tiles;
     int fwd_w;
     int bwd_w;
+    int expand_t;
     int64_t nbp;
     int64_t nh_pad;
     int64_t n_native;
@@ -71,6 +72,7 @@
     int ksplit = 0;
     int fwd_kernel = -1;
     int bwd_kernel = -1;
+    int expand_kernel = -1;
     int jexp_bias = 0;
     int fwd_mode = -1;
     double acc_factor = 8.0;
@@ -158,6 +160,15 @@
                                 hipStream_t st);
 hipError_t plm_launch_maxabs(const PlmDims &d, const float *x, uint32_t *maxbits, int32_t *jexp,
                              hipStream_t st);
+#define PLM_SCALE_GROUPS 32
+#define PLM_SCALE_STRIDE 32
+#define PLM_SCALE_WORDS ((2 * PLM_SCALE_GROUPS + 1) * PLM_SCALE_STRIDE)
+struct PlmScaleFuse {
+    uint32_t *state = nullptr;
+    int32_t *jexp = nullptr;
+    int64_t first = 0;
+    int bias = 0;
+};
 hipError_t plm_launch_expand(const PlmDims &d, const float *x, const float *xhalo, const int32_t *jexp,
                              void *Bt, int exact, hipStream_t st);
 hipError_t plm_launch_forward_energy(const PlmDims &d, const int8_t *msa_rm, const void *Bt, const float *x,
@@ -264,4 +275,6 @@
                                   hipStream_t st);
 hipError_t plm_launch_multiaxpy_trial(float *out, const PlmVecList &basis, const PlmCoefList &coef, int64_t n,
                                       const float *dinv, int first_weighted, const float *xacc, float stp, float *trial,
-                                      hipStream_t st);
+                                      const PlmScaleFuse &fuse, hipStream_t st);
+hipError_t plm_launch_lincomb_scale(float *out, float ca, const float *a, float cb, const float *b, int64_t n,
+                                    const PlmScaleFuse &fuse, hipStream_t st);
diff --git a/evcouplings_amd/csrc/plm_kernels.hip b/evcouplings_amd/csrc/plm_kernels.hip
--- a/evcouplings_amd/csrc/plm_kernels.hip
+++ b/evcouplings_amd/csrc/plm_kernels.hip
@@ -458,13 +458,44 @@
         if (t) atomicMax(maxbits, t);
     }
 }
-__global__ void k_scale_from_max(const u32 *maxbits, int32_t *jexp, int bias) {
-    const float mx = __uint_as_float(*maxbits);
+__device__ __forceinline__ int32_t scale_exponent(u32 maxbits, int bias) {
+    const float mx = __uint_as_float(maxbits);
     int e = 0;
     if (mx > 0.f && mx < INFINITY) frexpf(mx, &e);
     int s = PLM_R_EXP - e + bias;
     s = max(-100, min(100, s));
-    *jexp = (mx > 0.f) ? s : 0;
+    return (mx > 0.f) ? s : 0;
+}
+__global__ void k_scale_from_max(const u32 *maxbits, int32_t *jexp, int bias) { *jexp = scale_exponent(*maxbits, bias); }
+
+__device__ __forceinline__ u32 scale_fold(u32 m, const float4 &v) {
+    return max(max(m, __float_as_uint(v.x) & 0x7fffffffu),
+               max(max(__float_as_uint(v.y) & 0x7fffffffu, __float_as_uint(v.z) & 0x7fffffffu), __float_as_uint(v.w) & 0x7fffffffu));
+}
+__device__ __forceinline__ void scale_fuse_finish(const PlmScaleFuse &F, u32 m) {
+    for (int o = 32; o > 0; o >>= 1) m = max(m, (u32)__shfl_down((int)m, o, 64));
+    __shared__ u32 wmax[4];
+    if ((threadIdx.x & 63) == 0) wmax[threadIdx.x >> 6] = m;
+    __syncthreads();
+    if (threadIdx.x != 0) return;
+    const u32 t = max(max(wmax[0], wmax[1]), max(wmax[2], wmax[3]));
+    const u32 grp = blockIdx.x % PLM_SCALE_GROUPS;
+    const u32 members = (gridDim.x - grp + PLM_SCALE_GROUPS - 1) / PLM_SCALE_GROUPS;
+    const u32 ngroups = min((u32)PLM_SCALE_GROUPS, gridDim.x);
+    u32 *slot = F.state + (size_t)grp * PLM_SCALE_STRIDE, *gcnt = F.state + (size_t)(PLM_SCALE_GROUPS + grp) * PLM_SCALE_STRIDE;
+    u32 *top = F.state + (size_t)2 * PLM_SCALE_GROUPS * PLM_SCALE_STRIDE;
+    if (t) {
+        const u32 before = __hip_atomic_fetch_max(slot, t, __ATOMIC_RELAXED, __HIP_MEMORY_SCOPE_AGENT);
+        asm volatile("s_waitcnt vmcnt(0)" : : "v"(before) : "memory");
+    }
+    if (__hip_atomic_fetch_add(gcnt, 1u, __ATOMIC_RELAXED, __HIP_MEMORY_SCOPE_AGENT) != members - 1) return;
+    __hip_atomic_store(gcnt, 0u, __ATOMIC_RELAXED, __HIP_MEMORY_SCOPE_AGENT);
+    if (__hip_atomic_fetch_add(top, 1u, __ATOMIC_RELAXED, __HIP_MEMORY_SCOPE_AGENT) != ngroups - 1) return;
+    u32 mx = 0;
+    for (u32 k = 0; k < ngroups; k++)
+        mx = max(mx, __hip_atomic_exchange(F.state + (size_t)k * PLM_SCALE_STRIDE, 0u, __ATOMIC_RELAXED, __HIP_MEMORY_SCOPE_AGENT));
+    __hip_atomic_store(top, 0u, __ATOMIC_RELAXED, __HIP_MEMORY_SCOPE_AGENT);
+    *F.jexp = scale_exponent(mx, F.bias);
 }
 hipError_t plm_launch_maxabs2(const float *a, int64_t na, const float *b, int64_t nb, u32 *maxbits, int32_t *jexp,
                               int jexp_bias, hipStream_t st) {
@@ -546,6 +577,97 @@
             *(half8 *)(tile_hi + (size_t)(half * d.Q + a) * 512 + lane * 8) = hi;
             *(half8 *)(tile_lo + (size_t)(half * d.Q + a) * 512 + lane * 8) = lo;
         }
+    }
+}
+
+__global__ __launch_bounds__(256) void k_expand_t(PlmDims d, const float *__restrict__ x,
+                                                 const float *__restrict__ xhalo,
+                                                 const int32_t *__restrict__ jexp, _Float16 *__restrict__ Bt) {
+    extern __shared__ float stage[];
+    const int Q = d.Q, QQ = Q * Q, NG = PLM_FWD_NG(Q), SPU = 4 * NG;
+    const int u = blockIdx.x, b16l = blockIdx.y, b16 = d.b16_lo + b16l, a = blockIdx.z;
+    const float *__restrict__ xj = x + d.nh_pad_l;
+    const float *blk[2];
+#pragma unroll
+    for (int J2 = 0; J2 < 2; J2++) {
+        const int J = 2 * u + J2;
+        blk[J2] = nullptr;
+        if (J < d.nb16) {
+            int h = -1;
+            const int64_t k = plm_pair_local(d, min(b16, J), max(b16, J), &h);
+            blk[J2] = k >= 0 ? xj + (size_t)k * QQ * 256 : xhalo + (size_t)h * QQ * 256;
+        }
+    }
+    const int npieces = 2 * Q * 64;
+    for (int p0 = threadIdx.x; p0 < npieces; p0 += 4 * 256) {
+        float4 lo4[4], up4[4];
+#pragma unroll
+        for (int s = 0; s < 4; s++) {
+            const int p = p0 + s * 256;
+            if (p >= npieces) break;
+            const int J2 = p / (Q * 64), rem = p - J2 * Q * 64, b = rem >> 6, row = (rem & 63) >> 2, c4 = (rem & 3) * 4;
+            const int J = 2 * u + J2;
+            const float *bl = J2 ? blk[1] : blk[0];
+            if (!bl) continue;
+            if (J <= b16) lo4[s] = *(const float4 *)(bl + (size_t)(b * Q + a) * 256 + row * 16 + c4);
+            if (J >= b16) up4[s] = *(const float4 *)(bl + (size_t)(a * Q + b) * 256 + row * 16 + c4);
+        }
+#pragma unroll
+        for (int s = 0; s < 4; s++) {
+            const int p = p0 + s * 256;
+            if (p >= npieces) break;
+            const int J2 = p / (Q * 64), rem = p - J2 * Q * 64, b = rem >> 6, row = (rem & 63) >> 2, c4 = (rem & 3) * 4;
+            const int J = 2 * u + J2;
+            const float *bl = J2 ? blk[1] : blk[0];
+            if (!bl) continue;
+            float *t = stage + (size_t)(J2 * Q + b) * 256;
+            if (J < b16) {
+                *(float4 *)(t + row * 16 + c4) = lo4[s];
+            } else if (J > b16) {
+                t[(c4 + 0) * 16 + row] = up4[s].x; t[(c4 + 1) * 16 + row] = up4[s].y;
+                t[(c4 + 2) * 16 + row] = up4[s].z; t[(c4 + 3) * 16 + row] = up4[s].w;
+            } else {
+                const float lv[4] = {lo4[s].x, lo4[s].y, lo4[s].z, lo4[s].w}, uv[4] = {up4[s].x, up4[s].y, up4[s].z, up4[s].w};
+#pragma unroll
+                for (int c = 0; c < 4; c++) {
+                    if (c4 + c > row) t[row * 16 + c4 + c] = lv[c];
+                    if (row < c4 + c) t[(c4 + c) * 16 + row] = uv[c];
+                }
+            }
+        }
+    }
+    __syncthreads();
+    const float sc = ldexpf(1.f, *jexp);
+    const int lane = threadIdx.x & 63, gb = lane >> 4, r = lane & 15, i = b16 * 16 + r;
+    _Float16 *tiles = Bt + ((size_t)b16l * d.nu * SPU + (size_t)u * SPU) * (size_t)(2 * Q * 512);
+    for (int w = threadIdx.x >> 6; w < 4 * NG; w += 4) {
+        const int ci = w >> 1, half = w & 1;
+        const int ga = 2 * half + (gb >> 1), J2 = ga >> 1;
+        half8 hi, lo;
+#pragma unroll
+        for (int e2 = 0; e2 < 2; e2++) {
+            const int pp = 2 * (gb & 1) + e2, gl = 4 * ci + pp, s8 = gl & 7, sg = gl >> 3;
+            const int j = 32 * u + 8 * ga + s8, jj = j & 15;
+            const bool site = i < d.L && j < d.L && i != j;
+            const float *t = stage + (size_t)J2 * Q * 256 + jj * 16 + r;
+            const float ref = (site && !d.gap_mode) ? t[0] : 0.f;
+#pragma unroll
+            for (int e = 0; e < 4; e++) {
+                const int b = 4 * sg + e + 1;
+                float v = 0.f;
+                if (b < Q && site) {
+                    v = t[(size_t)b * 256];
+                    if (!d.gap_mode) v -= ref;
+                    v *= sc;
+                }
+                const _Float16 h = (_Float16)v;
+                hi[4 * e2 + e] = h;
+                lo[4 * e2 + e] = (_Float16)(v - (float)h);
+            }
+        }
+        _Float16 *tile_hi = tiles + (size_t)(2 * ci) * (size_t)(2 * Q * 512), *tile_lo = tile_hi + (size_t)(2 * Q * 512);
+        *(half8 *)(tile_hi + (size_t)(half * Q + a) * 512 + lane * 8) = hi;
+        *(half8 *)(tile_lo + (size_t)(half * Q + a) * 512 + lane * 8) = lo;
     }
 }
 
@@ -600,6 +722,9 @@
     const int NG = PLM_FWD_NG(d.Q);
     if (exact)
         hipLaunchKernelGGL(k_expand_x, dim3(d.nu * NG, d.b16_hi - d.b16_lo), dim3(256), 0, st, d, x, xhalo, jexp, (char *)Bt);
+    else if (d.expand_t)
+        hipLaunchKernelGGL(k_expand_t, dim3(d.nu, d.b16_hi - d.b16_lo, d.Q), dim3(256), (size_t)2 * d.Q * 256 * sizeof(float), st, d,
+                           x, xhalo, jexp, (_Float16 *)Bt);
     else
         hipLaunchKernelGGL(k_expand, dim3(d.nu * 2 * NG, d.b16_hi - d.b16_lo, (d.Q * 64 + 255) / 256), dim3(256), 0, st, d, x, xhalo,
                            jexp, (_Float16 *)Bt);
@@ -2635,7 +2760,9 @@
 }
 
 __global__ __launch_bounds__(256) void k_lincomb(float4 *__restrict__ out, float ca, const float4 *__restrict__ a,
-                                                float cb, const float4 *__restrict__ b, int64_t n4) {
+                                                float cb, const float4 *__restrict__ b, int64_t n4, PlmScaleFuse F) {
+    const int64_t first4 = F.first / 4;
+    u32 m = 0;
     for (int64_t i = (int64_t)blockIdx.x * 256 + threadIdx.x; i < n4; i += (int64_t)gridDim.x * 256) {
         const float4 u = a[i];
         float4 r;
@@ -2647,14 +2774,20 @@
             r.x = ca * u.x; r.y = ca * u.y; r.z = ca * u.z; r.w = ca * u.w;
         }
         out[i] = r;
-    }
+        if (F.state && i >= first4) m = scale_fold(m, r);
+    }
+    if (F.state) scale_fuse_finish(F, m);
+}
+hipError_t plm_launch_lincomb_scale(float *out, float ca, const float *a, float cb, const float *b, int64_t n,
+                                    const PlmScaleFuse &fuse, hipStream_t st) {
+    if ((n & 3) || (fuse.state && (!fuse.jexp || fuse.first < 0 || (fuse.first & 3)))) return hipErrorInvalidValue;
+    hipLaunchKernelGGL(k_lincomb, dim3(2048), dim3(256), 0, st, (float4 *)out, ca, (const float4 *)a, cb,
+                       (const float4 *)b, n / 4, fuse);
+    return hipGetLastError();
 }
 hipError_t plm_launch_lincomb(float *out, float ca, const float *a, float cb, const float *b, int64_t n,
                               hipStream_t st) {
-    if (n & 3) return hipErrorInvalidValue;
-    hipLaunchKernelGGL(k_lincomb, dim3(2048), dim3(256), 0, st, (float4 *)out, ca, (const float4 *)a, cb,
-                       (const float4 *)b, n / 4);
-    return hipGetLastError();
+    return plm_launch_lincomb_scale(out, ca, a, cb, b, n, PlmScaleFuse(), st);
 }
 
 __global__ __launch_bounds__(256) void k_canon_to_native(PlmDims d, const float *__restrict__ xc,
@@ -2979,53 +3112,85 @@
     return hipGetLastError();
 }
 
+#ifndef PLM_VEC_NT
+#define PLM_VEC_NT 1
+#endif
+__device__ __forceinline__ float4 load_stream(const float4 *p) {
+#if PLM_VEC_NT
+    const f32x4 v = __builtin_nontemporal_load((const f32x4 *)p);
+    return make_float4(v.x, v.y, v.z, v.w);
+#else
+    return *p;
+#endif
+}
+__device__ __forceinline__ void store_stream(float4 *p, const float4 &v) {
+#if PLM_VEC_NT
+    __builtin_nontemporal_store((f32x4){v.x, v.y, v.z, v.w}, (f32x4 *)p);
+#else
+    *p = v;
+#endif
+}
+#ifndef AXPY_CHUNK
+#define AXPY_CHUNK 8
+#endif
 __global__ __launch_bounds__(256) void k_multiaxpy(float4 *__restrict__ out, PlmVecList B, PlmCoefList C, int64_t n4,
                                                   const float4 *__restrict__ dinv, int kw,
-                                                  const float4 *__restrict__ xacc, float stp, float4 *__restrict__ trial) {
+                                                  const float4 *__restrict__ xacc, float stp, float4 *__restrict__ trial,
+                                                  PlmScaleFuse F) {
     const int nb = B.n;
+    const int64_t first4 = F.first / 4;
+    u32 m = 0;
     for (int64_t i = (int64_t)blockIdx.x * 256 + threadIdx.x; i < n4; i += (int64_t)gridDim.x * 256) {
-        float4 r = {0.f, 0.f, 0.f, 0.f}, t = {0.f, 0.f, 0.f, 0.f};
-#pragma unroll 4
-        for (int k = 0; k < kw; k++) {
-            const float4 b = ((const float4 *)B.v[k])[i];
-            const float c = C.c[k];
-            r.x = fmaf(c, b.x, r.x); r.y = fmaf(c, b.y, r.y); r.z = fmaf(c, b.z, r.z); r.w = fmaf(c, b.w, r.w);
-        }
-#pragma unroll 4
-        for (int k = kw; k < nb; k++) {
-            const float4 b = ((const float4 *)B.v[k])[i];
-            const float c = C.c[k];
-            t.x = fmaf(c, b.x, t.x); t.y = fmaf(c, b.y, t.y); t.z = fmaf(c, b.z, t.z); t.w = fmaf(c, b.w, t.w);
+        float4 r = {0.f, 0.f, 0.f, 0.f}, t = {0.f, 0.f, 0.f, 0.f}, dv = r, u = r;
+        if (dinv) dv = dinv[i];
+        if (trial) u = xacc[i];
+        for (int k0 = 0; k0 < nb; k0 += AXPY_CHUNK) {
+            float4 b[AXPY_CHUNK];
+#pragma unroll
+            for (int j = 0; j < AXPY_CHUNK; j++)
+                if (k0 + j < nb) b[j] = load_stream((const float4 *)B.v[k0 + j] + i);
+#pragma unroll
+            for (int j = 0; j < AXPY_CHUNK; j++) {
+                if (k0 + j >= nb) break;
+                const float c = C.c[k0 + j];
+                if (k0 + j < kw) {
+                    r.x = fmaf(c, b[j].x, r.x); r.y = fmaf(c, b[j].y, r.y); r.z = fmaf(c, b[j].z, r.z); r.w = fmaf(c, b[j].w, r.w);
+                } else {
+                    t.x = fmaf(c, b[j].x, t.x); t.y = fmaf(c, b[j].y, t.y); t.z = fmaf(c, b[j].z, t.z); t.w = fmaf(c, b[j].w, t.w);
+                }
+            }
         }
         if (dinv) {
-            const float4 dv = dinv[i];
             r.x = fmaf(dv.x, t.x, r.x); r.y = fmaf(dv.y, t.y, r.y); r.z = fmaf(dv.z, t.z, r.z); r.w = fmaf(dv.w, t.w, r.w);
         } else {
             r.x += t.x; r.y += t.y; r.z += t.z; r.w += t.w;
         }
-        out[i] = r;
+        store_stream(out + i, r);
         if (trial) {
-            const float4 u = xacc[i];
-            trial[i] = make_float4(fmaf(stp, r.x, 1.f * u.x), fmaf(stp, r.y, 1.f * u.y), fmaf(stp, r.z, 1.f * u.z),
-                                   fmaf(stp, r.w, 1.f * u.w));
-        }
-    }
+            const float4 tv = make_float4(fmaf(stp, r.x, 1.f * u.x), fmaf(stp, r.y, 1.f * u.y), fmaf(stp, r.z, 1.f * u.z),
+                                          fmaf(stp, r.w, 1.f * u.w));
+            trial[i] = tv;
+            if (F.state && i >= first4) m = scale_fold(m, tv);
+        }
+    }
+    if (F.state) scale_fuse_finish(F, m);
 }
 hipError_t plm_launch_multiaxpy(float *out, const PlmVecList &basis, const PlmCoefList &coef, int64_t n,
                                 const float *dinv, int first_weighted, hipStream_t st) {
     if (basis.n < 1 || basis.n > PLM_MAX_BASIS || (n & 3)) return hipErrorInvalidValue;
     const int kw = dinv ? std::max(0, std::min(basis.n, first_weighted)) : basis.n;
     hipLaunchKernelGGL(k_multiaxpy, dim3(2048), dim3(256), 0, st, (float4 *)out, basis, coef, n / 4,
-                       (const float4 *)dinv, kw, (const float4 *)nullptr, 0.f, (float4 *)nullptr);
+                       (const float4 *)dinv, kw, (const float4 *)nullptr, 0.f, (float4 *)nullptr, PlmScaleFuse());
     return hipGetLastError();
 }
 hipError_t plm_launch_multiaxpy_trial(float *out, const PlmVecList &basis, const PlmCoefList &coef, int64_t n,
                                       const float *dinv, int first_weighted, const float *xacc, float stp, float *trial,
-                                      hipStream_t st) {
+                                      const PlmScaleFuse &fuse, hipStream_t st) {
     if (basis.n < 1 || basis.n > PLM_MAX_BASIS || (n & 3) || !xacc || !trial) return hipErrorInvalidValue;
+    if (fuse.state && (!fuse.jexp || fuse.first < 0 || (fuse.first & 3))) return hipErrorInvalidValue;
     const int kw = dinv ? std::max(0, std::min(basis.n, first_weighted)) : basis.n;
     hipLaunchKernelGGL(k_multiaxpy, dim3(2048), dim3(256), 0, st, (float4 *)out, basis, coef, n / 4,
-                       (const float4 *)dinv, kw, (const float4 *)xacc, stp, (float4 *)trial);
+                       (const float4 *)dinv, kw, (const float4 *)xacc, stp, (float4 *)trial, fuse);
     return hipGetLastError();
 }
 
@@ -3043,10 +3208,10 @@
 __device__ __forceinline__ double dot4(const float4 &a, const float4 &b) {
     return (double)a.x * b.x + (double)a.y * b.y + (double)a.z * b.z + (double)a.w * b.w;
 }
-__global__ __launch_bounds__(256) void k_sy_multidot(PlmSyDot A, double *__restrict__ scratch) {
-    __shared__ double red[4];
+template <bool FIRST, bool W>
+__device__ __forceinline__ void sy_multidot_body(const PlmSyDot &A, double *__restrict__ scratch, double *red) {
     const int k0 = blockIdx.y * SYD_OLD;
-    const bool first = blockIdx.y == 0;
+    constexpr bool first = FIRST;
     const float4 *bp[SYD_OLD];
     unsigned wold = 0;
 #pragma unroll
@@ -3058,8 +3223,7 @@
     const int spos[4] = {A.pos_s, A.pos_y, A.pos_g0, A.pos_g1};
     bool wsp[4];
 #pragma unroll
-    for (int e = 0; e < 4; e++) wsp[e] = spos[e] >= 0 && ((A.wb >> spos[e]) & 1ull);
-    const bool any_w = A.dinv != nullptr && A.wq != 0;
+    for (int e = 0; e < 4; e++) wsp[e] = W && spos[e] >= 0 && ((A.wb >> spos[e]) & 1ull);
     double acc[3][SYD_OLD], sp[3][4], ex[3] = {0, 0, 0}, ssh = 0;
 #pragma unroll
     for (int q = 0; q < 3; q++) {
@@ -3070,39 +3234,45 @@
     }
     for (int64_t i = (int64_t)blockIdx.x * 256 + threadIdx.x; i < A.n4; i += (int64_t)gridDim.x * 256) {
         const float4 xv = A.x[i], xpv = A.xp[i], gv = A.g[i], gpv = A.gp[i];
+        float4 dv = xv, dirv = xv, b[SYD_OLD];
+        if (W) dv = A.dinv[i];
+        if (first) dirv = A.dir[i];
+#pragma unroll
+        for (int k = 0; k < SYD_OLD / 2; k++) b[k] = load_stream(bp[k] + i);
         float4 qv[3], qd[3];
         qv[0] = make_float4(xv.x - xpv.x, xv.y - xpv.y, xv.z - xpv.z, xv.w - xpv.w);
         qv[1] = make_float4(gv.x - gpv.x, gv.y - gpv.y, gv.z - gpv.z, gv.w - gpv.w);
         qv[2] = gv;
         if (first) {
-            A.s_new[i] = qv[0];
-            A.y_new[i] = qv[1];
+            store_stream(A.s_new + i, qv[0]);
+            store_stream(A.y_new + i, qv[1]);
         }
 #pragma unroll
         for (int q = 0; q < 3; q++) qd[q] = qv[q];
-        if (any_w) {
-            const float4 dv = A.dinv[i];
+        if (W) {
 #pragma unroll
             for (int q = 0; q < 3; q++)
                 if ((A.wq >> q) & 1u) { qd[q].x *= dv.x; qd[q].y *= dv.y; qd[q].z *= dv.z; qd[q].w *= dv.w; }
         }
-        if (A.n_old > 0) {
-#pragma unroll
-            for (int k = 0; k < SYD_OLD; k++) {
-                const float4 b = bp[k][i];
-                const bool wk = (wold >> k) & 1u;
-#pragma unroll
-                for (int q = 0; q < 3; q++) acc[q][k] += dot4(wk ? qd[q] : qv[q], b);
-            }
+#pragma unroll
+        for (int k = 0; k < SYD_OLD; k++) {
+            if (k == SYD_OLD / 2) {
+                __builtin_amdgcn_sched_barrier(0);
+#pragma unroll
+                for (int k2 = SYD_OLD / 2; k2 < SYD_OLD; k2++) b[k2] = load_stream(bp[k2] + i);
+            }
+            const bool wk = W && ((wold >> k) & 1u);
+#pragma unroll
+            for (int q = 0; q < 3; q++) acc[q][k] += dot4(wk ? qd[q] : qv[q], b[k]);
         }
         if (first) {
 #pragma unroll
             for (int e = 0; e < 4; e++) {
-                const float4 b = e == 0 ? qv[0] : e == 1 ? qv[1] : gv;
-#pragma unroll
-                for (int q = 0; q < 3; q++) sp[q][e] += dot4(wsp[e] ? qd[q] : qv[q], b);
-            }
-            ex[0] += dot4(gv, A.dir[i]);
+                const float4 bv = e == 0 ? qv[0] : e == 1 ? qv[1] : gv;
+#pragma unroll
+                for (int q = 0; q < 3; q++) sp[q][e] += dot4(wsp[e] ? qd[q] : qv[q], bv);
+            }
+            ex[0] += dot4(gv, dirv);
             const double x2 = dot4(xv, xv);
             ex[1] += x2;
             if (i < A.nh4) {
@@ -3139,6 +3309,17 @@
         const double t = block_reduce_sum(ex[e], red);
         if (threadIdx.x == 0) scratch[((size_t)3 * A.nb + 1 + e) * PLM_DOT_BLOCKS + blockIdx.x] = t;
         __syncthreads();
+    }
+}
+__global__ __launch_bounds__(256, 2) void k_sy_multidot(PlmSyDot A, double *__restrict__ scratch) {
+    __shared__ double red[4];
+    const bool w = A.dinv != nullptr && A.wq != 0;
+    if (blockIdx.y == 0) {
+        if (w) sy_multidot_body<true, true>(A, scratch, red);
+        else sy_multidot_body<true, false>(A, scratch, red);
+    } else {
+        if (w) sy_multidot_body<false, true>(A, scratch, red);
+        else sy_multidot_body<false, false>(A, scratch, red);
     }
 }
 __global__ __launch_bounds__(256) void k_dots_final2(const double *__restrict__ scratch, double *out_a, int na, double *out_b) {
diff --git a/evcouplings_amd/plm.py b/evcouplings_amd/plm.py
--- a/evcouplings_amd/plm.py
+++ b/evcouplings_amd/plm.py
@@ -818,6 +818,20 @@
     check(_lib.load().plm_lbfgs_direction(n, m, int(stored), int(end), _ptr(S), _ptr(Y), _ptr(g), _ptr(cs), _ptr(cy),
                                           float(cg), _ptr(dinv), _ptr(xacc), float(stp0), device, _ptr(out), _ptr(trial)))
     return out if xacc is None else (out, trial)
+
+
+def lbfgs_trial_scale(S, Y, g, cs, cy, cg, stored, end, xacc, steps, nh, dinv=None, jexp_bias=0, device=0):
+    S, Y, g, dinv, xacc, steps = (_f32(a) for a in (S, Y, g, dinv, xacc, steps))
+    cs, cy = _f64(cs), _f64(cy)
+    m, n = S.shape
+    trials = _nan((steps.size, n), np.float32)
+    fused, passed = np.full(steps.size, -9999, np.int32), np.full(steps.size, -9999, np.int32)
+    dirty = C.c_int32(-1)
+    check(_lib.load().plm_lbfgs_trial_scale(n, int(nh), m, int(stored), int(end), _ptr(S), _ptr(Y), _ptr(g), _ptr(cs),
+                                            _ptr(cy), float(cg), _ptr(dinv), _ptr(xacc), steps.size, _ptr(steps),
+                                            int(jexp_bias), device, _ptr(trials), _ptr(fused), _ptr(passed),
+                                            C.byref(dirty)))
+    return trials, fused, passed, dirty.value
 
 
 def lbfgs_multidot(V, q_index, b_index, dinv=None, wq=0, wb=0, device=0):
diff --git a/include/plm_hip.h b/include/plm_hip.h
--- a/include/plm_hip.h
+++ b/include/plm_hip.h
@@ -405,6 +405,10 @@
 int plm_lbfgs_dots(int64_t stride, int32_t nv, const float *V, int32_t npairs, const int32_t *a_index,
                    const int32_t *b_index, int64_t n, int device, double *out);
 int plm_lbfgs_lincomb(int64_t n, float ca, const float *a, float cb, const float *b, int device, float *out);
+int plm_lbfgs_trial_scale(int64_t n, int64_t nh, int32_t m, int32_t stored, int32_t end, const float *S, const float *Y,
+                          const float *g, const double *cs, const double *cy, double cg, const float *dinv, const float *xacc,
+                          int32_t nsteps, const float *steps, int32_t jexp_bias, int device, float *trials, int32_t *jexp_fused,
+                          int32_t *jexp_pass, int32_t *state_nonzero);
 int plm_ctx_precond_diagonal(plm_ctx_t *ctx, float *canonical_out);
 
 void plm_lbfgs_coefficients(int m, int stored, int end, const double *SY, const double *YDY, const double *Sg,
```
